# PJLab-ADG/OpenPCSeg

Hardware: AMD Instinct MI355X
Metric: LiDAR frames/sec training MinkUNet-34 SemanticKITTI (higher is better)
Workload: dtype f32; 1 GPU; MinkUNet-34 cr1.0 train step, 12 x 120k-pt synthetic SemanticKITTI scans/GPU, fp32; global_batch=12, voxels_per_gpu_batch=1158864, parallelism=dp1, wgrad=fp32

## Files before the change

include/pcseg_hip.h:

```cpp
#ifndef PCSEG_HIP_H_
#define PCSEG_HIP_H_

#include <stddef.h>
#include <stdint.h>

#ifdef __cplusplus
extern "C" {
#endif

#define PCS_OK 0
#define PCS_EINVAL (-1)
#define PCS_EWORKSPACE (-2)
#define PCS_ELAUNCH (-3)
#define PCS_EUNSUPPORTED (-4)

#define PCS_ABI_VERSION 12

int pcs_abi_version(void);
const char *pcs_last_error(void);

int pcs_hash(const int32_t *coords, int64_t n, int64_t *out, void *stream);

int pcs_kernel_hash(const int32_t *coords, int64_t n, const int32_t *offsets, int32_t K,
                    int64_t *out, void *stream);

int64_t pcs_hashtable_capacity(int64_t n);
size_t pcs_hashtable_bytes(int64_t capacity);
int pcs_hashtable_build(const int64_t *keys, int64_t n, void *table, int64_t capacity,
                        void *stream);
int pcs_hashtable_query(const void *table, int64_t capacity, const int64_t *queries,
                        int64_t n1, int64_t *out, void *stream);

int pcs_count(const int32_t *idx, int64_t n, int32_t *out, int64_t s, void *stream);

int pcs_voxelize_fwd_f32(const float *feats, const int32_t *idx, const int32_t *counts,
                         int64_t n, int64_t m, int32_t c, float *out, void *stream);
size_t pcs_index_csr_ws_bytes(int64_t n, int64_t m);
int pcs_index_csr_i32(const int32_t *index, int64_t n, int64_t m, int64_t *order, int64_t *rowptr, void *ws,
                      size_t ws_bytes, void *stream);
int pcs_voxelize_fwd_csr_f32(const float *feats, const int64_t *order, const int64_t *rowptr,
                             const int32_t *counts, int64_t m, int32_t c, float *out, void *stream);
int pcs_voxelize_bwd_f32(const float *gout, const int32_t *idx, const int32_t *counts,
                         int64_t n, int32_t c, float *gin, void *stream);
int pcs_voxelize_fwd_csr_h(const void *feats, const int64_t *order, const int64_t *rowptr, const int32_t *counts,
                           int64_t m, int32_t c, int32_t dtype, void *out, void *stream);
int pcs_voxelize_bwd_h(const void *gout, const int32_t *idx, const int32_t *counts, int64_t n, int32_t c,
                       int32_t dtype, void *gin, void *stream);

int pcs_devoxelize_fwd_f32(const float *feat, const int32_t *idx8, const float *w8, int64_t n,
                           int32_t c, float *out, void *stream);
int pcs_devoxelize_bwd_f32(const float *gout, const int32_t *idx8, const float *w8, int64_t n,
                           int64_t m, int32_t c, float *gfeat, void *stream);
int pcs_devoxelize_fwd_h(const void *feat, const int32_t *idx8, const float *w8, int64_t n, int32_t c,
                         int32_t dtype, void *out, void *stream);
int pcs_point_merge_f32(const float *vox, const int32_t *idx8, const float *w8, const float *lin, const double *stat,
                        const float *gamma, const float *beta, int64_t n, int32_t c, float *out, uint32_t *mask,
                        void *stream);
int pcs_point_merge_h(const void *vox, const int32_t *idx8, const float *w8, const void *lin, const double *stat,
                      const float *gamma, const float *beta, int64_t n, int32_t c, int32_t dtype, void *out,
                      uint32_t *mask, void *stream);
int pcs_range_point_merge_f32(const float *vox, const int32_t *idx8, const float *w8, const float *img, const float *pxpy,
                              int32_t B, int32_t H, int32_t W, const float *lin, const double *stat, const float *gamma,
                              const float *beta, int64_t n, int32_t c, float *out, uint32_t *mask, void *stream);
int pcs_range_point_merge_h(const void *vox, const int32_t *idx8, const float *w8, const float *img, const float *pxpy,
                            int32_t B, int32_t H, int32_t W, const void *lin, const double *stat, const float *gamma,
                            const float *beta, int64_t n, int32_t c, int32_t dtype, void *out, uint32_t *mask, void *stream);

int pcs_corner_map_f32(const float *coords, int32_t coord_ld, int64_t n, int32_t stride, const void *table,
                       int64_t capacity, int32_t *idx8, float *w8, void *stream);

int pcs_devoxelize_bwd_csr_f32(const float *gout, const int64_t *order, const int64_t *rowptr,
                               const float *w8, int64_t m, int32_t c, float *gfeat, void *stream);
int pcs_devoxelize_bwd_csr_h(const void *gout, const int64_t *order, const int64_t *rowptr, const float *w8,
                             int64_t m, int32_t c, int32_t dtype, void *gfeat, void *stream);
void pcs_debug_pointvoxel_h_inflight(int32_t loads);

int pcs_ti_weights_f32(const float *coords, int32_t coord_ld, const int64_t *idx_query,
                       int64_t n, float scale, float *w, void *stream);

int pcs_downsample_pack(const int32_t *coords, int64_t n, const int32_t *sample_stride3,
                        int32_t mode, const int32_t *offsets, int32_t K,
                        const int32_t *coords_min3, int64_t *keys, int32_t *err, void *stream);
int pcs_downsample_unpack(const int64_t *keys, int64_t m, int32_t *coords, void *stream);
size_t pcs_sort_unique_ws_bytes(int64_t n);
int pcs_sort_unique_i64(const int64_t *keys, int64_t n, int64_t *out, int64_t *info, const int32_t *err_flag, void *ws,
                        size_t ws_bytes, void *stream);

size_t pcs_rulebook_ws_bytes(int64_t nq, int32_t K);
int pcs_rulebook_probe(const int32_t *qcoords, int64_t nq, const int32_t *offsets, int32_t K,
                       const void *table, int64_t capacity, int32_t *results,
                       int64_t *nbsizes, void *ws, size_t ws_bytes, int32_t symmetric, void *stream);
int pcs_rulebook_fill(const int32_t *results, int64_t nq, int32_t K, const void *ws,
                      int32_t *pairs, int32_t *koff, void *stream);
int pcs_rulebook_tile_segments(const int32_t *pairs, const int32_t *koff, int32_t K,
                               int64_t n_dst, int32_t tile_rows, int32_t dst_col,
                               int32_t *seg, void *stream);
int pcs_rulebook_tile_order(const int32_t *seg, int32_t K, int64_t ntiles, int32_t *order, void *stream);

const char *pcs_conv_kernel_revision(void);
int32_t pcs_conv_tile_rows(int32_t cin, int32_t cout);
int32_t pcs_conv_pick_tile_rows(int64_t n_dst, int64_t n_pairs, int32_t K, int32_t cin, int32_t cout);
int32_t pcs_conv_pick_tile_rows_dt(int64_t n_dst, int64_t n_pairs, int32_t K, int32_t cin, int32_t cout,
                                   int32_t dtype);
int32_t pcs_conv_emits_bn_partials(int32_t cin, int32_t cout, int32_t K, int32_t tile_rows, int32_t dtype);
int32_t pcs_conv_uses_tile_order(int32_t cin, int32_t cout, int32_t K, int32_t dtype);
int pcs_conv_gather_gemm_f32(const float *src, int64_t n_src, int32_t cin, const float *W,
                             int32_t K, int32_t cout, const int32_t *pairs, int32_t src_col,
                             const int32_t *seg, int32_t tile_rows, int64_t n_dst,
                             const float *bias, float *dst, double *bn_partial, const int32_t *tile_order,
                             void *stream);
#define PCS_EP_RELU 1
#define PCS_EP_POST_AFFINE 16
typedef struct pcs_conv_epilogue {
  const void *addend;
  float act_slope;
  int32_t flags;
  const float *post_scale;
  const float *post_shift;
} pcs_conv_epilogue;
int pcs_conv_gather_gemm_f32_ex(const float *src, int64_t n_src, int32_t cin, const float *W,
                                int32_t K, int32_t cout, const int32_t *pairs, int32_t src_col,
                                const int32_t *seg, int32_t tile_rows, int64_t n_dst,
                                const float *bias, const pcs_conv_epilogue *ep, float *dst, double *bn_partial,
                                const int32_t *tile_order, void *stream);
int32_t pcs_conv_supports_epilogue(int32_t cin, int32_t cout, int32_t K, int32_t dtype);

int pcs_transpose_kab_f32(const float *src, int32_t K, int32_t A, int32_t B, float *dst, void *stream);

size_t pcs_conv_wgrad_ws_bytes(const int32_t *koff_host, int32_t K, int32_t ca, int32_t cb);
int pcs_conv_wgrad_f32(const float *fa, int32_t ca, const float *fb, int32_t cb,
                       const int32_t *pairs, int32_t a_col, const int32_t *koff_dev,
                       const int32_t *koff_host, int32_t K, float *gW, void *ws,
                       size_t ws_bytes, void *stream);

int pcs_scatter_max_fwd_f32(const float *src, const int64_t *order, const int64_t *rowptr, int64_t m,
                            int32_t c, float *out, int32_t *arg, void *stream);
int pcs_scatter_max_bwd_f32(const float *gout, const int32_t *arg, int64_t m, int64_t n, int32_t c,
                            float *gsrc, void *stream);

int pcs_map_count(const int32_t *pxpy, int64_t n, int32_t B, int32_t H, int32_t W, int32_t *out,
                  void *stream);
int pcs_denselize_fwd_f32(const float *feat, const int32_t *count_map, const int32_t *pxpy, int64_t n,
                          int32_t B, int32_t C, int32_t H, int32_t W, float *out, void *stream);
int pcs_denselize_fwd_csr_f32(const float *feat, const int64_t *order, const int64_t *rowptr,
                              const int32_t *count_map, int32_t B, int32_t C, int32_t H, int32_t W,
                              float *out, void *stream);
int pcs_denselize_bwd_csr_f32(const float *gout, const int64_t *order, const int64_t *rowptr,
                              const int32_t *count_map, int64_t n, int32_t B, int32_t C, int32_t H, int32_t W,
                              float *gfeat, void *stream);
int pcs_denselize_bwd_f32(const float *gout, const int32_t *count_map, const int32_t *pxpy, int64_t n,
                          int32_t B, int32_t C, int32_t H, int32_t W, float *gfeat, void *stream);

int pcs_range_sample_fwd_f32(const float *img, const float *pxpy, int64_t n, int32_t B, int32_t C, int32_t H, int32_t W,
                             float *out, void *stream);
int pcs_range_sample_corners(const float *pxpy, int64_t n, int32_t B, int32_t H, int32_t W, int64_t *keys, float *wts,
                             void *stream);
int pcs_range_sample_bwd_csr_f32(const float *gout, const int64_t *order, const int64_t *rowptr, const float *wts,
                                 int32_t B, int32_t C, int32_t H, int32_t W, float *gimg, void *stream);

int32_t pcs_bn_num_partials(void);
int pcs_bn_stats_f32(const float *x, int64_t n, int32_t c, float *partial_ws, double *sums, void *stream);
int pcs_bn_reduce_partials(const double *partial, int64_t nrows, int32_t c, int64_t n, double *sums, void *stream);
int pcs_bn_reduce_partials_finalize(const double *partial, int64_t nrows, int32_t c, int64_t n, double eps, double momentum,
                                    float *running_mean, float *running_var, double *sums, double *stat, void *stream);
int pcs_bn_finalize_f32(const double *sums, double count, const double *count_dev, int32_t c, double eps,
                        double momentum, float *running_mean, float *running_var, double *stat, void *stream);
int pcs_bn_apply_f32(const float *x, const float *res, const double *stat, const float *w, const float *b,
                     int64_t n, int32_t c, int32_t relu, float *y, uint32_t *mask, int64_t ldy, const float *tail,
                     int32_t ctail, void *stream);
int pcs_bn_bwd_stats_f32(const float *dy, const float *x, const float *y, const uint32_t *mask, const double *stat,
                         int64_t n, int32_t c, int32_t relu, float *partial_ws, double *sums2, int64_t sums2_doubles,
                         int64_t lddy, void *stream);
int pcs_bn_bwd_apply_f32(const float *dy, const float *x, const float *y, const uint32_t *mask, const double *stat,
                         const double *sums2, double count, const double *count_dev, const float *w, int64_t n,
                         int32_t c, int32_t relu, float *dx, float *dres, int64_t lddy, void *stream);
int pcs_bn_stats_h(const void *x, int64_t n, int32_t c, int32_t dtype, float *partial_ws, double *sums, void *stream);
int pcs_bn_apply_h(const void *x, const void *res, const double *stat, const float *w, const float *b, int64_t n,
                   int32_t c, int32_t relu, int32_t dtype, void *y, uint32_t *mask, int64_t ldy, const void *tail,
                   int32_t ctail, void *stream);
int pcs_bn_bwd_stats_h(const void *dy, const void *x, const void *y, const uint32_t *mask, const double *stat, int64_t n,
                       int32_t c, int32_t relu, int32_t dtype, float *partial_ws, double *sums2, int64_t sums2_doubles,
                       int64_t lddy, void *stream);
int pcs_bn_bwd_apply_h(const void *dy, const void *x, const void *y, const uint32_t *mask, const double *stat,
                       const double *sums2, double count, const double *count_dev, const float *w, int64_t n,
                       int32_t c, int32_t relu, int32_t dtype, void *dx, void *dres, int64_t lddy, void *stream);
int pcs_bn_bwd_apply_act(const void *dy, const void *x, const void *y, const uint32_t *mask, const double *stat,
                         const double *sums2, double count, const double *count_dev, const float *w, int64_t n, int32_t c,
                         int32_t relu, int32_t dtype, float in_slope, void *dx, void *dres, int64_t lddy, void *stream);

int pcs_recon_gate_f32(const float *a0, const float *a1, const float *a2, const float *x, const double *stat3,
                       const float *gamma3, const float *beta3, int64_t n, int32_t c, float *out, void *stream);
int pcs_recon_gate_h(const void *a0, const void *a1, const void *a2, const void *x, const double *stat3, const float *gamma3,
                     const float *beta3, int64_t n, int32_t c, int32_t dtype, void *out, void *stream);
int pcs_recon_gate_bwd_stats_f32(const float *dy, const float *x, const float *a0, const float *a1, const float *a2,
                                 const double *stat3, const float *gamma3, const float *beta3, int64_t n, int32_t c,
                                 float *partial_ws, double *sums2, int64_t sums2_doubles, void *stream);
int pcs_recon_gate_bwd_stats_h(const void *dy, const void *x, const void *a0, const void *a1, const void *a2,
                               const double *stat3, const float *gamma3, const float *beta3, int64_t n, int32_t c,
                               int32_t dtype, float *partial_ws, double *sums2, int64_t sums2_doubles, void *stream);
int pcs_recon_gate_bwd_apply_f32(const float *dy, const float *x, const float *a0, const float *a1, const float *a2,
                                 const double *stat3, const float *gamma3, const float *beta3, const double *sums2,
                                 double count, const double *count_dev, int64_t n, int32_t c, float *dx_gate, float *da0,
                                 float *da1, float *da2, void *stream);
int pcs_recon_gate_bwd_apply_h(const void *dy, const void *x, const void *a0, const void *a1, const void *a2,
                               const double *stat3, const float *gamma3, const float *beta3, const double *sums2, double count,
                               const double *count_dev, int64_t n, int32_t c, int32_t dtype, void *dx_gate, void *da0,
                               void *da1, void *da2, void *stream);

int pcs_quantize_floor(const void *points, int32_t is_float, int64_t n, int32_t row_stride,
                       const double *voxel_size3, int32_t *coords, int32_t *bbox, void *stream);
int pcs_quantize_keys(const int32_t *coords, int64_t n, const int32_t *bbox, int64_t *keys, void *stream);
int pcs_quantize_frame_keys(const int32_t *coords, const int64_t *frames, int64_t n, const int32_t *bbox, int64_t *keys, void *stream);
int pcs_quantize_flags(const int64_t *sorted_keys, int64_t n, int32_t *flags, void *stream);
int pcs_quantize_emit(const int32_t *flags, const int64_t *rank, const int64_t *perm, const int32_t *coords,
                      int64_t n, int32_t *vox, int64_t *index, int64_t *inverse, void *stream);

#define PCS_SCAN_MAX_VOTES 16
#define PCS_SCAN_MAX_COLUMNS 8
int64_t pcs_scan_transform_ws_bytes(int64_t n, int32_t num_frames, int32_t num_votes);
int pcs_scan_transform(const float *points, int64_t n, int32_t c, const int64_t *frame_offsets, int32_t num_frames,
                       const double *params, int32_t num_votes, float voxel_size, float *feats, int32_t *coords,
                       int32_t *mins, void *ws, int64_t ws_bytes, void *stream);
int pcs_scan_shift(int32_t *coords, int64_t n, const int64_t *frame_offsets, int32_t num_frames, const int32_t *mins,
                   int32_t num_votes, int64_t *frames, void *stream);

int pcs_unique_emit(const int32_t *flags, const int64_t *rank, const int64_t *perm, const int64_t *sorted_keys,
                    int64_t n, int64_t *uniq, int64_t *inverse, int64_t *rowptr, void *stream);

int pcs_conv_x3_applies(int32_t cin, int32_t cout, int32_t K);
int32_t pcs_conv_x3_column_tiles(int32_t cout);
int32_t pcs_conv_x3_emits_bn_partials(int32_t cin, int32_t cout, int32_t K, int32_t tile_rows);
size_t pcs_conv_prepared_weights_x3_bytes(int32_t K, int32_t ccon, int32_t ccols);
int pcs_conv_prepare_weights_x3(const float *W, int32_t K, int32_t A, int32_t B, int32_t transpose, void *Wp, void *stream);
int pcs_conv_gather_gemm_f32_bf16x3(const float *src, int64_t n_src, int32_t cin, const void *Wp, int32_t K, int32_t cout,
                                    const int32_t *pairs, int32_t src_col, const int32_t *seg, int32_t tile_rows,
                                    int64_t n_dst, const float *bias, float *dst, double *bn_partial,
                                    const int32_t *tile_order, void *stream);

int pcs_conv_h_applies(int32_t cin, int32_t cout, int32_t K);
size_t pcs_conv_prepared_weights_bytes(int32_t K, int32_t contraction, int32_t columns);
int pcs_conv_prepare_weights_h(const float *W, int32_t K, int32_t A, int32_t B, int32_t transpose, int32_t dtype,
                               void *Wp, void *stream);
int pcs_conv_gather_gemm_h(const void *src, int64_t n_src, int32_t cin, const void *Wp, int32_t K, int32_t cout,
                           const int32_t *pairs, int32_t src_col, const int32_t *seg, int32_t tile_rows,
                           int64_t n_dst, const float *bias, void *dst, int32_t dtype, double *bn_partial,
                           const int32_t *tile_order, void *stream);
int pcs_conv_gather_gemm_h_ex(const void *src, int64_t n_src, int32_t cin, const void *Wp, int32_t K, int32_t cout,
                              const int32_t *pairs, int32_t src_col, const int32_t *seg, int32_t tile_rows,
                              int64_t n_dst, const float *bias, const pcs_conv_epilogue *ep, void *dst, int32_t dtype,
                              double *bn_partial, const int32_t *tile_order, void *stream);
int pcs_conv_wgrad_f32_bf16x3(const float *fa, int32_t ca, const float *fb, int32_t cb, const int32_t *pairs,
                              int32_t a_col, const int32_t *koff_dev, const int32_t *koff_host, int32_t K, float *gW,
                              void *ws, size_t ws_bytes, void *stream);
int pcs_conv_wgrad_h(const void *fa, int32_t ca, const void *fb, int32_t cb, const int32_t *pairs, int32_t a_col,
                     const int32_t *koff_dev, const int32_t *koff_host, int32_t K, float *gW, void *ws,
                     size_t ws_bytes, int32_t dtype, void *stream);

int pcs_cylinder_partition_f32(const float *points, int64_t n, int32_t row_stride, const double *space_min3,
                               const double *space_max3, const int32_t *grid3, float *polar, int32_t *coord,
                               float *feat, void *stream);
int pcs_voxel_label_vote(const int64_t *inverse, const int64_t *labels, int64_t n, int64_t m, int32_t num_classes,
                         int64_t ignore_label, int32_t *counter_ws, int32_t *bad_flag, int64_t *voxel_labels,
                         void *stream);
int pcs_rows_argmax_gather_f32(const float *logits, int64_t m, int32_t c, const int64_t *inverse, int64_t n,
                               int64_t *out, void *stream);

int pcs_cylinder_scan_batch_f32(const float *points, int64_t n, int32_t c, const int64_t *frame_offsets, int32_t num_frames,
                                const double *params, int32_t num_votes, const double *space_min3, const double *space_max3,
                                const int32_t *grid3, float *feat, int32_t *coord, int64_t *scenes, void *stream);

int64_t pcs_range_project_ws_bytes(int32_t num_scenes, int32_t H, int32_t W);
int pcs_range_project_f32(const float *feats, int64_t n, int32_t c, const int32_t *scenes, const float *cuts32, int32_t num_scenes,
                          int32_t H, int32_t W, int32_t *winner, float *pxpy, int32_t *bad, void *stream);
int pcs_range_image_fill_f32(const int32_t *winner, const float *feats, int64_t n, int32_t c, int32_t num_scenes, int32_t H,
                             int32_t W, float *image, void *stream);

int64_t pcs_range_scan_ws_bytes(int32_t num_frames, int32_t H, int32_t W);
int pcs_range_scan_f32(const float *points, int64_t n, int32_t c, const int64_t *frame_offsets, int32_t num_frames,
                       const int64_t *labels, const int64_t *lut, int32_t lut_size, int32_t H, int32_t W, float fov_down_abs,
                       float fov_total, int32_t mask_hit, void *winner, float *scan, int64_t *label_rv, float *mask_rv,
                       int32_t *proj_idx, int32_t *proj_x, int32_t *proj_y, float *unproj_range, int32_t *bad, void *stream);
int pcs_range_knn_vote(const float *proj_range, const int64_t *proj_argmax, int32_t num_scenes, int32_t H, int32_t W,
                       const float *unproj_range, const int32_t *proj_x, const int32_t *proj_y, int64_t n,
                       const int64_t *point_offset, int32_t search, int32_t knn, float cutoff, const float *weights_host,
                       int32_t num_class, const int64_t *labels, int64_t *hist, int64_t *pred, void *stream);

#define PCS_MIX_BUCKETS 10
#define PCS_MIX_MAX_CLASSES 8
#define PCS_MIX_PLAN_STRIDE 16
int64_t pcs_scan_mix_ws_bytes(int64_t n1, int64_t n2, int32_t num_frames);
int pcs_scan_mix_count(const float *points1, int64_t n1, const int64_t *frame_offsets1, const float *points2,
                       const int64_t *labels2, int64_t n2, const int64_t *frame_offsets2, int32_t num_frames, const double *plan,
                       const int64_t *classes, int32_t num_classes, void *ws, int64_t ws_bytes, int32_t *totals,
                       int64_t *frame_base, void *stream);
int pcs_scan_mix_place(const float *points1, const int64_t *labels1, int64_t n1, const int64_t *frame_offsets1,
                       const float *points2, const int64_t *labels2, int64_t n2, const int64_t *frame_offsets2,
                       int32_t num_frames, const double *plan, const int64_t *classes, int32_t num_classes, const double *omega,
                       const void *ws, int64_t ws_bytes, const int32_t *totals, const int64_t *frame_base, int64_t m, int32_t c_out,
                       float *out_points, int64_t *out_labels, void *stream);
int64_t pcs_scan_ring_ws_bytes(int64_t m);
int pcs_scan_ring_f32(float *points, int64_t m, int32_t c, const int64_t *frame_base, int32_t num_frames, void *ws,
                      int64_t ws_bytes, void *stream);

int pcs_predict_points_f32(const float *logits, int64_t m, int32_t c, const int64_t *inverse, int64_t n,
                           const int64_t *point_offset, const int64_t *row_offset, int32_t n_scenes,
                           const int64_t *labels, float *votes, int64_t *pred, int64_t *hist, int32_t *bad_flag,
                           void *stream);

typedef struct {
  const float *src;
  void *dst;
  int32_t K, A, B;
  int32_t kind;
  int32_t transpose;
  int32_t nctt, nt16, ns;
  int64_t first_block;
} pcs_weight_job;
int64_t pcs_weights_multi_plan(pcs_weight_job *jobs_host, int32_t n_jobs);
int pcs_weights_multi(const pcs_weight_job *jobs_dev, int32_t n_jobs, int64_t total_blocks, void *stream);

#define PCS_STEP_BLOCK_ELEMS 4096
#define PCS_STEP_MAX_GROUPS 8
#define PCS_STEP_WS_BYTES(total_blocks) (16 + 12 * (int64_t)(total_blocks))
typedef struct {
  float *p;
  const float *g;
  float *buf;
  int64_t numel;
  int32_t group;
  int32_t reserved;
  int64_t first_block;
} pcs_step_job;
typedef struct {
  float lr[PCS_STEP_MAX_GROUPS], wd[PCS_STEP_MAX_GROUPS], mu[PCS_STEP_MAX_GROUPS];
  int32_t nesterov[PCS_STEP_MAX_GROUPS];
  int32_t n_groups;
} pcs_step_hyper;
int64_t pcs_step_plan(pcs_step_job *jobs_host, int32_t n_jobs, const pcs_step_hyper *hyper);
int pcs_step_norm(const pcs_step_job *jobs_dev, int32_t n_jobs, int64_t total_blocks, float max_norm, float *scale,
                  int32_t *growth_tracker, double growth_factor, double backoff_factor, int32_t growth_interval, void *ws,
                  int64_t ws_bytes, float *record, void *stream);
int pcs_step_apply(const pcs_step_job *jobs_dev, int32_t n_jobs, int64_t total_blocks, const pcs_step_hyper *hyper,
                   const float *record, int32_t skip_on_inf, void *stream);

int64_t pcs_lovasz_workspace_bytes(int64_t n, int32_t num_class, int32_t has_ignore, int64_t ignore);
int pcs_lovasz_softmax_f32(const float *probas, const int64_t *labels, int64_t n, int32_t num_class, int32_t has_ignore,
                           int64_t ignore, float *loss, float *grad, void *ws, int64_t ws_bytes, void *stream);

void pcs_debug_convh_ws(int32_t mode, int32_t ru, int32_t rs);
void pcs_debug_conv_plan(int32_t kind, int32_t dtype, int32_t cin, int32_t cout, int32_t K, int32_t tile_rows, int32_t flags,
                         int32_t out[12]);
void pcs_debug_wgrad_interleave(int32_t mode);
void pcs_debug_cylscan_store(int32_t form);

#ifdef __cplusplus
}
#endif
#endif
```

openpcseg_amd/csrc/conv_wgrad.hip:

```cpp
#include "conv_common.h"

using namespace pcs;

namespace {

constexpr int WG_PB = 32;
constexpr int WG_TS = 128 + 16;

struct WgradArgs {
  const float *fa;
  const float *fb;
  const int32_t *pairs;
  const int32_t *koff;
  float *partial;
  int ca, cb, K, a_col, pch;
};

__device__ __forceinline__ void find_split(const int32_t *koff, int K, int pch, int split, int *k_out,
                                           int *beg, int *end) {
  int acc = 0;
  for (int k = 0; k < K; ++k) {
    const int nk = koff[k + 1] - koff[k];
    const int ns = (nk + pch - 1) / pch;
    if (split < acc + ns) {
      const int s = split - acc;
      *k_out = k;
      *beg = koff[k] + s * pch;
      const int e = *beg + pch;
      *end = e < koff[k + 1] ? e : koff[k + 1];
      return;
    }
    acc += ns;
  }
  *k_out = -1; *beg = 0; *end = 0;
}

__device__ __forceinline__ void find_split_wave(const int32_t *koff, int K, int pch, int split, int lane, int *beg,
                                                int *end, int *gsid, int interleave) {
  if (K > 64) {
    int k;
    find_split(koff, K, pch, split, &k, beg, end);
    *gsid = split;
    return;
  }
  const int lo = lane < K ? koff[lane] : 0, hi = lane < K ? koff[lane + 1] : 0;
  const int ns = (hi - lo + pch - 1) / pch;
  int incl = ns;
  for (int o = 1; o < 64; o <<= 1) {
    const int t = __shfl_up(incl, o, 64);
    if (lane >= o) incl += t;
  }
  int src, sidx;
  if (!interleave) {
    const unsigned long long hit = __ballot(split >= incl - ns && split < incl);
    if (!hit) { *beg = 0; *end = 0; *gsid = split; return; }
    src = __ffsll((long long)hit) - 1;
    sidx = split - __shfl(incl - ns, src, 64);
  } else {
    const int total = __shfl(incl, 63, 64);
    if (interleave == 2) {
      const int chunk = (total + 7) >> 3;
      split = (split & 7) * chunk + (split >> 3);
    }
    if (split >= total) { *beg = 0; *end = 0; *gsid = 0; return; }
    int rmax = ns;
    for (int o = 32; o > 0; o >>= 1) { const int t = __shfl_xor(rmax, o, 64); rmax = t > rmax ? t : rmax; }
    auto upto = [&](int r) {
      int c = ns > 0 ? (int)(((long long)r * ns) / rmax) + 1 : 0;
      for (int o = 32; o > 0; o >>= 1) c += __shfl_xor(c, o, 64);
      return c;
    };
    int a = 0, b = rmax - 1;
    while (a < b) {
      const int m = (a + b) >> 1;
      if (upto(m) > split) b = m; else a = m + 1;
    }
    const int r = a;
    const int before = r > 0 ? upto(r - 1) : 0;
    const int s_r = ns > 0 ? (int)(((long long)r * ns) / rmax) : -1;
    const int s_p = (ns > 0 && r > 0) ? (int)(((long long)(r - 1) * ns) / rmax) : -1;
    unsigned long long fresh = __ballot(ns > 0 && s_r != s_p);
    int want = split - before;
    while (want > 0) { fresh &= fresh - 1; --want; }
    src = __ffsll((long long)fresh) - 1;
    sidx = __shfl(s_r, src, 64);
  }
  const int b0 = lo + sidx * pch;
  const int e0 = b0 + pch < hi ? b0 + pch : hi;
  *beg = __shfl(b0, src, 64);
  *end = __shfl(e0, src, 64);
  *gsid = __shfl(incl - ns, src, 64) + sidx;
}

__global__ void __launch_bounds__(256) wgrad_kernel(WgradArgs w) {
  __shared__ __attribute__((aligned(16))) float abuf[WG_PB * WG_TS];
  __shared__ __attribute__((aligned(16))) float bbuf[WG_PB * WG_TS];
  __shared__ int ia[WG_PB], ib[WG_PB];
  __shared__ int sh[3];
  const int tid = threadIdx.x, lane = tid & 63, wid = tid >> 6;
  const int a0 = blockIdx.y * 128, b0 = blockIdx.z * 128;
  const int cat = (w.ca - a0) < 128 ? (w.ca - a0) : 128;
  const int cbt = (w.cb - b0) < 128 ? (w.cb - b0) : 128;
  const int ta_n = (cat + 15) / 16, tb_n = (cbt + 15) / 16;
  if (tid == 0) find_split(w.koff, w.K, w.pch, blockIdx.x, &sh[0], &sh[1], &sh[2]);
  __syncthreads();
  const int beg = sh[1], end = sh[2];
  const int wa = wid >> 1, wb = wid & 1;
  f32x4 acc[4][4];
#pragma unroll
  for (int i = 0; i < 4; ++i)
#pragma unroll
    for (int j = 0; j < 4; ++j) acc[i][j] = (f32x4){0, 0, 0, 0};

  const int capad = ta_n * 16, cbpad = tb_n * 16;
  for (int p0 = beg; p0 < end; p0 += WG_PB) {
    const int np = (end - p0) < WG_PB ? (end - p0) : WG_PB;
    __syncthreads();
    if (tid < WG_PB) {
      int2 p = make_int2(-1, -1);
      if (tid < np) p = reinterpret_cast<const int2 *>(w.pairs)[p0 + tid];
      ia[tid] = w.a_col ? p.y : p.x;
      ib[tid] = w.a_col ? p.x : p.y;
    }
    __syncthreads();
    for (int e = tid; e < WG_PB * capad; e += 256) {
      const int r = e / capad, c = e % capad;
      abuf[r * WG_TS + c] = (r < np && c < cat) ? w.fa[(int64_t)ia[r] * w.ca + a0 + c] : 0.f;
    }
    for (int e = tid; e < WG_PB * cbpad; e += 256) {
      const int r = e / cbpad, c = e % cbpad;
      bbuf[r * WG_TS + c] = (r < np && c < cbt) ? w.fb[(int64_t)ib[r] * w.cb + b0 + c] : 0.f;
    }
    __syncthreads();
    const int g = lane >> 4, l15 = lane & 15;
#pragma unroll
    for (int kk = 0; kk < WG_PB / 4; ++kk) {
      float av[4], bv[4];
#pragma unroll
      for (int i = 0; i < 4; ++i) {
        const int ta = wa + 2 * i;
        av[i] = (ta < ta_n) ? abuf[(kk * 4 + g) * WG_TS + ta * 16 + l15] : 0.f;
      }
#pragma unroll
      for (int j = 0; j < 4; ++j) {
        const int tb = wb + 2 * j;
        bv[j] = (tb < tb_n) ? bbuf[(kk * 4 + g) * WG_TS + tb * 16 + l15] : 0.f;
      }
#pragma unroll
      for (int i = 0; i < 4; ++i) {
        if (wa + 2 * i < ta_n) {
#pragma unroll
          for (int j = 0; j < 4; ++j) {
            if (wb + 2 * j < tb_n)
// ... 97 lines not shown
  __syncthreads();
  if (ql == 0 && ok) {
    float4 t = red[0][et];
#pragma unroll
    for (int j = 1; j < 16; ++j) {
      const float4 v = red[j][et];
      t.x += v.x; t.y += v.y; t.z += v.z; t.w += v.w;
    }
    *reinterpret_cast<float4 *>(gW + (int64_t)k * cc + e) = t;
  }
}

struct Wgrad2Args {
  const void *fa;
  const void *fb;
  const int32_t *pairs;
  const int32_t *koff;
  float *partial;
  int ca, cb, K, a_col, pch, nbg;
  int interleave;
};

__host__ __device__ inline int wg_ngroups(int c) { return (c + 63) / 64; }
__host__ __device__ inline int wg_gwidth(int c) {
  const int per = (c + wg_ngroups(c) - 1) / wg_ngroups(c);
  return (per + 15) / 16 * 16;
}

template <int W> struct WVec;
template <> struct WVec<64> { using T = float4; static constexpr int N = 4; };
template <> struct WVec<48> { using T = float3; static constexpr int N = 3; };
template <> struct WVec<32> { using T = float2; static constexpr int N = 2; };
template <> struct WVec<16> { using T = float;  static constexpr int N = 1; };
__device__ __forceinline__ float wcomp(const float4 &v, int i) { return i == 0 ? v.x : (i == 1 ? v.y : (i == 2 ? v.z : v.w)); }
__device__ __forceinline__ float wcomp(const float3 &v, int i) { return i == 0 ? v.x : (i == 1 ? v.y : v.z); }
__device__ __forceinline__ float wcomp(const float2 &v, int i) { return i == 0 ? v.x : v.y; }
__device__ __forceinline__ float wcomp(const float &v, int) { return v; }

template <typename V, int N> __device__ __forceinline__ V wload(Fp32, const void *base, int64_t elem) {
  return *reinterpret_cast<const V *>(reinterpret_cast<const float *>(base) + elem);
}
template <typename V, int N, typename HT> __device__ __forceinline__ V wload(HT, const void *base, int64_t elem) {
  const uint16_t *p = reinterpret_cast<const uint16_t *>(base) + elem;
  V v;
  if constexpr (N == 4) {
    const uint2 r = *reinterpret_cast<const uint2 *>(p);
    v.x = h2f(HT{}, (uint16_t)(r.x & 0xFFFFu)); v.y = h2f(HT{}, (uint16_t)(r.x >> 16));
    v.z = h2f(HT{}, (uint16_t)(r.y & 0xFFFFu)); v.w = h2f(HT{}, (uint16_t)(r.y >> 16));
  } else if constexpr (N == 3) {
    v.x = h2f(HT{}, p[0]); v.y = h2f(HT{}, p[1]); v.z = h2f(HT{}, p[2]);
  } else if constexpr (N == 2) {
    const uint32_t r = *reinterpret_cast<const uint32_t *>(p);
    v.x = h2f(HT{}, (uint16_t)(r & 0xFFFFu)); v.y = h2f(HT{}, (uint16_t)(r >> 16));
  } else {
    v = h2f(HT{}, p[0]);
  }
  return v;
}

template <int AW, int BW, typename ET>
__device__ __forceinline__ void wgrad_block(const Wgrad2Args &w, int a0, int b0, int beg, int end,
                                            float *out, int lane) {
  using AV = typename WVec<AW>::T;
  using BV = typename WVec<BW>::T;
  constexpr int NA = WVec<AW>::N, NB = WVec<BW>::N;
  const int g = lane >> 4, l15 = lane & 15;
  const int ac = a0 + NA * l15, bc = b0 + NB * l15;
  const bool aok = ac + NA <= w.ca, bok = bc + NB <= w.cb;
  const int acl = aok ? ac : 0, bcl = bok ? bc : 0;
  f32x4 acc[NA][NB];
#pragma unroll
  for (int f = 0; f < NA; ++f)
#pragma unroll
    for (int h = 0; h < NB; ++h) acc[f][h] = (f32x4){0, 0, 0, 0};

  struct Batch { AV a[4]; BV b[4]; };
  auto load_pairs = [&](int p0) {
    int pi = p0 + l15;
    pi = pi < end ? pi : end - 1;
    return reinterpret_cast<const int2 *>(w.pairs)[pi];
  };
  auto load_rows = [&](Batch &bt, const int2 pr) {
    const int ia = w.a_col ? pr.y : pr.x, ib = w.a_col ? pr.x : pr.y;
#pragma unroll
    for (int j = 0; j < 4; ++j) {
      const int ra = __shfl(ia, 4 * j + g, 64), rb = __shfl(ib, 4 * j + g, 64);
      bt.a[j] = wload<AV, NA>(ET{}, w.fa, (int64_t)ra * w.ca + acl);
      bt.b[j] = wload<BV, NB>(ET{}, w.fb, (int64_t)rb * w.cb + bcl);
    }
  };
  auto mfma_batch = [&](const Batch &bt, int p0) {
#pragma unroll
    for (int j = 0; j < 4; ++j) {
      const bool pv = aok && (p0 + 4 * j + g) < end;
#pragma unroll
      for (int f = 0; f < NA; ++f) {
        const float av = pv ? wcomp(bt.a[j], f) : 0.f;
#pragma unroll
        for (int h = 0; h < NB; ++h)
          acc[f][h] = __builtin_amdgcn_mfma_f32_16x16x4f32(av, wcomp(bt.b[j], h), acc[f][h], 0, 0, 0);
      }
    }
  };
  Batch b0s, b1s;
  load_rows(b0s, load_pairs(beg));
  int2 prn = load_pairs(beg + 16 < end ? beg + 16 : beg);
#ifndef PCS_ABLATEW
#define PCS_ABLATEW 0
#endif
#if PCS_ABLATEW == 1
  load_rows(b1s, prn);
#endif
  for (int p0 = beg; p0 < end; p0 += 32) {
    const int p2 = p0 + 32 < end ? p0 + 32 : p0;
    const int p3 = p0 + 48 < end ? p0 + 48 : p0;
#if PCS_ABLATEW != 1
    load_rows(b1s, prn);
#endif
    prn = load_pairs(p2);
    __builtin_amdgcn_sched_barrier(0);
#if PCS_ABLATEW != 2
    mfma_batch(b0s, p0);
#else
    acc[0][0][0] += wcomp(b0s.a[0], 0) + wcomp(b0s.a[1], 0) + wcomp(b0s.a[2], 0) + wcomp(b0s.a[3], 0) + wcomp(b0s.b[0], 0) + wcomp(b0s.b[1], 0) + wcomp(b0s.b[2], 0) + wcomp(b0s.b[3], 0);
#endif
    __builtin_amdgcn_sched_barrier(0);
#if PCS_ABLATEW != 1
    load_rows(b0s, prn);
#endif
    prn = load_pairs(p3);
    __builtin_amdgcn_sched_barrier(0);
#if PCS_ABLATEW != 2
    if (p0 + 16 < end) mfma_batch(b1s, p0 + 16);
#else
    acc[0][0][1] += wcomp(b1s.a[0], 0) + wcomp(b1s.a[1], 0) + wcomp(b1s.a[2], 0) + wcomp(b1s.a[3], 0) + wcomp(b1s.b[0], 0) + wcomp(b1s.b[1], 0) + wcomp(b1s.b[2], 0) + wcomp(b1s.b[3], 0);
#endif
    __builtin_amdgcn_sched_barrier(0);
  }
#pragma unroll
  for (int f = 0; f < NA; ++f) {
#pragma unroll
    for (int r = 0; r < 4; ++r) {
      const int row = a0 + NA * (4 * g + r) + f;
      if (row < w.ca && bok) {
        float *d = out + (int64_t)row * w.cb + bc;
#pragma unroll
        for (int h = 0; h < NB; ++h) d[h] = acc[f][h][r];
      }
    }
  }
}

template <typename ET>
__global__ void __launch_bounds__(256, 3) wgrad2_kernel(Wgrad2Args w) {
  const int tid = threadIdx.x, lane = tid & 63, wid = tid >> 6;
  int beg, end, gsid;
  find_split_wave(w.koff, w.K, w.pch, blockIdx.x, lane, &beg, &end, &gsid, w.interleave);
  const int nag = wg_ngroups(w.ca);
  const int nsb = (w.nbg + 1) >> 1;
  const int sa = blockIdx.y / nsb, sb = blockIdx.y - sa * nsb;
  const int ag = 2 * sa + (wid >> 1), bg = 2 * sb + (wid & 1);
  if (beg >= end || ag >= nag || bg >= w.nbg) return;
  const int aw = wg_gwidth(w.ca), bw = wg_gwidth(w.cb);
  float *out = w.partial + (int64_t)gsid * w.ca * w.cb;
  const int a0 = aw * ag, b0 = bw * bg;
#define PCS_WG_CASE(A, B) if (aw == A && bw == B) { wgrad_block<A, B, ET>(w, a0, b0, beg, end, out, lane); return; }
  PCS_WG_CASE(64, 64) PCS_WG_CASE(64, 48) PCS_WG_CASE(64, 32) PCS_WG_CASE(64, 16)
  PCS_WG_CASE(48, 64) PCS_WG_CASE(48, 48) PCS_WG_CASE(48, 32) PCS_WG_CASE(48, 16)
  PCS_WG_CASE(32, 64) PCS_WG_CASE(32, 48) PCS_WG_CASE(32, 32) PCS_WG_CASE(32, 16)
  PCS_WG_CASE(16, 64) PCS_WG_CASE(16, 48) PCS_WG_CASE(16, 32) PCS_WG_CASE(16, 16)
#undef PCS_WG_CASE
}

constexpr int W3_PB = 32;
constexpr int W3_ROW = 128;

typedef __bf16 w3_bf16x2 __attribute__((ext_vector_type(2)));
typedef float w3_f32x2 __attribute__((ext_vector_type(2)));
typedef __bf16 w3_bf16x8 __attribute__((ext_vector_type(8)));
typedef _Float16 w3_f16x8 __attribute__((ext_vector_type(8)));

struct Wgrad3Args {
  const void *fa;
  const void *fb;
  const int32_t *pairs;
  const int32_t *koff;
  float *partial;
  int ca, cb, K, a_col, pch;
  int aw, bw, nag, nbg, nsb;
  int interleave;
  int nsy = 1;
};

template <typename ET> struct W3Mode;
template <> struct W3Mode<Fp32> { static constexpr int PLANES = 3; using MT = Bf16; };
template <> struct W3Mode<Bf16> { static constexpr int PLANES = 1; using MT = Bf16; };
template <> struct W3Mode<Fp16> { static constexpr int PLANES = 1; using MT = Fp16; };

__device__ __forceinline__ f32x4 w3_mfma(Bf16, const uint4 &a, const uint4 &b, f32x4 c) {
  return __builtin_amdgcn_mfma_f32_16x16x32_bf16(__builtin_bit_cast(w3_bf16x8, a), __builtin_bit_cast(w3_bf16x8, b), c, 0, 0, 0);
}
__device__ __forceinline__ f32x4 w3_mfma(Fp16, const uint4 &a, const uint4 &b, f32x4 c) {
  return __builtin_amdgcn_mfma_f32_16x16x32_f16(__builtin_bit_cast(w3_f16x8, a), __builtin_bit_cast(w3_f16x8, b), c, 0, 0, 0);
}

__device__ __forceinline__ void w3_split(float x, float y, uint32_t &hi, uint32_t &mid, uint32_t &lo) {
  const w3_f32x2 v = {x, y};
  const w3_bf16x2 h = __builtin_convertvector(v, w3_bf16x2);
  const w3_f32x2 r1 = v - __builtin_convertvector(h, w3_f32x2);
  const w3_bf16x2 m = __builtin_convertvector(r1, w3_bf16x2);
  const w3_f32x2 r2 = r1 - __builtin_convertvector(m, w3_f32x2);
  const w3_bf16x2 l = __builtin_convertvector(r2, w3_bf16x2);
  hi = __builtin_bit_cast(uint32_t, h); mid = __builtin_bit_cast(uint32_t, m); lo = __builtin_bit_cast(uint32_t, l);
}

template <typename ET, int NA, int NB, int NT = 256, int ROW = W3_ROW>
__global__ void __launch_bounds__(NT, NT == 256 ? (W3Mode<ET>::PLANES == 1 ? 3 : 2) : 4) wgrad3_kernel(Wgrad3Args w) {
  constexpr int PL = W3Mode<ET>::PLANES;
  using MT = typename W3Mode<ET>::MT;
  constexpr bool F32IN = std::is_same<ET, Fp32>::value;
  constexpr int NBUF = PL == 1 ? 2 : 1;
  constexpr int IMG = PL * 2 * W3_PB * ROW;
  __shared__ __attribute__((aligned(16))) uint16_t lds[NBUF * IMG];
  const int tid = threadIdx.x, lane = tid & 63, wid = tid >> 6;
  const int g = lane >> 4, l15 = lane & 15;
  int beg, end, gsid;
  int bx = blockIdx.x, by = blockIdx.y;
  if (w.interleave == 2 && w.nsy > 1) {
    const int slot = bx >> 3;
    by = slot % w.nsy;
    bx = ((slot / w.nsy) << 3) | (bx & 7);
  }
  find_split_wave(w.koff, w.K, w.pch, bx, lane, &beg, &end, &gsid, w.interleave);
  if (beg >= end) return;
  const int sa = by / w.nsb, sb = by - sa * w.nsb;
  const int a_base = 2 * sa * w.aw, b_base = 2 * sb * w.bw;
  const int a_stage = (w.ca - a_base) < 2 * w.aw ? (w.ca - a_base) : 2 * w.aw;
  const int b_stage = (w.cb - b_base) < 2 * w.bw ? (w.cb - b_base) : 2 * w.bw;
  const int ag = 2 * sa + (wid >> 1), bg = 2 * sb + (wid & 1);
  const bool active = ag < w.nag && bg < w.nbg;
  const int aoff = (wid >> 1) * w.aw, boff = (wid & 1) * w.bw;

  f32x4 acc[NA][NB];
#pragma unroll
  for (int i = 0; i < NA; ++i)
#pragma unroll
    for (int j = 0; j < NB; ++j) acc[i][j] = (f32x4){0, 0, 0, 0};

  constexpr int CPP = F32IN ? 4 : 8;
  constexpr int PPR = ROW / CPP;
  constexpr int PIECES = (W3_PB / 2) * PPR / NT;
  static_assert(PIECES >= 1 && (W3_PB / 2) * PPR % NT == 0, "staging items must divide over the threads");
  uint32_t *ldw = reinterpret_cast<uint32_t *>(lds);
  constexpr int IMGW = IMG / 2;
  constexpr int OPW = (W3_PB / 2) * ROW;
  auto wpos = [](int q, int ch) { return q * ROW + ((((ch >> 4) ^ (q >> 2)) & (ROW / 16 - 1)) << 4) + (ch & 15); };
  int2 prs[PIECES][2];
  uint4 ra[PIECES][2], rb[PIECES][2];
  auto fetch_pairs = [&](int p0) {
#pragma unroll
    for (int i = 0; i < PIECES; ++i) {
      const int q = (tid + NT * i) / PPR;
#pragma unroll
      for (int h = 0; h < 2; ++h) {
        prs[i][h] = make_int2(-1, -1);
        if (p0 + 2 * q + h < end) prs[i][h] = reinterpret_cast<const int2 *>(w.pairs)[p0 + 2 * q + h];
      }
    }
  };
  auto fetch_rows = [&]() {
#pragma unroll
    for (int i = 0; i < PIECES; ++i) {
      const int c = ((tid + NT * i) % PPR) * CPP;
#pragma unroll
      for (int h = 0; h < 2; ++h) {
        const bool pv = prs[i][h].x >= 0;
        const int ia = w.a_col ? prs[i][h].y : prs[i][h].x, ib = w.a_col ? prs[i][h].x : prs[i][h].y;
        ra[i][h] = make_uint4(0u, 0u, 0u, 0u);
        rb[i][h] = make_uint4(0u, 0u, 0u, 0u);
        if (pv && c < a_stage) {
          if (F32IN) ra[i][h] = *reinterpret_cast<const uint4 *>(reinterpret_cast<const float *>(w.fa) + (int64_t)ia * w.ca + a_base + c);
          else ra[i][h] = *reinterpret_cast<const uint4 *>(reinterpret_cast<const uint16_t *>(w.fa) + (int64_t)ia * w.ca + a_base + c);
        }
        if (pv && c < b_stage) {
          if (F32IN) rb[i][h] = *reinterpret_cast<const uint4 *>(reinterpret_cast<const float *>(w.fb) + (int64_t)ib * w.cb + b_base + c);
          else rb[i][h] = *reinterpret_cast<const uint4 *>(reinterpret_cast<const uint16_t *>(w.fb) + (int64_t)ib * w.cb + b_base + c);
        }
      }
    }
  };
  auto stage = [&](int buf) {
#pragma unroll
    for (int i = 0; i < PIECES; ++i) {
      const int e = tid + NT * i, q = e / PPR, c = (e % PPR) * CPP;
      const int pos = wpos(q, c);
#pragma unroll
      for (int op = 0; op < 2; ++op) {
        const uint4 v0 = op ? rb[i][0] : ra[i][0], v1 = op ? rb[i][1] : ra[i][1];
        uint32_t *base = ldw + buf * IMGW + op * OPW + pos;
        if (F32IN) {
          uint4 hi, mid, lo;
          w3_split(__uint_as_float(v0.x), __uint_as_float(v1.x), hi.x, mid.x, lo.x);
          w3_split(__uint_as_float(v0.y), __uint_as_float(v1.y), hi.y, mid.y, lo.y);
          w3_split(__uint_as_float(v0.z), __uint_as_float(v1.z), hi.z, mid.z, lo.z);
          w3_split(__uint_as_float(v0.w), __uint_as_float(v1.w), hi.w, mid.w, lo.w);
          *reinterpret_cast<uint4 *>(base) = hi;
          *reinterpret_cast<uint4 *>(base + 2 * OPW) = mid;
          *reinterpret_cast<uint4 *>(base + 4 * OPW) = lo;
        } else {
          uint4 w0, w1;
          w0.x = __builtin_amdgcn_perm(v1.x, v0.x, 0x05040100u); w0.y = __builtin_amdgcn_perm(v1.x, v0.x, 0x07060302u);
          w0.z = __builtin_amdgcn_perm(v1.y, v0.y, 0x05040100u); w0.w = __builtin_amdgcn_perm(v1.y, v0.y, 0x07060302u);
          w1.x = __builtin_amdgcn_perm(v1.z, v0.z, 0x05040100u); w1.y = __builtin_amdgcn_perm(v1.z, v0.z, 0x07060302u);
          w1.z = __builtin_amdgcn_perm(v1.w, v0.w, 0x05040100u); w1.w = __builtin_amdgcn_perm(v1.w, v0.w, 0x07060302u);
          *reinterpret_cast<uint4 *>(base) = w0;
          *reinterpret_cast<uint4 *>(base + 4) = w1;
        }
      }
    }
  };
  auto frag = [&](int buf, int plane, int op, int ch) {
    const uint32_t *q = ldw + buf * IMGW + (plane * 2 + op) * OPW + wpos(4 * g, ch);
    uint4 f;
    f.x = q[0 * ROW]; f.y = q[1 * ROW]; f.z = q[2 * ROW]; f.w = q[3 * ROW];
    return f;
  };
  auto compute = [&](int buf) {
    uint4 bf[NB][PL];
#pragma unroll
    for (int j = 0; j < NB; ++j)
#pragma unroll
      for (int pl = 0; pl < PL; ++pl) bf[j][pl] = frag(buf, pl, 1, boff + 16 * j + l15);
#pragma unroll
    for (int i = 0; i < NA; ++i) {
      uint4 af[PL];
#pragma unroll
      for (int pl = 0; pl < PL; ++pl) af[pl] = frag(buf, pl, 0, aoff + 16 * i + l15);
      if (PL == 3) {
#pragma unroll
        for (int j = 0; j < NB; ++j) acc[i][j] = w3_mfma(MT{}, af[PL - 1], bf[j][0], acc[i][j]);
#pragma unroll
        for (int j = 0; j < NB; ++j) acc[i][j] = w3_mfma(MT{}, af[0], bf[j][PL - 1], acc[i][j]);
#pragma unroll
        for (int j = 0; j < NB; ++j) acc[i][j] = w3_mfma(MT{}, af[PL / 2], bf[j][PL / 2], acc[i][j]);
#pragma unroll
        for (int j = 0; j < NB; ++j) acc[i][j] = w3_mfma(MT{}, af[PL / 2], bf[j][0], acc[i][j]);
#pragma unroll
        for (int j = 0; j < NB; ++j) acc[i][j] = w3_mfma(MT{}, af[0], bf[j][PL / 2], acc[i][j]);
      }
#pragma unroll
      for (int j = 0; j < NB; ++j) acc[i][j] = w3_mfma(MT{}, af[0], bf[j][0], acc[i][j]);
    }
  };

  fetch_pairs(beg);
  fetch_rows();
  fetch_pairs(beg + W3_PB);
  stage(0);
  __syncthreads();
  int cur = 0;
  for (int p0 = beg; p0 < end; p0 += W3_PB) {
    const bool more = p0 + W3_PB < end;
    if (more) {
      fetch_rows();
      fetch_pairs(p0 + 2 * W3_PB);
    }
    if (active) compute(cur);
    if (NBUF == 2) {
      if (more) stage(cur ^ 1);
      __syncthreads();
      cur ^= 1;
    } else {
      __syncthreads();
      if (more) stage(0);
      __syncthreads();
    }
  }
  if (!active) return;
  const int a0 = a_base + aoff, b0 = b_base + boff;
  float *out = w.partial + (int64_t)gsid * w.ca * w.cb;
#pragma unroll
  for (int i = 0; i < NA; ++i)
#pragma unroll
    for (int r = 0; r < 4; ++r) {
      const int row = a0 + 16 * i + 4 * g + r;
      if (row < w.ca) {
#pragma unroll
        for (int j = 0; j < NB; ++j) {
          const int col = b0 + 16 * j + l15;
          if (col < w.cb) out[(int64_t)row * w.cb + col] = acc[i][j][r];
        }
      }
    }
}

struct WgradEnv { int wgrad3, thin, target, interleave; };
const WgradEnv &wgrad_env() {
  auto num = [](const char *v, int dflt) { return v ? atoi(v) : dflt; };
  static const WgradEnv env = {num(getenv("PCS_WGRAD3"), 1),
                               num(getenv("PCS_WGRAD3_THIN"), 1),
                               num(getenv("PCS_WGRAD_TARGET"), 0),
                               num(getenv("PCS_WGRAD_INTERLEAVE"), -1)};
  return env;
}

int g_wgrad_interleave = -1;
enum class WgradFamily { generic, wgrad2, wgrad3, wgrad3_thin };
struct WgradPlan { WgradFamily family; int pch, ns, interleave; dim3 grid; };

int wgrad_splits(const int32_t *koff_host, int K, int pch) {
  int64_t ns = 0;
  for (int k = 0; k < K; ++k) ns += ceil_div((int64_t)koff_host[k + 1] - koff_host[k], pch);
  return (int)ns;
}

WgradPlan wgrad_route(const int32_t *koff_host, int K, int ca, int cb, int dtype, bool force_split, bool operands_aligned,
                      int use3 = wgrad_env().wgrad3, bool count = true) {
  const WgradEnv &env = wgrad_env();
  const bool half = dtype != 0;
  const int nag = wg_ngroups(ca), nbg = wg_ngroups(cb);
  WgradPlan p;
  const bool thin = use3 >= 1 && env.thin && half && ca % 16 == 0 && cb % 16 == 0 && ca <= 64 && cb <= 64 && ca >= 32 && cb >= 32 &&
                    operands_aligned;
  const bool vec = (ca % 4 == 0) && (cb % 4 == 0) && operands_aligned;
  const int cgran = half ? 8 : 4;
  const bool want3 = !half ? (use3 == 2 || force_split) : (use3 >= 1 && (use3 == 2 || nag * nbg >= 4));
  p.family = thin ? WgradFamily::wgrad3_thin
                  : (vec && want3 && ca % cgran == 0 && cb % cgran == 0) ? WgradFamily::wgrad3
                                                                         : (vec ? WgradFamily::wgrad2 : WgradFamily::generic);
  const int nbq = (nag * nbg + 3) / 4;
  const int64_t P = koff_host[K] - koff_host[0];
  int64_t target = (env.target > 0 ? env.target : (nbq >= 4 ? (half ? 2048 : 3072) : 1536)) / nbq;
  if (thin) target *= 4;
  if (target < K) target = K;
  p.pch = (int)ceil_div(P > 0 ? P : 1, target);
  p.pch = (int)(ceil_div(p.pch, 32) * 32);
  if (p.pch < 64) p.pch = 64;
  p.ns = count ? wgrad_splits(koff_host, K, p.pch) : 0;
  p.interleave = g_wgrad_interleave >= 0 ? g_wgrad_interleave : (env.interleave >= 0 ? env.interleave : (half ? 2 : 0));
  const unsigned nx = (unsigned)(p.interleave == 2 ? 8 * ((p.ns + 7) / 8) : p.ns), nsy = (unsigned)(((nag + 1) / 2) * ((nbg + 1) / 2));
  if (p.family == WgradFamily::generic) p.grid = dim3((unsigned)p.ns, (unsigned)ceil_div(ca, 128), (unsigned)ceil_div(cb, 128));
  else if (p.family == WgradFamily::wgrad2) p.grid = dim3(nx, nsy);
  else p.grid = p.interleave == 2 ? dim3(nx * nsy, 1u) : dim3((unsigned)p.ns, nsy);
  return p;
}

template <typename Args>
Args wgrad_args(const void *fa, const void *fb, const int32_t *pairs, const int32_t *koff_dev, void *ws, int ca, int cb, int K,
                int a_col, int pch) {
  Args w;
  w.fa = static_cast<decltype(w.fa)>(fa); w.fb = static_cast<decltype(w.fb)>(fb); w.pairs = pairs; w.koff = koff_dev;
  w.partial = reinterpret_cast<float *>(ws);
  w.ca = ca; w.cb = cb; w.K = K; w.a_col = a_col; w.pch = pch;
  return w;
}

template <typename ET, int NT, int ROW>
int launch_wgrad3(const Wgrad3Args &w, dim3 grid, hipStream_t st, const char *what) {
  const int na = w.aw / 16, nb = w.bw / 16;
#define PCS_W3_CASE(A, B) if constexpr (NT == 256 || (A >= 2 && B >= 2)) if (na == A && nb == B) { hipLaunchKernelGGL((wgrad3_kernel<ET, A, B, NT, ROW>), grid, dim3(NT), 0, st, w); return check_launch(what); }
  PCS_W3_CASE(4, 4) PCS_W3_CASE(4, 3) PCS_W3_CASE(4, 2) PCS_W3_CASE(4, 1)
  PCS_W3_CASE(3, 4) PCS_W3_CASE(3, 3) PCS_W3_CASE(3, 2) PCS_W3_CASE(3, 1)
  PCS_W3_CASE(2, 4) PCS_W3_CASE(2, 3) PCS_W3_CASE(2, 2) PCS_W3_CASE(2, 1)
  PCS_W3_CASE(1, 4) PCS_W3_CASE(1, 3) PCS_W3_CASE(1, 2) PCS_W3_CASE(1, 1)
#undef PCS_W3_CASE
  set_error("%s: unreachable", what);
  return PCS_EINVAL;
}

}

extern "C" size_t pcs_conv_wgrad_ws_bytes(const int32_t *koff_host, int32_t K, int32_t ca, int32_t cb) {
  if (!koff_host || K <= 0 || ca <= 0 || cb <= 0) return 0;
  int pch = INT_MAX;
  for (int dtype = 0; dtype <= 2; ++dtype)
    for (int in = 0; in < 4; ++in)
      for (int use3 = 0; use3 <= 2; ++use3) pch = std::min(pch, wgrad_route(koff_host, K, ca, cb, dtype, in & 1, in & 2, use3, false).pch);
  return (size_t)std::max(wgrad_splits(koff_host, K, pch), 1) * ca * cb * sizeof(float);
}

extern "C" void pcs_debug_wgrad_interleave(int32_t mode) { g_wgrad_interleave = mode; }

static int conv_wgrad_any(const void *fa, int32_t ca, const void *fb, int32_t cb, const int32_t *pairs, int32_t a_col,
                          const int32_t *koff_dev, const int32_t *koff_host, int32_t K, float *gW, void *ws, size_t ws_bytes,
                          int dtype, void *stream, bool force_split = false) {
  if (ca <= 0 || cb <= 0 || K <= 0 || !koff_dev || !koff_host || !gW || (a_col != 0 && a_col != 1) || dtype < 0 || dtype > 2) {
    set_error("pcs_conv_wgrad_f32: bad args");
    return PCS_EINVAL;
  }
  hipStream_t st = as_stream(stream);
  const WgradPlan p = wgrad_route(koff_host, K, ca, cb, dtype, force_split, (((uintptr_t)fa | (uintptr_t)fb) & 15) == 0);
  const int64_t cc = (int64_t)ca * cb;
  if (p.ns == 0) {
    if (hipMemsetAsync(gW, 0, (size_t)K * cc * 4, st) != hipSuccess) { set_error("pcs_conv_wgrad_f32: memset failed"); return PCS_ELAUNCH; }
    return PCS_OK;
  }
  if (!fa || !fb || !pairs || !ws) { set_error("pcs_conv_wgrad_f32: null pointer"); return PCS_EINVAL; }
  if (ws_bytes < (size_t)p.ns * cc * 4) { set_error("pcs_conv_wgrad_f32: workspace too small"); return PCS_EWORKSPACE; }
  const bool vec = p.family != WgradFamily::generic;
  if (dtype != 0 && !vec) { set_error("pcs_conv_wgrad_h: half operands need channel counts that are multiples of 4 and 16-byte aligned tensors"); return PCS_EUNSUPPORTED; }
  switch (p.family) {
    case WgradFamily::generic:
      hipLaunchKernelGGL(wgrad_kernel, p.grid, dim3(256), 0, st, wgrad_args<WgradArgs>(fa, fb, pairs, koff_dev, ws, ca, cb, K, a_col, p.pch));
      break;
    case WgradFamily::wgrad2: {
      Wgrad2Args w = wgrad_args<Wgrad2Args>(fa, fb, pairs, koff_dev, ws, ca, cb, K, a_col, p.pch);
      w.nbg = wg_ngroups(cb); w.interleave = p.interleave;
      if (dtype == 0) hipLaunchKernelGGL(wgrad2_kernel<Fp32>, p.grid, dim3(256), 0, st, w);
      else if (dtype == 1) hipLaunchKernelGGL(wgrad2_kernel<Bf16>, p.grid, dim3(256), 0, st, w);
      else hipLaunchKernelGGL(wgrad2_kernel<Fp16>, p.grid, dim3(256), 0, st, w);
      break;
    }
    default: {
      Wgrad3Args w = wgrad_args<Wgrad3Args>(fa, fb, pairs, koff_dev, ws, ca, cb, K, a_col, p.pch);
      w.aw = wg_gwidth(ca); w.bw = wg_gwidth(cb); w.nag = wg_ngroups(ca); w.nbg = wg_ngroups(cb); w.nsb = (w.nbg + 1) / 2;
      w.interleave = p.interleave;
      w.nsy = ((w.nag + 1) / 2) * w.nsb;
      const bool thin = p.family == WgradFamily::wgrad3_thin;
      const char *what = thin ? "pcs_conv_wgrad(wgrad3 thin)" : "pcs_conv_wgrad(wgrad3)";
      const int rc3 = thin ? (dtype == 1 ? launch_wgrad3<Bf16, 64, 64>(w, p.grid, st, what) : launch_wgrad3<Fp16, 64, 64>(w, p.grid, st, what))
                      : dtype == 0 ? launch_wgrad3<Fp32, 256, W3_ROW>(w, p.grid, st, what)
                      : dtype == 1 ? launch_wgrad3<Bf16, 256, W3_ROW>(w, p.grid, st, what) : launch_wgrad3<Fp16, 256, W3_ROW>(w, p.grid, st, what);
      if (rc3) return rc3;
    }
  }
  int rc = check_launch("pcs_conv_wgrad_f32");
  if (rc) return rc;
  if (vec && (((uintptr_t)ws | (uintptr_t)gW) & 15) == 0) {
    hipLaunchKernelGGL(wgrad_reduce4_kernel, dim3((unsigned)ceil_div(cc, 64), K), dim3(256), 0, st,
                       reinterpret_cast<const float *>(ws), koff_dev, (int)K, p.pch, cc, gW);
  } else {
    int gx = (int)ceil_div(cc, 256);
    if (gx > 64) gx = 64;
    hipLaunchKernelGGL(wgrad_reduce_kernel, dim3(gx, K), dim3(256), 0, st,
                       reinterpret_cast<const float *>(ws), koff_dev, (int)K, p.pch, cc, gW);
  }
  return check_launch("pcs_conv_wgrad_f32(reduce)");
}

extern "C" int pcs_conv_wgrad_f32(const float *fa, int32_t ca, const float *fb, int32_t cb,
                                  const int32_t *pairs, int32_t a_col, const int32_t *koff_dev,
                                  const int32_t *koff_host, int32_t K, float *gW, void *ws,
                                  size_t ws_bytes, void *stream) {
  return conv_wgrad_any(fa, ca, fb, cb, pairs, a_col, koff_dev, koff_host, K, gW, ws, ws_bytes, 0, stream);
}

extern "C" int pcs_conv_wgrad_h(const void *fa, int32_t ca, const void *fb, int32_t cb,
                                const int32_t *pairs, int32_t a_col, const int32_t *koff_dev,
                                const int32_t *koff_host, int32_t K, float *gW, void *ws,
                                size_t ws_bytes, int32_t dtype, void *stream) {
  if (dtype != 1 && dtype != 2) { set_error("pcs_conv_wgrad_h: dtype must be 1 (bf16) or 2 (fp16)"); return PCS_EINVAL; }
  return conv_wgrad_any(fa, ca, fb, cb, pairs, a_col, koff_dev, koff_host, K, gW, ws, ws_bytes, dtype, stream);
}

extern "C" int pcs_conv_wgrad_f32_bf16x3(const float *fa, int32_t ca, const float *fb, int32_t cb,
                                         const int32_t *pairs, int32_t a_col, const int32_t *koff_dev,
                                         const int32_t *koff_host, int32_t K, float *gW, void *ws,
                                         size_t ws_bytes, void *stream) {
  if ((ca % 4) || (cb % 4) || (((uintptr_t)fa | (uintptr_t)fb) & 15)) { set_error("pcs_conv_wgrad_f32_bf16x3: needs 16-byte granular rows"); return PCS_EUNSUPPORTED; }
  return conv_wgrad_any(fa, ca, fb, cb, pairs, a_col, koff_dev, koff_host, K, gW, ws, ws_bytes, 0, stream, true);
}
```

openpcseg_amd/csrc/norm.hip:

```cpp
#include "row_storage.h"

using namespace pcs;

namespace {

template <int V> struct NV;
template <> struct NV<4> { using T = float4; };
template <> struct NV<1> { using T = float; };
template <int V, typename ET> __device__ __forceinline__ typename NV<V>::T ldv(ET, const void *p, int64_t e) {
  const Acc<V> a = widen(ET{}, *reinterpret_cast<const typename Raw<ET, V>::T *>(reinterpret_cast<const typename Elem<ET>::T *>(p) + e));
  if constexpr (V == 4) return make_float4(a.f[0], a.f[1], a.f[2], a.f[3]);
  else return a.f[0];
}
template <typename ET> __device__ __forceinline__ void stv(ET, void *p, int64_t e, const float4 &v) {
  *reinterpret_cast<typename Raw<ET, 4>::T *>(reinterpret_cast<typename Elem<ET>::T *>(p) + e) = narrow(ET{}, Acc<4>{{v.x, v.y, v.z, v.w}});
}
template <typename ET> __device__ __forceinline__ void stv(ET, void *p, int64_t e, const float &v) {
  reinterpret_cast<typename Elem<ET>::T *>(p)[e] = narrow(ET{}, Acc<1>{{v}});
}

__device__ __forceinline__ float comp(const float4 &v, int i) { return i == 0 ? v.x : (i == 1 ? v.y : (i == 2 ? v.z : v.w)); }
__device__ __forceinline__ float comp(const float &v, int) { return v; }
__device__ __forceinline__ void setc(float4 &v, int i, float s) { if (i == 0) v.x = s; else if (i == 1) v.y = s; else if (i == 2) v.z = s; else v.w = s; }
__device__ __forceinline__ void setc(float &v, int, float s) { v = s; }


template <bool BWD, int V, typename ET>
__global__ void __launch_bounds__(256) bn_partial_kernel(const void *__restrict__ x, const void *__restrict__ dy,
                                                         const void *__restrict__ y, const uint32_t *__restrict__ mask,
                                                         const double *__restrict__ stat,
                                                         int64_t n, int c, int cv, int relu, float *__restrict__ partial,
                                                         int64_t lddy) {
  using VT = typename NV<V>::T;
  extern __shared__ float red[];
  const int tx = threadIdx.x, ty = threadIdx.y, TX = blockDim.x, TY = blockDim.y;
  const int W = TX * V;
  for (int j0 = 0; j0 < cv; j0 += TX) {
    const int j = j0 + tx;
    float s0[V], s1[V];
#pragma unroll
    for (int q = 0; q < V; ++q) { s0[q] = 0.f; s1[q] = 0.f; }
    if (j < cv) {
      float mean[V], invstd[V];
#pragma unroll
      for (int q = 0; q < V; ++q) {
        mean[q] = BWD ? (float)stat[j * V + q] : (n > 0 ? ldv<1>(ET{}, x, j * V + q) : 0.f);
        invstd[q] = BWD ? (float)stat[c + j * V + q] : 0.f;
        if (!BWD && blockIdx.x == 0 && ty == 0) partial[(int64_t)gridDim.x * 2 * c + j * V + q] = mean[q];
      }
#pragma unroll 4
      for (int64_t i = (int64_t)blockIdx.x * TY + ty; i < n; i += (int64_t)gridDim.x * TY) {
        const VT xv = ldv<V>(ET{}, x, i * c + (int64_t)j * V);
        if (BWD) {
          const VT gv = ldv<V>(ET{}, dy, i * lddy + (int64_t)j * V);
          VT yv; unsigned bits = 0xFu;
          if (relu) {
            if (V == 4 && mask) bits = (mask[i * (c >> 5) + (j >> 3)] >> (4 * (j & 7))) & 0xFu;
            else yv = ldv<V>(ET{}, y, i * c + (int64_t)j * V);
          }
#pragma unroll
          for (int q = 0; q < V; ++q) {
            float g = comp(gv, q);
            if (relu && ((V == 4 && mask) ? !((bits >> q) & 1u) : comp(yv, q) <= 0.f)) g = 0.f;
            s0[q] += g;
            s1[q] += g * ((comp(xv, q) - mean[q]) * invstd[q]);
          }
        } else {
#pragma unroll
          for (int q = 0; q < V; ++q) { const float t = comp(xv, q) - mean[q]; s0[q] += t; s1[q] += t * t; }
        }
      }
    }
#pragma unroll
    for (int q = 0; q < V; ++q) {
      red[(ty * 2 + 0) * W + tx * V + q] = s0[q];
      red[(ty * 2 + 1) * W + tx * V + q] = s1[q];
    }
    __syncthreads();
    if (ty == 0 && j < cv) {
#pragma unroll
      for (int q = 0; q < V; ++q) {
        float a = 0.f, b = 0.f;
        for (int r = 0; r < TY; ++r) { a += red[(r * 2 + 0) * W + tx * V + q]; b += red[(r * 2 + 1) * W + tx * V + q]; }
        partial[((int64_t)blockIdx.x * 2 + 0) * c + j * V + q] = a;
        partial[((int64_t)blockIdx.x * 2 + 1) * c + j * V + q] = b;
      }
    }
    __syncthreads();
  }
}

template <typename PT>
__global__ void __launch_bounds__(1024) bn_reduce_kernel(const PT *__restrict__ partial, int nblk, int c,
                                                         const float *__restrict__ pivot, int64_t n,
                                                         double *__restrict__ sums, int write_count,
                                                         float *__restrict__ f32copy = nullptr, double *__restrict__ stat = nullptr,
                                                         double eps = 0.0, double momentum = 0.0, float *running_mean = nullptr,
                                                         float *running_var = nullptr) {
  __shared__ double red[2][kRedLanes][kRedCh + 1];
  __shared__ double red2[2][16][kRedCh + 1];
  const int ch = blockIdx.x * kRedCh + threadIdx.x;
  double s0 = 0.0, s1 = 0.0;
  if (ch < c) {
    PT v0[8], v1[8];
    for (int b0 = threadIdx.y; b0 < nblk; b0 += kRedLanes * 8) {
#pragma unroll
      for (int u = 0; u < 8; ++u) {
        const int b = b0 + kRedLanes * u;
        v0[u] = b < nblk ? partial[(int64_t)b * 2 * c + ch] : (PT)0;
        v1[u] = b < nblk ? partial[(int64_t)b * 2 * c + c + ch] : (PT)0;
      }
#pragma unroll
      for (int u = 0; u < 8; ++u) { s0 += (double)v0[u]; s1 += (double)v1[u]; }
    }
  }
  red[0][threadIdx.y][threadIdx.x] = s0;
  red[1][threadIdx.y][threadIdx.x] = s1;
  __syncthreads();
  if (threadIdx.y < 16) {
    double a = 0.0, b = 0.0;
    for (int r = 0; r < 16; ++r) { a += red[0][threadIdx.y * 16 + r][threadIdx.x]; b += red[1][threadIdx.y * 16 + r][threadIdx.x]; }
    red2[0][threadIdx.y][threadIdx.x] = a;
    red2[1][threadIdx.y][threadIdx.x] = b;
  }
  __syncthreads();
  if (threadIdx.y == 0 && ch < c) {
    double t0 = 0.0, t1 = 0.0;
    for (int r = 0; r < 16; ++r) { t0 += red2[0][r][threadIdx.x]; t1 += red2[1][r][threadIdx.x]; }
    if (pivot) {
      const double p = n > 0 ? (double)pivot[ch] : 0.0, dn = (double)n;
      t1 = t1 + 2.0 * p * t0 + dn * p * p;
      t0 = t0 + dn * p;
    }
    if (sums) {
      sums[ch] = t0;
      sums[c + ch] = t1;
    }
    if (f32copy) {
      f32copy[ch] = (float)t0;
      f32copy[c + ch] = (float)t1;
    }
    if (stat) {
      const double count = n > 0 ? (double)n : 1.0;
      const double mean = t0 / count;
      double var = t1 / count - mean * mean;
      if (var < 0.0) var = 0.0;
      stat[ch] = mean;
      stat[c + ch] = 1.0 / sqrt(var + eps);
      if (running_mean) {
        const double unb = count > 1.0 ? var * count / (count - 1.0) : var;
        running_mean[ch] = (float)((1.0 - momentum) * running_mean[ch] + momentum * mean);
        running_var[ch] = (float)((1.0 - momentum) * running_var[ch] + momentum * unb);
      }
    }
  }
  if (sums && write_count && blockIdx.x == 0 && threadIdx.x == 0 && threadIdx.y == 0) sums[2 * c] = (double)n;
}

__global__ void __launch_bounds__(256) bn_finalize_kernel(const double *__restrict__ sums, double count,
                                                          const double *__restrict__ count_dev, int c,
                                                          double eps, double momentum, float *running_mean,
                                                          float *running_var, double *__restrict__ stat) {
  const int ch = blockIdx.x * blockDim.x + threadIdx.x;
  if (ch >= c) return;
  if (count_dev) count = *count_dev;
  if (!(count > 0.0)) count = 1.0;
  const double mean = sums[ch] / count;
  double var = sums[c + ch] / count - mean * mean;
  if (var < 0.0) var = 0.0;
  stat[ch] = mean;
  stat[c + ch] = 1.0 / sqrt(var + eps);
  if (running_mean) {
    const double unb = count > 1.0 ? var * count / (count - 1.0) : var;
    running_mean[ch] = (float)((1.0 - momentum) * running_mean[ch] + momentum * mean);
    running_var[ch] = (float)((1.0 - momentum) * running_var[ch] + momentum * unb);
  }
}

template <int V, typename ET>
__global__ void __launch_bounds__(256) bn_apply_kernel(const void *__restrict__ x, const void *__restrict__ res,
                                                       const double *__restrict__ stat, const float *__restrict__ w,
                                                       const float *__restrict__ b, int64_t n, int c, int cv, int relu,
                                                       void *__restrict__ y, uint32_t *__restrict__ mask, int64_t ldy,
                                                       const void *__restrict__ tail, int ctail) {
  using VT = typename NV<V>::T;
  for (int j = threadIdx.x; j < ctail / V; j += blockDim.x) {
#pragma unroll 4
    for (int64_t i = (int64_t)blockIdx.x * blockDim.y + threadIdx.y; i < n; i += (int64_t)gridDim.x * blockDim.y)
      stv(ET{}, y, i * ldy + c + (int64_t)j * V, ldv<V>(ET{}, tail, i * ctail + (int64_t)j * V));
  }
  for (int j = threadIdx.x; j < cv; j += blockDim.x) {
    float sc[V], sh[V];
#pragma unroll
    for (int q = 0; q < V; ++q) {
      const int ch = j * V + q;
      const float invstd = (float)stat[c + ch], mean = (float)stat[ch];
      sc[q] = invstd * (w ? w[ch] : 1.f);
      sh[q] = (b ? b[ch] : 0.f) - mean * sc[q];
    }
#pragma unroll 4
    for (int64_t i = (int64_t)blockIdx.x * blockDim.y + threadIdx.y; i < n; i += (int64_t)gridDim.x * blockDim.y) {
      const VT xv = ldv<V>(ET{}, x, i * c + (int64_t)j * V);
      VT rv; if (res) rv = ldv<V>(ET{}, res, i * c + (int64_t)j * V);
      VT o;
#pragma unroll
      for (int q = 0; q < V; ++q) {
        float t = fmaf(comp(xv, q), sc[q], sh[q]);
        if (res) t += comp(rv, q);
        if (relu && t < 0.f) t = 0.f;
        setc(o, q, t);
      }
      stv(ET{}, y, i * ldy + (int64_t)j * V, o);
      if (V == 4 && mask) {
        unsigned bits = 0;
#pragma unroll
        for (int q = 0; q < V; ++q) bits |= (stored(ET{}, comp(o, q)) > 0.f ? 1u : 0u) << q;
        unsigned m = bits << (4 * (j & 7));
        m |= __shfl_xor(m, 1, 64); m |= __shfl_xor(m, 2, 64); m |= __shfl_xor(m, 4, 64);
        if ((j & 7) == 0) mask[i * (c >> 5) + (j >> 3)] = m;
      }
    }
  }
}

template <int V, typename ET>
__global__ void __launch_bounds__(256) bn_bwd_apply_kernel(const void *__restrict__ dy, const void *__restrict__ x,
                                                           const void *__restrict__ y, const uint32_t *__restrict__ mask,
                                                           const double *__restrict__ stat,
                                                           const double *__restrict__ sums2, double count,
                                                           const double *__restrict__ count_dev,
                                                           const float *__restrict__ w, int64_t n, int c, int cv,
                                                           int relu, void *__restrict__ dx, void *__restrict__ dres,
                                                           int64_t lddy, float in_slope) {
  using VT = typename NV<V>::T;
  if (count_dev) count = *count_dev;
  if (!(count > 0.0)) count = 1.0;
  for (int j = threadIdx.x; j < cv; j += blockDim.x) {
    float mean[V], invstd[V], k1[V], k2[V], ws[V];
#pragma unroll
    for (int q = 0; q < V; ++q) {
      const int ch = j * V + q;
      mean[q] = (float)stat[ch]; invstd[q] = (float)stat[c + ch];
      k1[q] = (float)(sums2[ch] / count);
      k2[q] = (float)(sums2[c + ch] / count);
      ws[q] = invstd[q] * (w ? w[ch] : 1.f);
    }
#pragma unroll 4
    for (int64_t i = (int64_t)blockIdx.x * blockDim.y + threadIdx.y; i < n; i += (int64_t)gridDim.x * blockDim.y) {
      const VT gv = ldv<V>(ET{}, dy, i * lddy + (int64_t)j * V);
      const VT xv = ldv<V>(ET{}, x, i * c + (int64_t)j * V);
      VT yv; unsigned bits = 0xFu;
      if (relu) {
        if (V == 4 && mask) bits = (mask[i * (c >> 5) + (j >> 3)] >> (4 * (j & 7))) & 0xFu;
        else yv = ldv<V>(ET{}, y, i * c + (int64_t)j * V);
      }
      VT o, r;
#pragma unroll
      for (int q = 0; q < V; ++q) {
        float g = comp(gv, q);
        if (relu && ((V == 4 && mask) ? !((bits >> q) & 1u) : comp(yv, q) <= 0.f)) g = 0.f;
        const float xh = (comp(xv, q) - mean[q]) * invstd[q];
        float d = (g - k1[q] - xh * k2[q]) * ws[q];
        if (in_slope != 1.f && !(comp(xv, q) > 0.f)) d *= in_slope;
        setc(o, q, d);
        setc(r, q, g);
      }
      stv(ET{}, dx, i * c + (int64_t)j * V, o);
      if (dres) stv(ET{}, dres, i * c + (int64_t)j * V, r);
    }
  }
}

template <int V> RowLaunch geo(int64_t n, int c) { return row_launch(n, c / V, kRowsExact4); }

}

extern "C" int32_t pcs_bn_num_partials(void) { return kStatBlocks + 1; }

static bool al_v4(int dtype, const void *p) { return aligned(p, dtype == 0 ? 16 : 8); }

static int bn_partial(bool bwd, int dtype, const void *x, const void *dy, const void *y, const uint32_t *mask, const double *stat,
                      int64_t n, int c, int relu, float *partial, double *sums, hipStream_t st, int64_t lddy = 0) {
  if (lddy == 0) lddy = c;
  if (lddy < c) { set_error("pcs_bn: row stride of dy smaller than c"); return PCS_EINVAL; }
  const bool vec = (c & 3) == 0 && (lddy & 3) == 0 && al_v4(dtype, x) && al_v4(dtype, dy) && al_v4(dtype, y);
  if (mask && (!vec || (c & 31))) { set_error("pcs_bn: the ReLU bit mask needs c % 32 == 0 and aligned rows"); return PCS_EUNSUPPORTED; }
  const int V = vec ? 4 : 1, cv = c / V;
  const dim3 block = row_launch(n, cv, kRowsExact4).block;
  const size_t lds = (size_t)block.y * 2 * block.x * V * sizeof(float);
  if (vec) {
    if (bwd) PCS_DTYPE(dtype, hipLaunchKernelGGL((bn_partial_kernel<true, 4, ET>), dim3(kStatBlocks), block, lds, st, x, dy, y, mask, stat, n, c, cv, relu, partial, lddy));
    else PCS_DTYPE(dtype, hipLaunchKernelGGL((bn_partial_kernel<false, 4, ET>), dim3(kStatBlocks), block, lds, st, x, dy, y, mask, stat, n, c, cv, relu, partial, lddy));
  } else {
    if (bwd) PCS_DTYPE(dtype, hipLaunchKernelGGL((bn_partial_kernel<true, 1, ET>), dim3(kStatBlocks), block, lds, st, x, dy, y, mask, stat, n, c, cv, relu, partial, lddy));
    else PCS_DTYPE(dtype, hipLaunchKernelGGL((bn_partial_kernel<false, 1, ET>), dim3(kStatBlocks), block, lds, st, x, dy, y, mask, stat, n, c, cv, relu, partial, lddy));
  }
  const float *pivot = bwd ? nullptr : partial + (size_t)kStatBlocks * 2 * c;
  hipLaunchKernelGGL(bn_reduce_kernel<float>, dim3((unsigned)ceil_div(c, kRedCh)), dim3(kRedCh, kRedLanes), 0, st, partial, kStatBlocks, c,
                     pivot, n, sums, bwd ? 0 : 1, bwd ? reinterpret_cast<float *>(sums + 2 * (size_t)c) : (float *)nullptr,
                     (double *)nullptr, 0.0, 0.0, (float *)nullptr, (float *)nullptr);
  return check_launch("pcs_bn_partial");
}

static int bn_apply_any(int dtype, const void *x, const void *res, const double *stat, const float *w, const float *b,
                        int64_t n, int32_t c, int32_t relu, void *y, uint32_t *mask, int64_t ldy, const void *tail,
                        int32_t ctail, void *stream) {
  if (n < 0 || c <= 0 || ctail < 0) { set_error("pcs_bn_apply: bad sizes"); return PCS_EINVAL; }
  if (n == 0) return PCS_OK;
  if (!x || !stat || !y || (ctail > 0 && !tail)) { set_error("pcs_bn_apply: null pointer"); return PCS_EINVAL; }
  if (ldy == 0) ldy = c;
  if (ldy < (int64_t)c + ctail) { set_error("pcs_bn_apply: row stride of y smaller than c + ctail"); return PCS_EINVAL; }
  hipStream_t st = as_stream(stream);
  const bool vec = (c & 3) == 0 && (ldy & 3) == 0 && (ctail & 3) == 0 && al_v4(dtype, x) && al_v4(dtype, y) && al_v4(dtype, res) &&
                   al_v4(dtype, tail);
  if (mask && (!vec || (c & 31))) { set_error("pcs_bn_apply: the ReLU bit mask needs c % 32 == 0 and aligned rows"); return PCS_EUNSUPPORTED; }
  if (vec) {
    const RowLaunch g = geo<4>(n, c);
    PCS_DTYPE(dtype, hipLaunchKernelGGL((bn_apply_kernel<4, ET>), g.grid, g.block, 0, st, x, res, stat, w, b, n, c, g.cv, relu, y, mask, ldy, tail, ctail));
  } else {
    const RowLaunch g = geo<1>(n, c);
    PCS_DTYPE(dtype, hipLaunchKernelGGL((bn_apply_kernel<1, ET>), g.grid, g.block, 0, st, x, res, stat, w, b, n, c, g.cv, relu, y, mask, ldy, tail, ctail));
  }
  return check_launch("pcs_bn_apply");
}

static int bn_bwd_apply_any(int dtype, const void *dy, const void *x, const void *y, const uint32_t *mask,
                            const double *stat, const double *sums2, double count, const double *count_dev,
                            const float *w, int64_t n, int32_t c, int32_t relu, void *dx, void *dres, int64_t lddy,
                            void *stream, float in_slope = 1.f) {
  if (n < 0 || c <= 0) { set_error("pcs_bn_bwd_apply: bad sizes"); return PCS_EINVAL; }
  if (n == 0) return PCS_OK;
  if (!count_dev && !(count > 0)) { set_error("pcs_bn_bwd_apply: count must be positive"); return PCS_EINVAL; }
  if (lddy == 0) lddy = c;
  if (lddy < c) { set_error("pcs_bn_bwd_apply: row stride of dy smaller than c"); return PCS_EINVAL; }
  if (!dy || !x || !stat || !sums2 || !dx || (relu && !y && !mask)) { set_error("pcs_bn_bwd_apply: null pointer"); return PCS_EINVAL; }
  hipStream_t st = as_stream(stream);
  const bool vec = (c & 3) == 0 && (lddy & 3) == 0 && al_v4(dtype, dy) && al_v4(dtype, x) && al_v4(dtype, y) && al_v4(dtype, dx) && al_v4(dtype, dres);
  if (mask && (!vec || (c & 31))) { set_error("pcs_bn_bwd_apply: the ReLU bit mask needs c % 32 == 0 and aligned rows"); return PCS_EUNSUPPORTED; }
  if (vec) {
    const RowLaunch g = geo<4>(n, c);
    PCS_DTYPE(dtype, hipLaunchKernelGGL((bn_bwd_apply_kernel<4, ET>), g.grid, g.block, 0, st, dy, x, y, mask, stat, sums2, count, count_dev, w, n, c, g.cv, relu, dx, dres, lddy, in_slope));
  } else {
    const RowLaunch g = geo<1>(n, c);
    PCS_DTYPE(dtype, hipLaunchKernelGGL((bn_bwd_apply_kernel<1, ET>), g.grid, g.block, 0, st, dy, x, y, mask, stat, sums2, count, count_dev, w, n, c, g.cv, relu, dx, dres, lddy, in_slope));
  }
  return check_launch("pcs_bn_bwd_apply");
}

extern "C" int pcs_bn_stats_f32(const float *x, int64_t n, int32_t c, float *partial_ws, double *sums, void *stream) {
  if (n < 0 || c <= 0 || (n > 0 && !x) || !partial_ws || !sums) { set_error("pcs_bn_stats: bad args"); return PCS_EINVAL; }
  return bn_partial(false, 0, x, nullptr, nullptr, nullptr, nullptr, n, c, 0, partial_ws, sums, as_stream(stream));
}
extern "C" int pcs_bn_stats_h(const void *x, int64_t n, int32_t c, int32_t dtype, float *partial_ws, double *sums, void *stream) {
  if (n < 0 || c <= 0 || (n > 0 && !x) || !partial_ws || !sums || !is_half(dtype)) { set_error("pcs_bn_stats_h: bad args"); return PCS_EINVAL; }
  return bn_partial(false, dtype, x, nullptr, nullptr, nullptr, nullptr, n, c, 0, partial_ws, sums, as_stream(stream));
}

extern "C" int pcs_bn_reduce_partials(const double *partial, int64_t nrows, int32_t c, int64_t n, double *sums, void *stream) {
  if (nrows < 0 || nrows > 0x7FFFFFFF || c <= 0 || n < 0 || (nrows > 0 && !partial) || !sums) { set_error("pcs_bn_reduce_partials: bad args"); return PCS_EINVAL; }
  hipLaunchKernelGGL(bn_reduce_kernel<double>, dim3((unsigned)ceil_div(c, kRedCh)), dim3(kRedCh, kRedLanes), 0, as_stream(stream), partial,
                     (int)nrows, c, (const float *)nullptr, n, sums, 1, (float *)nullptr, (double *)nullptr, 0.0, 0.0,
                     (float *)nullptr, (float *)nullptr);
  return check_launch("pcs_bn_reduce_partials");
}

extern "C" int pcs_bn_reduce_partials_finalize(const double *partial, int64_t nrows, int32_t c, int64_t n, double eps,
                                               double momentum, float *running_mean, float *running_var, double *sums,
                                               double *stat, void *stream) {
  if (nrows < 0 || nrows > 0x7FFFFFFF || c <= 0 || n < 0 || (nrows > 0 && !partial) || !stat || (!running_mean) != (!running_var)) {
    set_error("pcs_bn_reduce_partials_finalize: bad args");
    return PCS_EINVAL;
  }
  hipLaunchKernelGGL(bn_reduce_kernel<double>, dim3((unsigned)ceil_div(c, kRedCh)), dim3(kRedCh, kRedLanes), 0, as_stream(stream), partial,
                     (int)nrows, c, (const float *)nullptr, n, sums, 1, (float *)nullptr, stat, eps, momentum, running_mean,
                     running_var);
  return check_launch("pcs_bn_reduce_partials_finalize");
}

extern "C" int pcs_bn_finalize_f32(const double *sums, double count, const double *count_dev, int32_t c, double eps,
                                   double momentum, float *running_mean, float *running_var, double *stat, void *stream) {
  if (c <= 0 || (!count_dev && !(count > 0)) || !sums || !stat) { set_error("pcs_bn_finalize: bad args"); return PCS_EINVAL; }
  hipLaunchKernelGGL(bn_finalize_kernel, dim3((unsigned)ceil_div(c, 256)), dim3(256), 0, as_stream(stream), sums, count,
                     count_dev, c, eps, momentum, running_mean, running_var, stat);
  return check_launch("pcs_bn_finalize");
}

extern "C" int pcs_bn_apply_f32(const float *x, const float *res, const double *stat, const float *w, const float *b,
                                int64_t n, int32_t c, int32_t relu, float *y, uint32_t *mask, int64_t ldy, const float *tail,
                                int32_t ctail, void *stream) {
  return bn_apply_any(0, x, res, stat, w, b, n, c, relu, y, mask, ldy, tail, ctail, stream);
}
extern "C" int pcs_bn_apply_h(const void *x, const void *res, const double *stat, const float *w, const float *b,
                              int64_t n, int32_t c, int32_t relu, int32_t dtype, void *y, uint32_t *mask, int64_t ldy,
                              const void *tail, int32_t ctail, void *stream) {
  if (bad_half("pcs_bn_apply_h", dtype, false)) return PCS_EINVAL;
  return bn_apply_any(dtype, x, res, stat, w, b, n, c, relu, y, mask, ldy, tail, ctail, stream);
}

extern "C" int pcs_bn_bwd_stats_f32(const float *dy, const float *x, const float *y, const uint32_t *mask,
                                    const double *stat, int64_t n, int32_t c, int32_t relu, float *partial_ws,
                                    double *sums2, int64_t sums2_doubles, int64_t lddy, void *stream) {
  if (n < 0 || c <= 0 || (n > 0 && (!dy || !x || (relu && !y && !mask))) || !stat || !partial_ws || !sums2) { set_error("pcs_bn_bwd_stats: bad args"); return PCS_EINVAL; }
  if (sums2_doubles < 3 * (int64_t)c) { set_error("pcs_bn_bwd_stats: sums2 must hold 3c doubles (2c sums + the same 2c values as floats)"); return PCS_EWORKSPACE; }
  return bn_partial(true, 0, x, dy, y, mask, stat, n, c, relu, partial_ws, sums2, as_stream(stream), lddy);
}
extern "C" int pcs_bn_bwd_stats_h(const void *dy, const void *x, const void *y, const uint32_t *mask,
                                  const double *stat, int64_t n, int32_t c, int32_t relu, int32_t dtype, float *partial_ws,
                                  double *sums2, int64_t sums2_doubles, int64_t lddy, void *stream) {
  if (n < 0 || c <= 0 || (n > 0 && (!dy || !x || (relu && !y && !mask))) || !stat || !partial_ws || !sums2 || !is_half(dtype)) { set_error("pcs_bn_bwd_stats_h: bad args"); return PCS_EINVAL; }
  if (sums2_doubles < 3 * (int64_t)c) { set_error("pcs_bn_bwd_stats_h: sums2 must hold 3c doubles (2c sums + the same 2c values as floats)"); return PCS_EWORKSPACE; }
  return bn_partial(true, dtype, x, dy, y, mask, stat, n, c, relu, partial_ws, sums2, as_stream(stream), lddy);
}

extern "C" int pcs_bn_bwd_apply_f32(const float *dy, const float *x, const float *y, const uint32_t *mask,
                                    const double *stat, const double *sums2, double count, const double *count_dev,
                                    const float *w, int64_t n, int32_t c, int32_t relu, float *dx, float *dres,
                                    int64_t lddy, void *stream) {
  return bn_bwd_apply_any(0, dy, x, y, mask, stat, sums2, count, count_dev, w, n, c, relu, dx, dres, lddy, stream);
}
extern "C" int pcs_bn_bwd_apply_act(const void *dy, const void *x, const void *y, const uint32_t *mask,
                                    const double *stat, const double *sums2, double count, const double *count_dev,
                                    const float *w, int64_t n, int32_t c, int32_t relu, int32_t dtype, float in_slope, void *dx,
                                    void *dres, int64_t lddy, void *stream) {
  if (dtype < 0 || dtype > 2 || !(in_slope > 0.f)) { set_error("pcs_bn_bwd_apply_act: dtype must be 0 / 1 / 2 and in_slope > 0"); return PCS_EINVAL; }
  return bn_bwd_apply_any(dtype, dy, x, y, mask, stat, sums2, count, count_dev, w, n, c, relu, dx, dres, lddy, stream, in_slope);
}
extern "C" int pcs_bn_bwd_apply_h(const void *dy, const void *x, const void *y, const uint32_t *mask,
                                  const double *stat, const double *sums2, double count, const double *count_dev,
                                  const float *w, int64_t n, int32_t c, int32_t relu, int32_t dtype, void *dx, void *dres,
                                  int64_t lddy, void *stream) {
  if (bad_half("pcs_bn_bwd_apply_h", dtype, false)) return PCS_EINVAL;
  return bn_bwd_apply_any(dtype, dy, x, y, mask, stat, sums2, count, count_dev, w, n, c, relu, dx, dres, lddy, stream);
}
```

openpcseg_amd/functional.py:

```python
import os

import torch
from torch.autograd import Function
from torch.amp import custom_bwd, custom_fwd

from . import native
from .sparse import SparseTensor, get_kernel_offsets, make_ntuple

__all__ = ["sphash", "sphashquery", "spcount", "spvoxelize", "spdevoxelize", "calc_ti_weights",
           "spdownsample", "prebuild_coords", "conv3d", "conv3d_inference", "relu", "leaky_relu"]


def _be():
    return native.backend()


def sphash(coords, offsets=None):
    assert coords.dtype == torch.int, coords.dtype
    assert coords.ndim == 2 and coords.shape[1] == 4, coords.shape
    coords = coords.contiguous()
    if offsets is None:
        return _be().hash(coords)
    assert offsets.dtype == torch.int, offsets.dtype
    assert offsets.ndim == 2 and offsets.shape[1] == 3, offsets.shape
# ... 25 lines not shown


def _voxelize_forward(ctx, feats, coords, counts):
    feats = feats.contiguous()
    holder = coords
    coords = coords.contiguous().int()
    out = _be().voxelize_fwd(feats, coords, counts, cache_on=holder)
    ctx.for_backwards = (coords, counts, feats.shape[0])
    return out


def _devoxelize_forward(ctx, feats, coords, weights):
    feats = feats.contiguous()
    coords = coords.contiguous().int()
    weights = weights.contiguous().float()
    out = _be().devoxelize_fwd(feats, coords, weights)
    ctx.for_backwards = (coords, weights, feats.shape[0])
    return out


class _Voxelize(Function):
    @staticmethod
    @custom_fwd(device_type="cuda", cast_inputs=torch.float32)
    def forward(ctx, feats, coords, counts):
        return _voxelize_forward(ctx, feats, coords, counts)

    @staticmethod
    @custom_bwd(device_type="cuda")
    def backward(ctx, grad_output):
        coords, counts, n = ctx.for_backwards
        return _be().voxelize_bwd(grad_output.contiguous(), coords, counts, n), None, None


class _VoxelizeKeep(_Voxelize):

    @staticmethod
    @custom_fwd(device_type="cuda")
    def forward(ctx, feats, coords, counts):
        return _voxelize_forward(ctx, feats, coords, counts)


def spvoxelize(feats, coords, counts):
    fn = _VoxelizeKeep if _POINTVOXEL_POLICY["mode"] == "keep" else _Voxelize
    return fn.apply(feats, coords, counts)


class _Devoxelize(Function):
    @staticmethod
    @custom_fwd(device_type="cuda", cast_inputs=torch.float32)
    def forward(ctx, feats, coords, weights):
        return _devoxelize_forward(ctx, feats, coords, weights)

    @staticmethod
    @custom_bwd(device_type="cuda")
    def backward(ctx, grad_output):
        coords, weights, m = ctx.for_backwards
        return _be().devoxelize_bwd(grad_output.contiguous(), coords, weights, m), None, None


class _DevoxelizeKeep(_Devoxelize):
    @staticmethod
    @custom_fwd(device_type="cuda")
    def forward(ctx, feats, coords, weights):
        return _devoxelize_forward(ctx, feats, coords, weights)


def spdevoxelize(feats, coords, weights):
    fn = _DevoxelizeKeep if _POINTVOXEL_POLICY["mode"] == "keep" else _Devoxelize
    return fn.apply(feats, coords, weights)


def calc_ti_weights(coords, idx_query, scale=1):
    with torch.no_grad():
        return _be().ti_weights(coords.float(), idx_query.long(), scale)


def spdownsample(coords, stride=2, kernel_size=2, tensor_stride=1):
    stride = make_ntuple(stride, ndim=3)
    kernel_size = make_ntuple(kernel_size, ndim=3)
    tensor_stride = make_ntuple(tensor_stride, ndim=3)
    sample_stride = [stride[k] * tensor_stride[k] for k in range(3)]
    if all(stride[k] in [1, kernel_size[k]] for k in range(3)):
        return _be().downsample(coords, sample_stride)
    offsets = get_kernel_offsets(kernel_size, tensor_stride, device=coords.device)
    coords_min = torch.min(coords[:, :3], dim=0).values.int()
    return _be().downsample(coords, sample_stride, offsets, coords_min)


class KmapEntry(list):

    def __init__(self, fwd, in_coords, out_coords, offsets, symmetric=False, hint_key=None):
        super().__init__([None, fwd.nbsizes, (in_coords.shape[0], out_coords.shape[0])])
        self.fwd = fwd
        self._rev = None
        self._ctx = (in_coords, out_coords, offsets)
        self._hint_key = hint_key
        self._mirror = symmetric and in_coords is out_coords

    def __getitem__(self, i):
        if isinstance(i, int) and i in (0, -3):
            return self.fwd.pairs
        return super().__getitem__(i)

    def __iter__(self):
        return iter([self[0], super().__getitem__(1), super().__getitem__(2)])

    @property
    def rev(self):
        if self._rev is None:
            in_coords, out_coords, offsets = self._ctx
            if self._mirror:
                self._rev = self.fwd.mirror()
            else:
                key = None if self._hint_key is None else self._hint_key + ("rev",)
                self._rev = _be().build_kmap(out_coords, in_coords, -offsets, hint_key=key)
        return self._rev


def build_kernel_map(in_coords, out_coords, kernel_size, in_stride, dilation):
    offsets = get_kernel_offsets(kernel_size, stride=in_stride, dilation=dilation, device="cpu")
    symmetric = bool(torch.equal(offsets.flip(0), -offsets))
    offsets = (offsets.pin_memory() if in_coords.is_cuda else offsets).to(in_coords.device, non_blocking=True)
    hint_key = (tuple(kernel_size), tuple(in_stride), tuple(dilation), in_coords is out_coords)
    fwd = _be().build_kmap(in_coords, out_coords, offsets, hint_key=hint_key, symmetric=symmetric and in_coords is out_coords)
    return KmapEntry(fwd, in_coords, out_coords, offsets, symmetric, hint_key)


_HALF = (torch.bfloat16, torch.float16)

_WGRAD_POLICY = {"mode": "fp32"}


def set_wgrad_policy(mode):
    if mode not in ("fp32", "bf16x3"):
        raise ValueError("wgrad policy must be 'fp32' or 'bf16x3'")
    _WGRAD_POLICY["mode"] = mode


def get_wgrad_policy():
    return _WGRAD_POLICY["mode"]


_CONV_POLICY = {"mode": "fp32"}


def set_conv_policy(mode):
    if mode not in ("fp32", "bf16x3"):
        raise ValueError("conv policy must be 'fp32' or 'bf16x3'")
    _CONV_POLICY["mode"] = mode


def get_conv_policy():
    return _CONV_POLICY["mode"]


def _wgrad_split(cin, cout):
    return _WGRAD_POLICY["mode"] == "bf16x3" and cin >= 96 and cout >= 96 and cin % 4 == 0 and cout % 4 == 0


def _amp_dtype(t):
    if t.dtype in _HALF:
        return t.dtype
    if t.is_cuda and torch.is_autocast_enabled("cuda"):
        d = torch.get_autocast_dtype("cuda")
        return d if d in _HALF else None
    return None


class _WeightPrep:

    def __init__(self):
        self.entries = {}
        self.pass_id = 0

    @staticmethod
    def usable(be, weight):
        return (hasattr(be, "weights_multi") and isinstance(weight, torch.nn.Parameter) and weight.is_cuda and weight.dim() == 3 and
                weight.dtype == torch.float32 and weight.is_contiguous() and os.environ.get("PCS_WEIGHT_PREP", "1") != "0")

    def invalidate(self):
        self.pass_id += 1

    def _stamp(self, w):
        return (self.pass_id, w._version, w.data_ptr())

    def get(self, be, weight, key):
        import weakref
        e = self.entries.get(id(weight))
        if e is None or e[0]() is not weight:
            self.entries = {i: v for i, v in self.entries.items() if v[0]() is not None}
            e = [weakref.ref(weight), None, {}, set()]
            self.entries[id(weight)] = e
        if e[1] is not None and e[1][0] == self.pass_id and key in e[3]:
            self.pass_id += 1
        if e[1] == self._stamp(weight) and key in e[2]:
            e[3].add(key)
            return e[2][key]
        if key not in e[2]:
            e[2][key] = be.prepared_weights_buffer(weight, *((("t", False)) if key == ("t",) else key))
        jobs, marks = [], []
        for v in self.entries.values():
            w = v[0]()
            if w is None or w.device != weight.device:
                continue
            stamp = self._stamp(w)
            if v[1] != stamp or (v is e):
                for k_, dst in v[2].items():
                    if v[1] != stamp or k_ == key:
                        jobs.append((w.detach(), dst, "t" if k_ == ("t",) else k_[0], False if k_ == ("t",) else k_[1]))
                marks.append((v, stamp))
        be.weights_multi(jobs)
        for v, stamp in marks:
            if v[1] != stamp:
                v[3] = set()
            v[1] = stamp
        e[3].add(key)
        return e[2][key]


_WEIGHT_PREP = _WeightPrep()


def invalidate_prepared_weights():
    _WEIGHT_PREP.invalidate()


try:
    from torch.optim.optimizer import register_optimizer_step_post_hook as _reg_post_step
    _reg_post_step(lambda opt, args, kwargs: _WEIGHT_PREP.invalidate())
except ImportError:
    pass


def _conv_family(be, hd, on_device, cin, cout, k, x3=True):
    if not on_device:
        return "fp32"
    if hd is not None:
        return "half" if be.conv_h_applies(cin, cout, k) else "fp32"
    if x3 and _CONV_POLICY["mode"] == "bf16x3" and be.conv_x3_applies(cin, cout, k):
        return "x3"
    return "fp32"


def _memo(cache, key, make):
    if cache is None:
        return make()
    if key not in cache:
        cache[key] = make()
    return cache[key]


def _per_call(key, make):
    return make()


def _kept_in_pass(be, weight):
    return lambda key, make: (_WEIGHT_PREP.get(be, weight, key) if (key == ("t",) or key[0] in _HALF) and _WeightPrep.usable(be, weight)
                              else make())


def _kept_in(memo, prefix=()):
    return lambda key, make: _memo(memo, prefix + key, make)


def _weight_copy(be, w3, key, kept):
    def make():
        w = w3.detach().float().contiguous()
        if key == ("t",):
            return be.transpose_weights(w)
        return be.prepare_weights_x3(w, transpose=key[1]) if key[0] == "x3" else be.prepare_weights_h(w, key[0], transpose=key[1])
    return kept(key, make)


def _run_conv(be, fam, x, w3, kmap, hd, kept, transpose=False, bias=None, stats=None, addend=None, cast_addend=False,
              act_slope=None, relu=False, rounded=True, post_scale=None, post_shift=None, act_optional=False):
    k, a, b = w3.shape
    cin, cout = (b, a) if transpose else (a, b)
    kdt = hd if fam == "half" else torch.float32
    x = x.contiguous().to(hd) if fam == "half" else x.contiguous().float()
    if fam != "fp32":
        wp = _weight_copy(be, w3, (hd if fam == "half" else "x3", transpose), kept)
    else:
        wp = _weight_copy(be, w3, ("t",), kept) if transpose else w3.float().contiguous()
    kw = {}
    if bias is not None:
        kw["bias"] = bias
    if stats is not None:
        kw["bn_sums"] = stats
        if getattr(be, "supports_bn_raw", False):
            kw["bn_raw"] = True
    post = post_scale is not None
    if act_slope is not None and not act_optional:
        assert fam != "x3", "act_slope: the bf16x3 entry has no write-back extras (conv_act_fusable)"
        kw["act_slope"] = float(act_slope)
    took = False
    if (addend is not None or relu or post or (act_optional and act_slope is not None)) and fam != "x3" and \
            hasattr(be, "conv_supports_addend") and (not relu or getattr(be, "conv_epilogue_relu", False)) and \
            (not post or getattr(be, "conv_epilogue_post_affine", False)) and \
            (addend is None or cast_addend or (addend.is_cuda and addend.dtype == kdt == (hd or torch.float32))):
        code = native.HipBackend._HALF[hd] if fam == "half" else 0
        took = kept(("epilogue?", code, transpose), lambda: be.conv_supports_addend(cin, cout, k, code))
    if took and addend is not None:
        kw["addend"] = addend.to(hd) if fam == "half" else addend.float()
    if took and relu:
        kw["relu"] = True
    if took and act_optional and act_slope is not None:
        kw["act_slope"] = float(act_slope)
    if took and post:
        kw["post_scale"], kw["post_shift"] = post_scale, post_shift
    if fam == "fp32":
        out = be.conv_gather_gemm(x, wp, kmap, **kw)
    else:
        out = getattr(be, "conv_gather_gemm_h" if fam == "half" else "conv_gather_gemm_x3")(x, wp, k, cout, kmap, **kw)
    if rounded and hd is not None and out.dtype != hd:
        out = out.to(hd)
        if stats is not None:
            del stats[:]
    return out, x, took


class _SparseConv(Function):

    @staticmethod
    def forward(ctx, input, weight, entry, transposed, want_stats=False, with_skip=False, act_slope=None):
        be = _be()
        hd = _amp_dtype(input)
        w3 = weight if weight.dim() == 3 else weight.unsqueeze(0)
        k, cin, cout = w3.shape
        kmap = entry.rev if transposed else entry.fwd
        got = [] if want_stats else None
        fam = _conv_family(be, hd, input.is_cuda, cin, cout, k)
        out, x, _ = _run_conv(be, fam, input, w3, kmap, hd, _kept_in_pass(be, weight), stats=got, act_slope=act_slope)
        ctx.for_backwards = (x, weight, entry, transposed, hd)
        ctx.with_skip = with_skip
        ctx.in_dtype = input.dtype
        ctx.set_materialize_grads(False)
        outs = [out]
        if want_stats:
            sums = got[0] if got else torch.empty(0, dtype=torch.float64, device=out.device)
            ctx.mark_non_differentiable(sums)
            outs.append(sums)
        if with_skip:
            outs.append(input.view_as(input))
        return outs[0] if len(outs) == 1 else tuple(outs)

    @staticmethod
    def backward(ctx, grad_output, *rest):
        grad_skip = rest[-1] if ctx.with_skip and rest else None
        if grad_output is None:
            return grad_skip, None, None, None, None, None, None
        be = _be()
        x, weight, entry, transposed, hd = ctx.for_backwards
        w3 = weight if weight.dim() == 3 else weight.unsqueeze(0)
        k, cin, cout = w3.shape
        grad_input = grad_weight = None
        need_dx, need_dw = ctx.needs_input_grad[0], ctx.needs_input_grad[1]
        if need_dx:
            dmap = entry.fwd if transposed else entry.rev
            fam = _conv_family(be, hd, grad_output.is_cuda, cout, cin, k)
            grad_input, _, took = _run_conv(be, fam, grad_output, w3, dmap, hd, _kept_in_pass(be, weight), transpose=True,
                                            addend=grad_skip)
            if grad_skip is not None and not took:
                grad_input = grad_input + grad_skip.to(grad_input.dtype)
        elif grad_skip is not None:
            grad_input = grad_skip
        if need_dw:
            a_col = 1 if transposed else 0
            grad_weight = _weight_grad(be, x, grad_output.contiguous(), entry.fwd, a_col, x.dtype, split=_wgrad_split(cin, cout))
            grad_weight = grad_weight.view_as(weight).to(weight.dtype)
        return grad_input, grad_weight, None, None, None, None, None


def _weight_grad(be, fa, fb, kmap, a_col, hd, *, split=False, pad_a=False, pad_b=False):
    ca, cb = fa.shape[1], fb.shape[1]
    fa = torch.nn.functional.pad(fa, (0, (-ca) % 4)) if pad_a and ca % 4 else fa
    fb = torch.nn.functional.pad(fb, (0, (-cb) % 4)) if pad_b and cb % 4 else fb
    if hd in _HALF and hasattr(be, "conv_wgrad_h") and fa.shape[1] % 4 == 0 and fb.shape[1] % 4 == 0:
        gw = be.conv_wgrad_h(fa.to(hd), fb.to(hd), kmap, a_col)
    else:
        gw = be.conv_wgrad(fa.float(), fb.float(), kmap, a_col, split=split)
    return gw if gw.shape[1:] == (ca, cb) else gw[:, :ca, :cb]


def conv_act_fusable(feats, weight):
    be = _be()
    if not (feats.is_cuda and hasattr(be, "conv_supports_addend") and weight.dim() == 3) or _channel_padding(feats, weight) != (0, 0):
        return False
    k, cin, cout = weight.shape
    fam = _conv_family(be, _amp_dtype(feats), True, cin, cout, k)
    return fam == "half" or (fam == "fp32" and be.conv_supports_addend(cin, cout, k, 0))


def _identity_map(n, device, cache, limit=None):
    if limit is not None and len(cache) > limit:
        cache.clear()
    key = ("_pcs_identity", n, str(device))
    km = cache.get(key)
    if km is None:
        idx = torch.arange(n, dtype=torch.int32, device=device)
        km = native.KernelMap(torch.stack([idx, idx], dim=1).contiguous(),
                              native._h2d([0, n], torch.int32, device), [0, n],
                              native._h2d([n], torch.int64, device), n, n)
        cache[key] = km
    return km


def _rows_weight_grad(x, dy, hd, cache, limit=None, pad_in=False, pad_out=False):
    km = _identity_map(x.shape[0], x.device, cache, limit)
    return _weight_grad(_be(), x.contiguous(), dy, km, 0, hd, pad_a=pad_in, pad_b=pad_out)[0]


class _PointwiseConv(Function):

    @staticmethod
    def forward(ctx, feats, weight, cache):
        hd = _amp_dtype(feats)
        ctx.save_for_backward(feats, weight)
        ctx.cache, ctx.hd = cache, hd
        if hd is None:
            return feats.float().matmul(weight.float())
        return feats.to(hd).matmul(weight.to(hd))

    @staticmethod
    def backward(ctx, grad_output):
        feats, weight = ctx.saved_tensors
        grad_output = grad_output.contiguous()
        hd = ctx.hd
        gin = gw = None
        if ctx.needs_input_grad[0]:
            if hd is None:
                gin = grad_output.float().matmul(weight.float().t())
            else:
                gin = grad_output.to(hd).matmul(weight.to(hd).t())
        if ctx.needs_input_grad[1]:
            pad = feats.is_cuda and feats.shape[1] + (-feats.shape[1]) % 4 >= 32
            gw = _rows_weight_grad(feats, grad_output, hd, ctx.cache, pad_in=pad, pad_out=pad).to(weight.dtype)
        return gin, gw, None


def _channel_padding(feats, weight):
    if not feats.is_cuda or weight.dim() != 3 or weight.shape[0] > 32:
        return 0, 0
    k, cin, cout = weight.shape
    q = 8 if _amp_dtype(feats) is not None else 4
    pin, pout = (-cin) % q, (-cout) % q
    if (pin == 0 and pout == 0) or cin + pin < 32:
        return 0, 0
    return pin, pout


def _sparse_conv(feats, weight, entry, transposed, bn_stats, with_skip=False, act_slope=None):
    pin, pout = _channel_padding(feats, weight)
    assert act_slope is None or not (pin or pout), "act_slope: the caller checks conv_act_fusable()"
    x, cout, node_skip = feats, weight.shape[-1], bool(with_skip)
    if pin or pout:
        x = torch.nn.functional.pad(feats, (0, pin)) if pin else feats
        weight = torch.nn.functional.pad(weight, (0, pout, 0, pin))
        bn_stats = node_skip = False
    outs = _SparseConv.apply(x, weight, entry, transposed, bool(bn_stats), node_skip, act_slope)
    outs = outs if isinstance(outs, tuple) else (outs,)
    out = outs[0][:, :cout].contiguous() if pout else outs[0]
    sums = outs[1] if bn_stats and outs[1].numel() else None
    return (out, sums, outs[-1] if node_skip else feats) if with_skip else (out, sums)


def prebuild_coords(x, steps):
    coords, ts = x.coords, make_ntuple(x.stride, ndim=3)
    for stride, kernel_size in steps:
        stride, kernel_size = make_ntuple(stride, ndim=3), make_ntuple(kernel_size, ndim=3)
        out_stride = tuple(ts[k] * stride[k] for k in range(3))
        if out_stride in x.cmaps:
            coords = x.cmaps[out_stride]
        elif all(s == 1 for s in stride):
            pass
        else:
            coords = spdownsample(coords, stride, kernel_size, ts)
            x.cmaps[out_stride] = coords
        ts = out_stride
    return x


def _conv_geometry(input, kernel_size, stride, dilation, transposed):
    kernel_size = make_ntuple(kernel_size, ndim=3)
    stride = make_ntuple(stride, ndim=3)
    dilation = make_ntuple(dilation, ndim=3)
    ones = (1, 1, 1)
    if kernel_size == ones and stride == ones and dilation == ones:
        return input.stride, input.coords, None
    if not transposed:
        output_stride = tuple(input.stride[k] * stride[k] for k in range(3))
        if output_stride in input.cmaps:
            output_coords = input.cmaps[output_stride]
        elif all(stride[k] == 1 for k in range(3)):
            output_coords = input.coords
        else:
            output_coords = spdownsample(input.coords, stride, kernel_size, input.stride)
        key = (input.stride, kernel_size, stride, dilation)
        if key not in input.kmaps:
            input.kmaps[key] = build_kernel_map(input.coords, output_coords, kernel_size,
                                                input.stride, dilation)
        return output_stride, output_coords, input.kmaps[key]
    output_stride = tuple(input.stride[k] // stride[k] for k in range(3))
    output_coords = input.cmaps[output_stride]
    key = (output_stride, kernel_size, stride, dilation)
    return output_stride, output_coords, input.kmaps[key]


def conv3d(input, weight, kernel_size, bias=None, stride=1, dilation=1, transposed=False, bn_stats=False, with_skip=False,
           act_slope=None):
    skip_feats = None
    bn_sums = None
    output_stride, output_coords, entry = _conv_geometry(input, kernel_size, stride, dilation, transposed)

    if entry is None:
        if input.feats.is_cuda and weight.dim() == 2:
            output_feats = _PointwiseConv.apply(input.feats, weight, input.kmaps)
        else:
            output_feats = input.feats.matmul(weight)
    elif with_skip:
        output_feats, bn_sums, skip_feats = _sparse_conv(input.feats, weight, entry, bool(transposed), bn_stats and bias is None, True, act_slope)
    else:
        output_feats, bn_sums = _sparse_conv(input.feats, weight, entry, bool(transposed), bn_stats and bias is None, False, act_slope)

    if bias is not None:
        output_feats += bias

    output = SparseTensor(coords=output_coords, feats=output_feats, stride=output_stride)
    output.cmaps = input.cmaps
    output.cmaps.setdefault(output_stride, output_coords)
    output.kmaps = input.kmaps
    if bn_sums is not None:
# ... 70 lines not shown
```

openpcseg_amd/native.py:

```python
import ctypes
import os
from ctypes import c_char_p, c_double, c_float, c_int32, c_int64, c_size_t, c_void_p

import torch

_LIB_PATH = os.environ.get("PCS_LIB_PATH") or os.path.join(os.path.dirname(os.path.abspath(__file__)), "lib",
                                                          "libpcseg_hip.so")

_P = c_void_p
SIGNATURES = {
    "pcs_abi_version": (c_int32, []),
    "pcs_last_error": (c_char_p, []),
    "pcs_hash": (c_int32, [_P, c_int64, _P, _P]),
    "pcs_kernel_hash": (c_int32, [_P, c_int64, _P, c_int32, _P, _P]),
    "pcs_hashtable_capacity": (c_int64, [c_int64]),
    "pcs_hashtable_bytes": (c_size_t, [c_int64]),
    "pcs_hashtable_build": (c_int32, [_P, c_int64, _P, c_int64, _P]),
    "pcs_hashtable_query": (c_int32, [_P, c_int64, _P, c_int64, _P, _P]),
    "pcs_count": (c_int32, [_P, c_int64, _P, c_int64, _P]),
    "pcs_voxelize_fwd_f32": (c_int32, [_P, _P, _P, c_int64, c_int64, c_int32, _P, _P]),
    "pcs_voxelize_fwd_csr_f32": (c_int32, [_P, _P, _P, _P, c_int64, c_int32, _P, _P]),
    "pcs_voxelize_bwd_f32": (c_int32, [_P, _P, _P, c_int64, c_int32, _P, _P]),
    "pcs_devoxelize_fwd_f32": (c_int32, [_P, _P, _P, c_int64, c_int32, _P, _P]),
    "pcs_devoxelize_bwd_f32": (c_int32, [_P, _P, _P, c_int64, c_int64, c_int32, _P, _P]),
    "pcs_devoxelize_bwd_csr_f32": (c_int32, [_P, _P, _P, _P, c_int64, c_int32, _P, _P]),
    "pcs_voxelize_fwd_csr_h": (c_int32, [_P, _P, _P, _P, c_int64, c_int32, c_int32, _P, _P]),
    "pcs_voxelize_bwd_h": (c_int32, [_P, _P, _P, c_int64, c_int32, c_int32, _P, _P]),
    "pcs_devoxelize_fwd_h": (c_int32, [_P, _P, _P, c_int64, c_int32, c_int32, _P, _P]),
    "pcs_devoxelize_bwd_csr_h": (c_int32, [_P, _P, _P, _P, c_int64, c_int32, c_int32, _P, _P]),
    "pcs_point_merge_f32": (c_int32, [_P, _P, _P, _P, _P, _P, _P, c_int64, c_int32, _P, _P, _P]),
    "pcs_point_merge_h": (c_int32, [_P, _P, _P, _P, _P, _P, _P, c_int64, c_int32, c_int32, _P, _P, _P]),
    "pcs_range_point_merge_f32": (c_int32, [_P, _P, _P, _P, _P, c_int32, c_int32, c_int32, _P, _P, _P, _P, c_int64, c_int32, _P, _P, _P]),
    "pcs_range_point_merge_h": (c_int32, [_P, _P, _P, _P, _P, c_int32, c_int32, c_int32, _P, _P, _P, _P, c_int64, c_int32, c_int32,
                                          _P, _P, _P]),
    "pcs_recon_gate_f32": (c_int32, [_P, _P, _P, _P, _P, _P, _P, c_int64, c_int32, _P, _P]),
    "pcs_recon_gate_h": (c_int32, [_P, _P, _P, _P, _P, _P, _P, c_int64, c_int32, c_int32, _P, _P]),
    "pcs_recon_gate_bwd_stats_f32": (c_int32, [_P, _P, _P, _P, _P, _P, _P, _P, c_int64, c_int32, _P, _P, c_int64, _P]),
    "pcs_recon_gate_bwd_stats_h": (c_int32, [_P, _P, _P, _P, _P, _P, _P, _P, c_int64, c_int32, c_int32, _P, _P, c_int64, _P]),
    "pcs_recon_gate_bwd_apply_f32": (c_int32, [_P, _P, _P, _P, _P, _P, _P, _P, _P, c_double, _P, c_int64, c_int32,
                                               _P, _P, _P, _P, _P]),
    "pcs_recon_gate_bwd_apply_h": (c_int32, [_P, _P, _P, _P, _P, _P, _P, _P, _P, c_double, _P, c_int64, c_int32, c_int32,
                                             _P, _P, _P, _P, _P]),
    "pcs_corner_map_f32": (c_int32, [_P, c_int32, c_int64, c_int32, _P, c_int64, _P, _P, _P]),
    "pcs_ti_weights_f32": (c_int32, [_P, c_int32, _P, c_int64, c_float, _P, _P]),
    "pcs_downsample_pack": (c_int32, [_P, c_int64, _P, c_int32, _P, c_int32, _P, _P, _P, _P]),
    "pcs_downsample_unpack": (c_int32, [_P, c_int64, _P, _P]),
    "pcs_index_csr_ws_bytes": (c_size_t, [c_int64, c_int64]),
    "pcs_index_csr_i32": (c_int32, [_P, c_int64, c_int64, _P, _P, _P, c_size_t, _P]),
    "pcs_sort_unique_ws_bytes": (c_size_t, [c_int64]),
    "pcs_sort_unique_i64": (c_int32, [_P, c_int64, _P, _P, _P, _P, c_size_t, _P]),
    "pcs_rulebook_ws_bytes": (c_size_t, [c_int64, c_int32]),
    "pcs_rulebook_probe": (c_int32, [_P, c_int64, _P, c_int32, _P, c_int64, _P, _P, _P, c_size_t, c_int32, _P]),
    "pcs_rulebook_fill": (c_int32, [_P, c_int64, c_int32, _P, _P, _P, _P]),
    "pcs_rulebook_tile_segments": (c_int32, [_P, _P, c_int32, c_int64, c_int32, c_int32, _P, _P]),
    "pcs_rulebook_tile_order": (c_int32, [_P, c_int32, c_int64, _P, _P]),
    "pcs_conv_kernel_revision": (c_char_p, []),
    "pcs_conv_tile_rows": (c_int32, [c_int32, c_int32]),
    "pcs_conv_pick_tile_rows": (c_int32, [c_int64, c_int64, c_int32, c_int32, c_int32]),
    "pcs_conv_pick_tile_rows_dt": (c_int32, [c_int64, c_int64, c_int32, c_int32, c_int32, c_int32]),
    "pcs_conv_emits_bn_partials": (c_int32, [c_int32, c_int32, c_int32, c_int32, c_int32]),
    "pcs_conv_uses_tile_order": (c_int32, [c_int32, c_int32, c_int32, c_int32]),
    "pcs_conv_gather_gemm_f32": (c_int32, [_P, c_int64, c_int32, _P, c_int32, c_int32, _P, c_int32,
                                           _P, c_int32, c_int64, _P, _P, _P, _P, _P]),
    "pcs_conv_gather_gemm_f32_ex": (c_int32, [_P, c_int64, c_int32, _P, c_int32, c_int32, _P, c_int32,
                                              _P, c_int32, c_int64, _P, _P, _P, _P, _P, _P]),
    "pcs_conv_supports_epilogue": (c_int32, [c_int32, c_int32, c_int32, c_int32]),
    "pcs_bn_bwd_apply_act": (c_int32, [_P, _P, _P, _P, _P, _P, c_double, _P, _P, c_int64, c_int32, c_int32, c_int32, c_float, _P, _P,
                                       c_int64, _P]),
    "pcs_bn_reduce_partials": (c_int32, [_P, c_int64, c_int32, c_int64, _P, _P]),
    "pcs_bn_reduce_partials_finalize": (c_int32, [_P, c_int64, c_int32, c_int64, c_double, c_double, _P, _P, _P, _P, _P]),
    "pcs_transpose_kab_f32": (c_int32, [_P, c_int32, c_int32, c_int32, _P, _P]),
    "pcs_conv_wgrad_ws_bytes": (c_size_t, [_P, c_int32, c_int32, c_int32]),
    "pcs_conv_wgrad_f32": (c_int32, [_P, c_int32, _P, c_int32, _P, c_int32, _P, _P, c_int32, _P,
                                     _P, c_size_t, _P]),
    "pcs_scatter_max_fwd_f32": (c_int32, [_P, _P, _P, c_int64, c_int32, _P, _P, _P]),
    "pcs_scatter_max_bwd_f32": (c_int32, [_P, _P, c_int64, c_int64, c_int32, _P, _P]),
    "pcs_map_count": (c_int32, [_P, c_int64, c_int32, c_int32, c_int32, _P, _P]),
    "pcs_denselize_fwd_f32": (c_int32, [_P, _P, _P, c_int64, c_int32, c_int32, c_int32, c_int32, _P, _P]),
    "pcs_denselize_fwd_csr_f32": (c_int32, [_P, _P, _P, _P, c_int32, c_int32, c_int32, c_int32, _P, _P]),
    "pcs_denselize_bwd_csr_f32": (c_int32, [_P, _P, _P, _P, c_int64, c_int32, c_int32, c_int32, c_int32, _P, _P]),
    "pcs_denselize_bwd_f32": (c_int32, [_P, _P, _P, c_int64, c_int32, c_int32, c_int32, c_int32, _P, _P]),
    "pcs_range_sample_fwd_f32": (c_int32, [_P, _P, c_int64, c_int32, c_int32, c_int32, c_int32, _P, _P]),
    "pcs_range_sample_corners": (c_int32, [_P, c_int64, c_int32, c_int32, c_int32, _P, _P, _P]),
    "pcs_range_sample_bwd_csr_f32": (c_int32, [_P, _P, _P, _P, c_int32, c_int32, c_int32, c_int32, _P, _P]),
    "pcs_bn_num_partials": (c_int32, []),
    "pcs_bn_stats_f32": (c_int32, [_P, c_int64, c_int32, _P, _P, _P]),
    "pcs_bn_finalize_f32": (c_int32, [_P, c_double, _P, c_int32, c_double, c_double, _P, _P, _P, _P]),
    "pcs_bn_apply_f32": (c_int32, [_P, _P, _P, _P, _P, c_int64, c_int32, c_int32, _P, _P, c_int64, _P, c_int32, _P]),
    "pcs_bn_bwd_stats_f32": (c_int32, [_P, _P, _P, _P, _P, c_int64, c_int32, c_int32, _P, _P, c_int64, c_int64, _P]),
    "pcs_bn_bwd_apply_f32": (c_int32, [_P, _P, _P, _P, _P, _P, c_double, _P, _P, c_int64, c_int32, c_int32, _P, _P,
                                       c_int64, _P]),
    "pcs_bn_stats_h": (c_int32, [_P, c_int64, c_int32, c_int32, _P, _P, _P]),
    "pcs_bn_apply_h": (c_int32, [_P, _P, _P, _P, _P, c_int64, c_int32, c_int32, c_int32, _P, _P, c_int64, _P, c_int32, _P]),
    "pcs_bn_bwd_stats_h": (c_int32, [_P, _P, _P, _P, _P, c_int64, c_int32, c_int32, c_int32, _P, _P, c_int64, c_int64, _P]),
    "pcs_bn_bwd_apply_h": (c_int32, [_P, _P, _P, _P, _P, _P, c_double, _P, _P, c_int64, c_int32, c_int32, c_int32, _P, _P,
                                     c_int64, _P]),
    "pcs_quantize_floor": (c_int32, [_P, c_int32, c_int64, c_int32, _P, _P, _P, _P]),
    "pcs_quantize_keys": (c_int32, [_P, c_int64, _P, _P, _P]),
    "pcs_quantize_frame_keys": (c_int32, [_P, _P, c_int64, _P, _P, _P]),
    "pcs_quantize_flags": (c_int32, [_P, c_int64, _P, _P]),
    "pcs_quantize_emit": (c_int32, [_P, _P, _P, _P, c_int64, _P, _P, _P, _P]),
    "pcs_scan_transform_ws_bytes": (c_int64, [c_int64, c_int32, c_int32]),
    "pcs_scan_transform": (c_int32, [_P, c_int64, c_int32, _P, c_int32, _P, c_int32, c_float, _P, _P, _P, _P, c_int64, _P]),
    "pcs_scan_shift": (c_int32, [_P, c_int64, _P, c_int32, _P, c_int32, _P, _P]),
    "pcs_conv_h_applies": (c_int32, [c_int32, c_int32, c_int32]),
    "pcs_conv_prepared_weights_bytes": (c_size_t, [c_int32, c_int32, c_int32]),
    "pcs_conv_prepare_weights_h": (c_int32, [_P, c_int32, c_int32, c_int32, c_int32, c_int32, _P, _P]),
    "pcs_conv_gather_gemm_h": (c_int32, [_P, c_int64, c_int32, _P, c_int32, c_int32, _P, c_int32, _P, c_int32, c_int64,
                                         _P, _P, c_int32, _P, _P, _P]),
    "pcs_conv_gather_gemm_h_ex": (c_int32, [_P, c_int64, c_int32, _P, c_int32, c_int32, _P, c_int32, _P, c_int32, c_int64,
                                            _P, _P, _P, c_int32, _P, _P, _P]),
    "pcs_conv_x3_applies": (c_int32, [c_int32, c_int32, c_int32]),
    "pcs_conv_x3_column_tiles": (c_int32, [c_int32]),
    "pcs_conv_x3_emits_bn_partials": (c_int32, [c_int32, c_int32, c_int32, c_int32]),
    "pcs_conv_prepared_weights_x3_bytes": (c_size_t, [c_int32, c_int32, c_int32]),
    "pcs_conv_prepare_weights_x3": (c_int32, [_P, c_int32, c_int32, c_int32, c_int32, _P, _P]),
    "pcs_conv_gather_gemm_f32_bf16x3": (c_int32, [_P, c_int64, c_int32, _P, c_int32, c_int32, _P, c_int32, _P, c_int32, c_int64,
                                                  _P, _P, _P, _P, _P]),
    "pcs_conv_wgrad_f32_bf16x3": (c_int32, [_P, c_int32, _P, c_int32, _P, c_int32, _P, _P, c_int32, _P,
                                            _P, c_size_t, _P]),
    "pcs_conv_wgrad_h": (c_int32, [_P, c_int32, _P, c_int32, _P, c_int32, _P, _P, c_int32, _P, _P, c_size_t, c_int32, _P]),
    "pcs_unique_emit": (c_int32, [_P, _P, _P, _P, c_int64, _P, _P, _P, _P]),
    "pcs_cylinder_partition_f32": (c_int32, [_P, c_int64, c_int32, _P, _P, _P, _P, _P, _P, _P]),
    "pcs_cylinder_scan_batch_f32": (c_int32, [_P, c_int64, c_int32, _P, c_int32, _P, c_int32, _P, _P, _P, _P, _P, _P, _P]),
    "pcs_range_project_ws_bytes": (c_int64, [c_int32, c_int32, c_int32]),
    "pcs_range_project_f32": (c_int32, [_P, c_int64, c_int32, _P, _P, c_int32, c_int32, c_int32, _P, _P, _P, _P]),
    "pcs_range_image_fill_f32": (c_int32, [_P, _P, c_int64, c_int32, c_int32, c_int32, c_int32, _P, _P]),
    "pcs_range_scan_ws_bytes": (c_int64, [c_int32, c_int32, c_int32]),
    "pcs_range_scan_f32": (c_int32, [_P, c_int64, c_int32, _P, c_int32, _P, _P, c_int32, c_int32, c_int32, c_float, c_float, c_int32,
                                     _P, _P, _P, _P, _P, _P, _P, _P, _P, _P]),
    "pcs_range_knn_vote": (c_int32, [_P, _P, c_int32, c_int32, c_int32, _P, _P, _P, c_int64, _P, c_int32, c_int32, c_float, _P, c_int32,
                                     _P, _P, _P, _P]),
    "pcs_scan_mix_ws_bytes": (c_int64, [c_int64, c_int64, c_int32]),
    "pcs_scan_mix_count": (c_int32, [_P, c_int64, _P, _P, _P, c_int64, _P, c_int32, _P, _P, c_int32, _P, c_int64, _P, _P, _P]),
    "pcs_scan_mix_place": (c_int32, [_P, _P, c_int64, _P, _P, _P, c_int64, _P, c_int32, _P, _P, c_int32, _P, _P, c_int64, _P, _P, c_int64,
                                     c_int32, _P, _P, _P]),
    "pcs_scan_ring_ws_bytes": (c_int64, [c_int64]),
    "pcs_scan_ring_f32": (c_int32, [_P, c_int64, c_int32, _P, c_int32, _P, c_int64, _P]),
    "pcs_voxel_label_vote": (c_int32, [_P, _P, c_int64, c_int64, c_int32, c_int64, _P, _P, _P, _P]),
    "pcs_rows_argmax_gather_f32": (c_int32, [_P, c_int64, c_int32, _P, c_int64, _P, _P]),
    "pcs_predict_points_f32": (c_int32, [_P, c_int64, c_int32, _P, c_int64, _P, _P, c_int32, _P, _P, _P, _P, _P, _P]),
    "pcs_weights_multi_plan": (c_int64, [_P, c_int32]),
    "pcs_weights_multi": (c_int32, [_P, c_int32, c_int64, _P]),
    "pcs_step_plan": (c_int64, [_P, c_int32, _P]),
    "pcs_step_norm": (c_int32, [_P, c_int32, c_int64, c_float, _P, _P, c_double, c_double, c_int32, _P, c_int64, _P, _P]),
    "pcs_step_apply": (c_int32, [_P, c_int32, c_int64, _P, _P, c_int32, _P]),
    "pcs_lovasz_workspace_bytes": (c_int64, [c_int64, c_int32, c_int32, c_int64]),
    "pcs_lovasz_softmax_f32": (c_int32, [_P, _P, c_int64, c_int32, c_int32, c_int64, _P, _P, _P, c_int64, _P]),
    "pcs_debug_convh_ws": (None, [c_int32, c_int32, c_int32]),
    "pcs_debug_wgrad_interleave": (None, [c_int32]),
    "pcs_debug_conv_plan": (None, [c_int32] * 7 + [_P]),
    "pcs_debug_pointvoxel_h_inflight": (None, [c_int32]),
    "pcs_debug_cylscan_store": (None, [c_int32]),
}

class _WeightJob(ctypes.Structure):
    _fields_ = [("src", c_void_p), ("dst", c_void_p), ("K", c_int32), ("A", c_int32), ("B", c_int32), ("kind", c_int32),
                ("transpose", c_int32), ("nctt", c_int32), ("nt16", c_int32), ("ns", c_int32), ("first_block", c_int64)]


STEP_BLOCK_ELEMS = 4096
STEP_MAX_GROUPS = 8


class _StepJob(ctypes.Structure):
    _fields_ = [("p", c_void_p), ("g", c_void_p), ("buf", c_void_p), ("numel", c_int64), ("group", c_int32), ("reserved", c_int32),
                ("first_block", c_int64)]


class _StepHyper(ctypes.Structure):
    _fields_ = [("lr", c_float * STEP_MAX_GROUPS), ("wd", c_float * STEP_MAX_GROUPS), ("mu", c_float * STEP_MAX_GROUPS),
                ("nesterov", c_int32 * STEP_MAX_GROUPS), ("n_groups", c_int32)]


ABI_VERSION = 12
_lib = None


def lib_path():
    return _LIB_PATH


def load_library():
    global _lib
    if _lib is not None:
        return _lib
    if not os.path.exists(_LIB_PATH):
        raise RuntimeError(
            "openpcseg_amd: %s is missing -- build it with `python -m openpcseg_amd.build` "
            "(hipcc, gfx950). There is no CPU fallback." % _LIB_PATH)
    lib = ctypes.CDLL(_LIB_PATH)
    for name, (res, args) in SIGNATURES.items():
        fn = getattr(lib, name)
        fn.restype = res
        fn.argtypes = args
    if lib.pcs_abi_version() != ABI_VERSION:
        raise RuntimeError("openpcseg_amd: ABI version mismatch")
    _lib = lib
    return lib


def _check(rc, what):
    if rc != 0:
        msg = load_library().pcs_last_error()
        raise RuntimeError("openpcseg_amd: %s failed (%d): %s" % (what, rc, msg.decode() if msg else ""))


def _dev(t, name, dtype=None):
    if not isinstance(t, torch.Tensor) or not t.is_cuda:
        raise RuntimeError("openpcseg_amd: `%s` must be a HIP device tensor (got %s); the MI355X "
                           "backend has no CPU path" % (name, getattr(t, "device", type(t))))
    if dtype is not None and t.dtype != dtype:
        raise TypeError("openpcseg_amd: `%s` must be %s, got %s" % (name, dtype, t.dtype))
    return t if t.is_contiguous() else t.contiguous()


def _h2d(values, dtype, device):
    return torch.tensor(values, dtype=dtype, pin_memory=True).to(device, non_blocking=True)


def _ptr(t):
    return c_void_p(t.data_ptr()) if t is not None and t.numel() > 0 else c_void_p(0)


_raw_stream = getattr(torch._C, "_cuda_getCurrentRawStream", None)
_cur_device = getattr(torch._C, "_cuda_getDevice", None)


def _stream():
    if _raw_stream is not None and _cur_device is not None:
        return c_void_p(_raw_stream(_cur_device()))
    return c_void_p(torch.cuda.current_stream().cuda_stream)


def _cache_key(t):
    try:
        version = t._version
    except RuntimeError:
        _cache_key.uncached += 1
        return ("uncached", _cache_key.uncached)
    return (t.data_ptr(), tuple(t.shape), version)


_cache_key.uncached = 0


CACHE_STATS = {"hit": 0, "miss": 0, "cross": 0, "epoch": 0}


def _cached(holder, slot, extra, make):
    hit = getattr(holder, slot, None)
    if hit is not None and hit[0] == _cache_key(holder) + extra:
        CACHE_STATS["hit"] += 1
        if hit[2] != CACHE_STATS["epoch"]:
            CACHE_STATS["cross"] += 1
        return hit[1]
    CACHE_STATS["miss"] += 1
    return _cache_seed(holder, slot, extra, make())


def _cache_seed(holder, slot, extra, value):
    try:
        setattr(holder, slot, (_cache_key(holder) + extra, value, CACHE_STATS["epoch"]))
    except AttributeError:
        pass
    return value


def _vox_csr_memo(holder, m, n):
    return holder, "_pcs_vox_csr", (m, n)


def _sorted_csr(flat, m):
    vals, order = torch.sort(flat, stable=True)
    rowptr = torch.searchsorted(vals, torch.arange(m + 1, device=flat.device, dtype=vals.dtype))
    return order.contiguous(), rowptr.contiguous()


class HashTable:

    __slots__ = ("storage", "capacity", "n")

    def __init__(self, storage, capacity, n):
        self.storage, self.capacity, self.n = storage, capacity, n


_PPR_HINT = {}


class KernelMap:

    def __init__(self, pairs, koff, koff_host, nbsizes, n_src, n_dst, pending=None, hint_key=None):
        self._pairs_raw, self.koff, self.nbsizes = pairs, koff, nbsizes
        self.n_src, self.n_dst = n_src, n_dst
        self._koff_host, self._pending, self.hint_key = koff_host, pending, hint_key
        self.K = int(nbsizes.shape[0]) if koff_host is None else len(koff_host) - 1
        self._seg = {}
        self._koff_c_cache = None

    def _resolve(self):
        if self._koff_host is None:
            sizes, event = self._pending
            event.synchronize()
            ko = [0]
            for v in sizes.tolist():
                ko.append(ko[-1] + int(v))
            self._koff_host, self._pending = ko, None
            self._pairs_raw = self._pairs_raw[:ko[-1]].clone()
            if self.hint_key is not None and self.n_dst > 0:
                _PPR_HINT[self.hint_key] = ko[-1] / float(self.n_dst)
        return self._koff_host

    @property
    def resolved(self):
        return self._koff_host is not None

    @property
    def koff_host(self):
        return self._resolve()

    @property
    def pairs(self):
        self._resolve()
        return self._pairs_raw

    @property
    def _koff_c(self):
        if self._koff_c_cache is None:
            self._koff_c_cache = (c_int32 * (self.K + 1))(*self._resolve())
        return self._koff_c_cache

    @property
    def num_pairs(self):
        return self._resolve()[-1]

    def num_pairs_estimate(self):
        if self._koff_host is not None:
            return self._koff_host[-1]
        return int(_PPR_HINT.get(self.hint_key, 0.22 * self.K) * self.n_dst)

    def mirror(self):
        k, ko = self.K, self.koff_host
        pairs = torch.cat([self._pairs_raw[ko[k - 1 - j]:ko[k - j]] for j in range(k)], dim=0)
        koff_host = [0]
        for j in range(k):
            koff_host.append(koff_host[-1] + ko[k - j] - ko[k - 1 - j])
        koff = _h2d(koff_host, torch.int32, self._pairs_raw.device)
        return KernelMap(pairs, koff, koff_host, self.nbsizes.flip(0), self.n_dst, self.n_src)


class HipBackend:

    name = "hip-gfx950"

    def __init__(self):
        self.lib = load_library()

    def hash(self, coords):
        coords = _dev(coords, "coords", torch.int32)
        out = torch.empty(coords.shape[0], dtype=torch.int64, device=coords.device)
        _check(self.lib.pcs_hash(_ptr(coords), coords.shape[0], _ptr(out), _stream()), "pcs_hash")
        return out

    def kernel_hash(self, coords, offsets):
        coords = _dev(coords, "coords", torch.int32)
        offsets = _dev(offsets, "offsets", torch.int32)
        n, k = coords.shape[0], offsets.shape[0]
        out = torch.empty((k, n), dtype=torch.int64, device=coords.device)
        _check(self.lib.pcs_kernel_hash(_ptr(coords), n, _ptr(offsets), k, _ptr(out), _stream()),
               "pcs_kernel_hash")
        return out

    def table_build(self, keys):
        keys = _dev(keys, "references", torch.int64)
        n = keys.numel()
        cap = self.lib.pcs_hashtable_capacity(n)
        storage = torch.empty(self.lib.pcs_hashtable_bytes(cap), dtype=torch.uint8, device=keys.device)
        _check(self.lib.pcs_hashtable_build(_ptr(keys), n, _ptr(storage), cap, _stream()),
               "pcs_hashtable_build")
        return HashTable(storage, cap, n)

    def table_query(self, table, queries):
        queries = _dev(queries, "queries", torch.int64)
        out = torch.empty(queries.numel(), dtype=torch.int64, device=queries.device)
        _check(self.lib.pcs_hashtable_query(_ptr(table.storage), table.capacity, _ptr(queries),
                                            queries.numel(), _ptr(out), _stream()), "pcs_hashtable_query")
        return out

    def hash_query(self, queries, references):
        table = self.table_build(references)
        return self.table_query(table, queries.reshape(-1)) - 1

    def count(self, idx, num):
        idx = _dev(idx, "coords", torch.int32)
        out = torch.empty(int(num), dtype=torch.int32, device=idx.device)
        _check(self.lib.pcs_count(_ptr(idx), idx.numel(), _ptr(out), int(num), _stream()), "pcs_count")
        return out

    _CODE = {torch.float32: 0, torch.bfloat16: 1, torch.float16: 2}

    def _twin(self, stem, code, head, tail):
        name = stem + ("_h" if code else "_f32")
        _check(getattr(self.lib, name)(*head, *((code,) if code else ()), *tail), name)

    def _pv_feats(self, t, name):
        t = _dev(t, name)
        if t.dtype not in self._CODE:
            raise TypeError("openpcseg_amd: `%s` must be float32, bfloat16 or float16, got %s" % (name, t.dtype))
        return t, self._CODE[t.dtype]

    def voxelize_fwd(self, feats, idx, counts, cache_on=None):
        feats, code = self._pv_feats(feats, "feats")
        idx = _dev(idx, "coords", torch.int32)
        counts = _dev(counts, "counts", torch.int32)
        c = feats.shape[1]
        m = counts.shape[0]
        holder = cache_on if cache_on is not None else idx
        csr = _cached(*_vox_csr_memo(holder, m, idx.shape[0]), lambda: self._csr(idx, m))
        out = torch.empty((m, c), dtype=feats.dtype, device=feats.device)
        self._twin("pcs_voxelize_fwd_csr", code, [_ptr(feats), _ptr(csr[0]), _ptr(csr[1]), _ptr(counts), m, c], [_ptr(out), _stream()])
        return out

    def voxelize_fwd_atomic(self, feats, idx, counts):
        if isinstance(feats, torch.Tensor) and feats.dtype in self._HALF:
            raise TypeError("openpcseg_amd: voxelize_fwd_atomic is fp32 only (got %s); 16-bit rows take voxelize_fwd" % feats.dtype)
        feats = _dev(feats, "feats", torch.float32)
        idx = _dev(idx, "coords", torch.int32)
        counts = _dev(counts, "counts", torch.int32)
        n, c = feats.shape
        m = counts.shape[0]
        out = torch.empty((m, c), dtype=torch.float32, device=feats.device)
        _check(self.lib.pcs_voxelize_fwd_f32(_ptr(feats), _ptr(idx), _ptr(counts), n, m, c, _ptr(out),
                                             _stream()), "pcs_voxelize_fwd_f32")
        return out

    def voxelize_bwd(self, gout, idx, counts, n):
        gout, code = self._pv_feats(gout, "grad_output")
        c = gout.shape[1]
        gin = torch.empty((n, c), dtype=gout.dtype, device=gout.device)
        self._twin("pcs_voxelize_bwd", code, [_ptr(gout), _ptr(idx), _ptr(counts), n, c], [_ptr(gin), _stream()])
        return gin

    def devoxelize_fwd(self, feats, idx8, w8):
        feats, code = self._pv_feats(feats, "feats")
        idx8 = _dev(idx8, "coords", torch.int32)
        w8 = _dev(w8, "weights", torch.float32)
        n, c = idx8.shape[0], feats.shape[1]
        out = torch.empty((n, c), dtype=feats.dtype, device=feats.device)
        self._twin("pcs_devoxelize_fwd", code, [_ptr(feats), _ptr(idx8), _ptr(w8), n, c], [_ptr(out), _stream()])
        return out

    def _merge_operands(self, what, vox, idx8, w8, lin, stat, img=None, pxpy=None):
        vox, vcode = self._pv_feats(vox, "feats")
        lin, lcode = self._pv_feats(lin, "input")
        if vcode != lcode:
            if img is not None:
                raise TypeError("openpcseg_amd: %s takes vox and lin in one dtype, got %s and %s" % (what, vox.dtype, lin.dtype))
            vox, lin, vcode = vox.float(), lin.float(), 0
        idx8 = _dev(idx8, "coords", torch.int32)
        w8 = _dev(w8, "weights", torch.float32)
        n, c = lin.shape
        takes, got = "vox (m, c), lin (n, c), idx8 / w8 (n, 8)", [vox, lin, idx8, w8]
        ok = vox.dim() == 2 and vox.shape[1] == c and idx8.shape == (n, 8) and w8.shape == (n, 8)
        if img is not None:
            img = _dev(img, "feature_map", torch.float32)
            pxpy = _dev(pxpy, "pxpy", torch.float32)
            takes, got = takes + ", img (B, c, H, W), pxpy (n, 3)", got + [img, pxpy]
            ok = ok and img.dim() == 4 and img.shape[1] == c and pxpy.shape == (n, 3)
        if not ok:
            raise ValueError("openpcseg_amd: %s takes %s; got %s" % (what, takes, " ".join(str(tuple(t.shape)) for t in got)))
        out = torch.empty((n, c), dtype=lin.dtype, device=lin.device)
        mask = torch.empty((n, c // 32), dtype=torch.int32, device=lin.device) if stat is not None else None
        return vcode, vox, idx8, w8, lin, img, pxpy, out, mask

    def point_merge(self, vox, idx8, w8, lin, stat, gamma, beta):
        code, vox, idx8, w8, lin, _, _, out, mask = self._merge_operands("point_merge", vox, idx8, w8, lin, stat)
        n, c = lin.shape
        self._twin("pcs_point_merge", code, [_ptr(vox), _ptr(idx8), _ptr(w8), _ptr(lin), _ptr(stat), _ptr(gamma), _ptr(beta), n, c],
                   [_ptr(out), _ptr(mask), _stream()])
        return out, mask

    def range_point_merge(self, vox, idx8, w8, img, pxpy, lin, stat, gamma, beta):
        code, vox, idx8, w8, lin, img, pxpy, out, mask = self._merge_operands("range_point_merge", vox, idx8, w8, lin, stat, img, pxpy)
        if stat is None and (gamma is not None or beta is not None):
            raise ValueError("openpcseg_amd: range_point_merge in add mode (stat None) takes no gamma / beta")
        (n, c), (b, _, h, w) = lin.shape, img.shape
        self._twin("pcs_range_point_merge", code, [_ptr(vox), _ptr(idx8), _ptr(w8), _ptr(img), _ptr(pxpy), b, h, w, _ptr(lin),
                                                   _ptr(stat), _ptr(gamma), _ptr(beta), n, c], [_ptr(out), _ptr(mask), _stream()])
        return out, mask

    def devoxelize_bwd(self, gout, idx8, w8, m):
        gout, code = self._pv_feats(gout, "grad_output")
        n, c = gout.shape
        csr = self._index_csr(idx8, m)
        gfeat = torch.empty((m, c), dtype=gout.dtype, device=gout.device)
        if code:
            w8 = _dev(w8, "weights", torch.float32)
        self._twin("pcs_devoxelize_bwd_csr", code, [_ptr(gout), _ptr(csr[0]), _ptr(csr[1]), _ptr(w8), m, c], [_ptr(gfeat), _stream()])
        return gfeat

    def devoxelize_bwd_atomic(self, gout, idx8, w8, m):
        if isinstance(gout, torch.Tensor) and gout.dtype in self._HALF:
            raise TypeError("openpcseg_amd: devoxelize_bwd_atomic is fp32 only (got %s); 16-bit rows take devoxelize_bwd" % gout.dtype)
        gout = _dev(gout, "grad_output", torch.float32)
        n, c = gout.shape
        gfeat = torch.empty((m, c), dtype=torch.float32, device=gout.device)
        _check(self.lib.pcs_devoxelize_bwd_f32(_ptr(gout), _ptr(idx8), _ptr(w8), n, m, c, _ptr(gfeat),
                                               _stream()), "pcs_devoxelize_bwd_f32")
        return gfeat
# ... 217 lines not shown
        if src.shape[1] != cin:
            raise ValueError("Input feature size and kernel size mismatch")
        return self._conv_launch(self.lib.pcs_conv_gather_gemm_f32_ex, src, weight, k, cin, cout, kmap, bias, tile_rows, bn_sums, ordered,
                                 bn_raw, addend, act_slope, relu, post_scale=post_scale, post_shift=post_shift)

    _HALF = {torch.bfloat16: 1, torch.float16: 2}

    def conv_h_applies(self, cin, cout, k):
        return bool(self.lib.pcs_conv_h_applies(int(cin), int(cout), int(k)))

    def prepare_weights_h(self, weight, dtype, transpose):
        weight = _dev(weight, "weight", torch.float32)
        k, a, b = weight.shape
        con, cols = (b, a) if transpose else (a, b)
        nbytes = self.lib.pcs_conv_prepared_weights_bytes(k, con, cols)
        if nbytes == 0:
            raise RuntimeError("openpcseg_amd: shape (%d, %d, %d) is not served by the half-precision kernels" % (k, a, b))
        wp = torch.empty(nbytes, dtype=torch.uint8, device=weight.device)
        _check(self.lib.pcs_conv_prepare_weights_h(_ptr(weight), k, a, b, int(bool(transpose)), self._HALF[dtype], _ptr(wp),
                                                   _stream()), "pcs_conv_prepare_weights_h")
        wp._pcs_prepared = ("half", dtype, k, con, cols)
        return wp

    def conv_gather_gemm_h(self, src, wp, k, cout, kmap, bias=None, tile_rows=None, bn_sums=None, ordered=True, bn_raw=False,
                           addend=None, act_slope=None, relu=False, post_scale=None, post_shift=None):
        if src.dtype not in self._HALF:
            raise TypeError("openpcseg_amd: conv_gather_gemm_h wants bfloat16 / float16 features, got %s" % src.dtype)
        src = _dev(src, "input")
        cin = src.shape[1]
        meta = getattr(wp, "_pcs_prepared", None)
        if meta is not None and meta != ("half", src.dtype, k, cin, cout):
            raise ValueError("openpcseg_amd: prepared weights %s do not match this call (%s)" % (meta, ("half", src.dtype, k, cin, cout)))
        return self._conv_launch(self.lib.pcs_conv_gather_gemm_h_ex, src, wp, k, cin, cout, kmap, bias, tile_rows, bn_sums, ordered, bn_raw,
                                 addend, act_slope, relu, code=self._HALF[src.dtype], post_scale=post_scale, post_shift=post_shift)

    def conv_x3_applies(self, cin, cout, k):
        return bool(self.lib.pcs_conv_x3_applies(int(cin), int(cout), int(k)))

    def prepare_weights_x3(self, weight, transpose):
        weight = _dev(weight, "weight", torch.float32)
        k, a, b = weight.shape
        con, cols = (b, a) if transpose else (a, b)
        nbytes = self.lib.pcs_conv_prepared_weights_x3_bytes(k, con, cols)
        if nbytes == 0 or not self.conv_x3_applies(con, cols, k):
            raise RuntimeError("openpcseg_amd: shape (%d, %d, %d) is not served by the bf16x3 kernel" % (k, a, b))
        wp = torch.empty(nbytes, dtype=torch.uint8, device=weight.device)
        _check(self.lib.pcs_conv_prepare_weights_x3(_ptr(weight), k, a, b, int(bool(transpose)), _ptr(wp), _stream()),
               "pcs_conv_prepare_weights_x3")
        wp._pcs_prepared = ("x3", k, con, cols)
        return wp

    def conv_gather_gemm_x3(self, src, wp, k, cout, kmap, bias=None, tile_rows=None, bn_sums=None, ordered=True, bn_raw=False):
        src = _dev(src, "input", torch.float32)
        cin = src.shape[1]
        meta = getattr(wp, "_pcs_prepared", None)
        if meta is not None and meta != ("x3", k, cin, cout):
            raise ValueError("openpcseg_amd: prepared weights %s do not match this call (%s)" % (meta, ("x3", k, cin, cout)))
        return self._conv_launch(self.lib.pcs_conv_gather_gemm_f32_bf16x3, src, wp, k, cin, cout, kmap, bias, tile_rows, bn_sums, ordered,
                                 bn_raw, x3=True)

    def conv_wgrad_h(self, fa, fb, kmap, a_col):
        if fa.dtype not in self._HALF or fb.dtype != fa.dtype:
            raise TypeError("openpcseg_amd: conv_wgrad_h wants two tensors of the same half dtype")
        return self._wgrad_launch(self.lib.pcs_conv_wgrad_h, _dev(fa, "input"), _dev(fb, "grad_output"), kmap, a_col,
                                  self._HALF[fa.dtype])

    def transpose_weights(self, w):
        w = _dev(w, "weight", torch.float32)
        k, a, b = w.shape
        out = torch.empty((k, b, a), dtype=torch.float32, device=w.device)
        _check(self.lib.pcs_transpose_kab_f32(_ptr(w), k, a, b, _ptr(out), _stream()), "pcs_transpose_kab_f32")
        return out

    def prepared_weights_buffer(self, weight, kind, transpose):
        k, a, b = weight.shape
        if kind == "t":
            return torch.empty((k, b, a), dtype=torch.float32, device=weight.device)
        con, cols = (b, a) if transpose else (a, b)
        nbytes = self.lib.pcs_conv_prepared_weights_bytes(k, con, cols)
        if nbytes == 0:
            raise RuntimeError("openpcseg_amd: shape (%d, %d, %d) is not served by the half-precision kernels" % (k, a, b))
        wp = torch.empty(nbytes, dtype=torch.uint8, device=weight.device)
        wp._pcs_prepared = ("half", kind, k, con, cols)
        return wp

    def weights_multi(self, jobs):
        if not jobs:
            return
        arr = (_WeightJob * len(jobs))()
        sig = []
        for j, (w, dst, kind, tr) in zip(arr, jobs):
            w = _dev(w, "weight", torch.float32)
            if not w.is_contiguous() or w.dim() != 3:
                raise ValueError("openpcseg_amd: weights_multi wants contiguous (K, A, B) weights")
            j.src, j.dst = w.data_ptr(), dst.data_ptr()
            j.K, j.A, j.B = w.shape
            j.kind = 0 if kind == "t" else self._HALF[kind]
            j.transpose = int(bool(tr))
            sig.append((j.src, j.dst, j.K, j.A, j.B, j.kind, j.transpose))
        sig = (tuple(sig), str(jobs[0][0].device))
        hit = getattr(self, "_wm_table", None)
        if hit is None or hit[0] != sig:
            blocks = self.lib.pcs_weights_multi_plan(ctypes.byref(arr), len(jobs))
            if blocks < 0:
                _check(-1, "pcs_weights_multi_plan")
            host = torch.frombuffer(bytearray(bytes(arr)), dtype=torch.uint8).pin_memory()
            hit = (sig, host.to(jobs[0][0].device, non_blocking=True), int(blocks), host)
            self._wm_table = hit
        _check(self.lib.pcs_weights_multi(_ptr(hit[1]), len(jobs), hit[2], _stream()), "pcs_weights_multi")

    def step_tail(self, cache, jobs, hyper, record=None, max_norm=None, scaler=None):
        if not jobs:
            return
        if not 1 <= len(hyper) <= STEP_MAX_GROUPS:
            raise ValueError("openpcseg_amd: step_tail takes 1 .. %d groups" % STEP_MAX_GROUPS)
        hy = _StepHyper()
        hy.n_groups = len(hyper)
        for i, (lr, wd, mu, nesterov) in enumerate(hyper):
            hy.lr[i], hy.wd[i], hy.mu[i], hy.nesterov[i] = lr, wd, mu, int(bool(nesterov))
        dev = jobs[0][0].device
        sig = (tuple((p.data_ptr(), g.data_ptr(), 0 if b is None else b.data_ptr(), p.numel(), grp) for p, g, b, grp in jobs),
               tuple(h[2] != 0 for h in hyper), str(dev))
        hit = cache.get("table")
        if hit is None or hit[0] != sig:
            arr = (_StepJob * len(jobs))()
            for j, (pp, gp, bp, n, grp) in zip(arr, sig[0]):
                j.p, j.g, j.buf, j.numel, j.group = pp or None, gp or None, bp or None, n, grp
            blocks = self.lib.pcs_step_plan(ctypes.byref(arr), len(jobs), ctypes.byref(hy))
            if blocks < 0:
                _check(-1, "pcs_step_plan")
            host = torch.frombuffer(bytearray(bytes(arr)), dtype=torch.uint8).pin_memory()
            ws = cache.get("ws")
            if ws is None or ws.numel() < 16 + 12 * blocks or ws.device != dev:
                ws = torch.zeros(16 + 12 * int(blocks), dtype=torch.uint8, device=dev)
                cache["ws"] = ws
            hit = (sig, host.to(dev, non_blocking=True), int(blocks), host)
            cache["table"] = hit
        table, blocks = hit[1], hit[2]
        if blocks == 0:
            return
        if record is not None:
            ws = cache["ws"]
            scale, tracker, growth, backoff, interval = scaler if scaler is not None else (None, None, 1.0, 1.0, 0)
            _check(self.lib.pcs_step_norm(_ptr(table), len(jobs), blocks, -1.0 if max_norm is None else float(max_norm), _ptr(scale),
                                          _ptr(tracker), float(growth), float(backoff), int(interval), _ptr(ws), ws.numel(),
                                          _ptr(record), _stream()), "pcs_step_norm")
        _check(self.lib.pcs_step_apply(_ptr(table), len(jobs), blocks, ctypes.byref(hy), _ptr(record),
                                       int(scaler is not None), _stream()), "pcs_step_apply")

    def conv_wgrad(self, fa, fb, kmap, a_col, split=False):
        fn = self.lib.pcs_conv_wgrad_f32_bf16x3 if split else self.lib.pcs_conv_wgrad_f32
        return self._wgrad_launch(fn, _dev(fa, "input", torch.float32), _dev(fb, "grad_output", torch.float32), kmap, a_col)

    def _wgrad_launch(self, fn, fa, fb, kmap, a_col, *tail):
        ca, cb = fa.shape[1], fb.shape[1]
        gw = torch.empty((kmap.K, ca, cb), dtype=torch.float32, device=fa.device)
        ws_bytes = self.lib.pcs_conv_wgrad_ws_bytes(kmap._koff_c, kmap.K, ca, cb)
        ws = torch.empty(max(ws_bytes, 4), dtype=torch.uint8, device=fa.device)
        _check(fn(_ptr(fa), ca, _ptr(fb), cb, _ptr(kmap.pairs), a_col, _ptr(kmap.koff), kmap._koff_c, kmap.K, _ptr(gw),
                  _ptr(ws), ws_bytes, *tail, _stream()), "pcs_conv_wgrad_h" if tail else "pcs_conv_wgrad_f32")
        return gw

    def _csr(self, index, m):
        flat = index.reshape(-1)
        if not (flat.is_cuda and flat.dtype == torch.int32 and os.environ.get("PCS_INDEX_CSR", "1") != "0"):
            return _sorted_csr(flat, m)
        flat = flat if flat.is_contiguous() else flat.contiguous()
        n = flat.numel()
        order = torch.empty(n, dtype=torch.int64, device=flat.device)
        rowptr = torch.empty(m + 1, dtype=torch.int64, device=flat.device)
        ws_bytes = self.lib.pcs_index_csr_ws_bytes(n, m)
        ws = torch.empty(max(ws_bytes, 1), dtype=torch.uint8, device=flat.device)
        _check(self.lib.pcs_index_csr_i32(_ptr(flat), n, m, _ptr(order), _ptr(rowptr), _ptr(ws), ws_bytes, _stream()),
               "pcs_index_csr_i32")
        return order, rowptr

    def _index_csr(self, index, m):
        return _cached(index, "_pcs_csr", (m,), lambda: self._csr(index, m))

    def scatter_max_fwd(self, src, index, m):
        src = _dev(src, "src", torch.float32)
        index = _dev(index, "index", torch.int64)
        c = src.shape[1]
        order, rowptr = self._index_csr(index, m)
        out = torch.empty((m, c), dtype=torch.float32, device=src.device)
        arg = torch.empty((m, c), dtype=torch.int32, device=src.device)
        _check(self.lib.pcs_scatter_max_fwd_f32(_ptr(src), _ptr(order), _ptr(rowptr), m, c, _ptr(out), _ptr(arg),
                                                _stream()), "pcs_scatter_max_fwd_f32")
        return out, arg

    def scatter_max_bwd(self, gout, arg, n):
        gout = _dev(gout, "grad_output", torch.float32)
        m, c = gout.shape
        gsrc = torch.empty((n, c), dtype=torch.float32, device=gout.device)
        _check(self.lib.pcs_scatter_max_bwd_f32(_ptr(gout), _ptr(arg), m, n, c, _ptr(gsrc), _stream()),
               "pcs_scatter_max_bwd_f32")
        return gsrc

    def map_count(self, pxpy, b, h, w):
        pxpy = _dev(pxpy, "pxpy", torch.int32)
        out = torch.empty((b, h, w), dtype=torch.int32, device=pxpy.device)
        _check(self.lib.pcs_map_count(_ptr(pxpy), pxpy.shape[0], b, h, w, _ptr(out), _stream()), "pcs_map_count")
        return out

    def _pixel_csr(self, pxpy, b, h, w):
        def make():
            pb, px, py = pxpy[:, 0].long(), pxpy[:, 1].long(), pxpy[:, 2].long()
            ok = (pb >= 0) & (pb < b) & (px >= 0) & (px < w) & (py >= 0) & (py < h)
            return self._csr(torch.where(ok, (pb * h + py) * w + px, torch.full_like(pb, -1)), b * h * w)
        return _cached(pxpy, "_pcs_px_csr", (b, h, w), make)

    def denselize_fwd(self, feat, count_map, pxpy):
        feat = _dev(feat, "feat", torch.float32)
        count_map = _dev(count_map, "count_map", torch.int32)
        pxpy = _dev(pxpy, "pxpy", torch.int32)
        (b, h, w), c = count_map.shape, feat.shape[1]
        if c % 4:
            return self.denselize_fwd_atomic(feat, count_map, pxpy)
        csr = self._pixel_csr(pxpy, b, h, w)
        out = torch.empty((b, c, h, w), dtype=torch.float32, device=feat.device)
        _check(self.lib.pcs_denselize_fwd_csr_f32(_ptr(feat), _ptr(csr[0]), _ptr(csr[1]), _ptr(count_map), b, c, h, w,
                                                  _ptr(out), _stream()), "pcs_denselize_fwd_csr_f32")
        return out

    def denselize_fwd_atomic(self, feat, count_map, pxpy):
        feat = _dev(feat, "feat", torch.float32)
        count_map = _dev(count_map, "count_map", torch.int32)
        pxpy = _dev(pxpy, "pxpy", torch.int32)
        (b, h, w), c = count_map.shape, feat.shape[1]
        out = torch.empty((b, c, h, w), dtype=torch.float32, device=feat.device)
        _check(self.lib.pcs_denselize_fwd_f32(_ptr(feat), _ptr(count_map), _ptr(pxpy), feat.shape[0], b, c, h, w,
                                              _ptr(out), _stream()), "pcs_denselize_fwd_f32")
        return out

    def denselize_bwd(self, gout, count_map, pxpy):
        gout = _dev(gout, "top_grad", torch.float32)
        b, c, h, w = gout.shape
        n = pxpy.shape[0]
        gfeat = torch.empty((n, c), dtype=torch.float32, device=gout.device)
        if c % 4:
            return self.denselize_bwd_gather(gout, count_map, pxpy)
        csr = self._pixel_csr(pxpy, b, h, w)
        _check(self.lib.pcs_denselize_bwd_csr_f32(_ptr(gout), _ptr(csr[0]), _ptr(csr[1]), _ptr(count_map), n, b, c, h, w,
                                                  _ptr(gfeat), _stream()), "pcs_denselize_bwd_csr_f32")
        return gfeat

    def denselize_bwd_gather(self, gout, count_map, pxpy):
        gout = _dev(gout, "top_grad", torch.float32)
        b, c, h, w = gout.shape
        n = pxpy.shape[0]
        gfeat = torch.empty((n, c), dtype=torch.float32, device=gout.device)
        _check(self.lib.pcs_denselize_bwd_f32(_ptr(gout), _ptr(count_map), _ptr(pxpy), n, b, c, h, w, _ptr(gfeat),
                                              _stream()), "pcs_denselize_bwd_f32")
        return gfeat

    def range_sample_fwd(self, img, pxpy):
        img = _dev(img, "feature_map", torch.float32)
        pxpy = _dev(pxpy, "pxpy", torch.float32)
        b, c, h, w = img.shape
        n = pxpy.shape[0]
        out = torch.empty((n, c), dtype=torch.float32, device=img.device)
        _check(self.lib.pcs_range_sample_fwd_f32(_ptr(img), _ptr(pxpy), n, b, c, h, w, _ptr(out), _stream()), "pcs_range_sample_fwd_f32")
        return out

    def _corner_csr(self, pxpy, b, h, w):
        def make():
            n = pxpy.shape[0]
            keys = torch.empty(4 * n, dtype=torch.int64, device=pxpy.device)
            wts = torch.empty(4 * n, dtype=torch.float32, device=pxpy.device)
            _check(self.lib.pcs_range_sample_corners(_ptr(pxpy), n, b, h, w, _ptr(keys), _ptr(wts), _stream()), "pcs_range_sample_corners")
            return self._csr(keys, b * h * w) + (wts,)
        return _cached(pxpy, "_pcs_corner_csr", (b, h, w), make)

    def range_sample_bwd(self, gout, pxpy, b, h, w):
        gout = _dev(gout, "grad_output", torch.float32)
        pxpy = _dev(pxpy, "pxpy", torch.float32)
        c = gout.shape[1]
        order, rowptr, wts = self._corner_csr(pxpy, b, h, w)
        gimg = torch.empty((b, c, h, w), dtype=torch.float32, device=gout.device)
        _check(self.lib.pcs_range_sample_bwd_csr_f32(_ptr(gout), _ptr(order), _ptr(rowptr), _ptr(wts), b, c, h, w, _ptr(gimg),
                                                     _stream()), "pcs_range_sample_bwd_csr_f32")
        return gimg

    @staticmethod
    def _feat(t, name, like=None):
        t = _dev(t, name)
        if t.dtype not in HipBackend._CODE:
            raise TypeError("openpcseg_amd: `%s` must be float32 / bfloat16 / float16, got %s" % (name, t.dtype))
        if like is not None and t.dtype != like.dtype:
            t = t.to(like.dtype)
        return t

    def bn_stats(self, x):
        x = self._feat(x, "input")
        n, c = x.shape
        ws = torch.empty(self.lib.pcs_bn_num_partials() * 2 * c, dtype=torch.float32, device=x.device)
        sums = torch.empty(2 * c + 1, dtype=torch.float64, device=x.device)
        self._twin("pcs_bn_stats", self._CODE[x.dtype], [_ptr(x), n, c], [_ptr(ws), _ptr(sums), _stream()])
        return sums

    def bn_finalize(self, sums, count, eps, momentum, running_mean, running_var, count_dev=None):
        c = sums.numel() // 2
        stat = torch.empty(2 * c, dtype=torch.float64, device=sums.device)
        _check(self.lib.pcs_bn_finalize_f32(_ptr(sums), float(count), _ptr(count_dev), c, float(eps), float(momentum),
                                            _ptr(running_mean), _ptr(running_var), _ptr(stat), _stream()), "pcs_bn_finalize_f32")
        return stat

    def bn_apply(self, x, res, stat, w, b, relu, want_mask=False, tail=None):
        x = self._feat(x, "input")
        res = self._feat(res, "residual", x) if res is not None else None
        tail = self._feat(tail, "tail", x) if tail is not None else None
        n, c = x.shape
        ct = tail.shape[1] if tail is not None else 0
        if want_mask and c % 32:
            raise RuntimeError("openpcseg_amd: the ReLU bit mask needs a channel count that is a multiple of 32")
        if tail is not None and (tail.shape[0] != n or c % 4 or ct % 4):
            raise RuntimeError("openpcseg_amd: concat fusion needs equal row counts and channel counts that are multiples of 4")
        y = torch.empty((n, c + ct), dtype=x.dtype, device=x.device)
        mask = torch.empty((n, c // 32), dtype=torch.int32, device=x.device) if want_mask else None
        self._twin("pcs_bn_apply", self._CODE[x.dtype], [_ptr(x), _ptr(res), _ptr(stat), _ptr(w), _ptr(b), n, c, int(relu)],
                   [_ptr(y), _ptr(mask), c + ct, _ptr(tail), ct, _stream()])
        return (y, mask) if want_mask else y

    @staticmethod
    def _gate(gate, relu):
        if not relu or gate is None:
            return None, None
        return (None, _ptr(gate)) if gate.dtype == torch.int32 else (_ptr(gate), None)

    @staticmethod
    def _rows(t, name, like, c):
        if not isinstance(t, torch.Tensor) or not t.is_cuda:
            raise RuntimeError("openpcseg_amd: `%s` must be a HIP device tensor" % name)
        if t.dtype != like.dtype:
            t = t.to(like.dtype)
        unit = 16 // t.element_size() if t.dtype == torch.float32 else 4
        ok = t.dim() == 2 and t.stride(1) == 1 and t.stride(0) >= c and t.stride(0) % 4 == 0 and \
            t.data_ptr() % (unit * t.element_size()) == 0
        if not ok:
            t = t.contiguous()
        return t, t.stride(0)

    def bn_bwd_stats(self, dy, x, gate, stat, relu):
        x = self._feat(x, "input")
        n, c = x.shape
        dy, lddy = self._rows(dy, "grad_output", x, c)
        ws = torch.empty(self.lib.pcs_bn_num_partials() * 2 * c, dtype=torch.float32, device=x.device)
        buf = torch.empty(3 * c, dtype=torch.float64, device=x.device)
        sums2 = buf[:2 * c]
        sums2._pcs_f32 = buf[2 * c:].view(torch.float32)
        yp, mp = self._gate(gate, relu)
        self._twin("pcs_bn_bwd_stats", self._CODE[x.dtype], [_ptr(dy), _ptr(x), yp, mp, _ptr(stat), n, c, int(relu)],
                   [_ptr(ws), _ptr(sums2), buf.numel(), lddy, _stream()])
        return sums2

    def bn_bwd_apply(self, dy, x, gate, stat, sums2, count, w, relu, want_res, count_dev=None, in_slope=None):
        x = self._feat(x, "input")
        n, c = x.shape
        dy, lddy = self._rows(dy, "grad_output", x, c)
        dx = torch.empty_like(x)
        dres = torch.empty_like(x) if want_res else None
        yp, mp = self._gate(gate, relu)
        if in_slope is not None and float(in_slope) != 1.0:
            _check(self.lib.pcs_bn_bwd_apply_act(_ptr(dy), _ptr(x), yp, mp, _ptr(stat), _ptr(sums2), float(count), _ptr(count_dev),
                                                 _ptr(w), n, c, int(relu), self._CODE[x.dtype], float(in_slope),
                                                 _ptr(dx), _ptr(dres), lddy, _stream()), "pcs_bn_bwd_apply_act")
            return dx, dres
        self._twin("pcs_bn_bwd_apply", self._CODE[x.dtype],
                   [_ptr(dy), _ptr(x), yp, mp, _ptr(stat), _ptr(sums2), float(count), _ptr(count_dev), _ptr(w), n, c, int(relu)],
                   [_ptr(dx), _ptr(dres), lddy, _stream()])
        return dx, dres

    def _recon_rows(self, tensors):
        ts = [self._feat(t, "input") for t in tensors]
        dt = ts[0].dtype if all(t.dtype == ts[0].dtype for t in ts) else torch.float32
        ts = [(t if t.dtype == dt else t.to(dt)).contiguous() for t in ts]
        if any(t.dim() != 2 or t.shape != ts[0].shape for t in ts):
            raise ValueError("openpcseg_amd: the recon gate takes (n, c) tensors of one shape, got %s" % [tuple(t.shape) for t in ts])
        return ts, self._CODE[dt]

    def recon_gate(self, a3, x, stat3, gamma3, beta3):
        (a0, a1, a2, x), code = self._recon_rows(list(a3) + [x])
        n, c = x.shape
        out = torch.empty_like(x)
        self._twin("pcs_recon_gate", code, [_ptr(a0), _ptr(a1), _ptr(a2), _ptr(x), _ptr(stat3), _ptr(gamma3), _ptr(beta3), n, c],
                   [_ptr(out), _stream()])
        return out

    def recon_gate_bwd_stats(self, dy, x, a3, stat3, gamma3, beta3):
        (dy, x, a0, a1, a2), code = self._recon_rows([dy, x] + list(a3))
        n, c = x.shape
        buf = torch.empty(9 * c, dtype=torch.float64, device=x.device) if n > 0 else \
            torch.zeros(9 * c, dtype=torch.float64, device=x.device)
        ws = torch.empty(self.lib.pcs_bn_num_partials() * 6 * c, dtype=torch.float32, device=x.device)
        sums2 = buf[:6 * c]
        sums2._pcs_f32 = buf[6 * c:].view(torch.float32)
        self._twin("pcs_recon_gate_bwd_stats", code,
                   [_ptr(dy), _ptr(x), _ptr(a0), _ptr(a1), _ptr(a2), _ptr(stat3), _ptr(gamma3), _ptr(beta3), n, c],
                   [_ptr(ws), _ptr(sums2), buf.numel(), _stream()])
        return sums2

    def recon_gate_bwd_apply(self, dy, x, a3, stat3, gamma3, beta3, sums2, count, count_dev=None):
        (dy, x, a0, a1, a2), code = self._recon_rows([dy, x] + list(a3))
        n, c = x.shape
        dx = torch.empty_like(x)
        da = [torch.empty_like(x) for _ in range(3)]
        self._twin("pcs_recon_gate_bwd_apply", code,
                   [_ptr(dy), _ptr(x), _ptr(a0), _ptr(a1), _ptr(a2), _ptr(stat3), _ptr(gamma3), _ptr(beta3), _ptr(sums2), float(count),
                    _ptr(count_dev), n, c], [_ptr(dx), _ptr(da[0]), _ptr(da[1]), _ptr(da[2]), _stream()])
        return dx, da

    def quantize(self, points, voxel_size3, want_index, want_inverse):
        points = _dev(points, "coords")
        if points.dim() != 2 or points.shape[1] != 3:
            raise ValueError("sparse_quantize: coords must be (n, 3), got %s" % (tuple(points.shape),))
        if points.dtype not in (torch.float32, torch.float64, torch.int32):
            points = points.float() if points.is_floating_point() else points.int()
        points = points.contiguous()
        kind = 2 if points.dtype == torch.float64 else int(points.is_floating_point())
        n, stride = points.shape
        dev = points.device
        vox_size = (c_double * 3)(*[float(v) for v in voxel_size3])
        coords = torch.empty((n, 3), dtype=torch.int32, device=dev)
        i32 = torch.iinfo(torch.int32)
        bbox = _h2d([i32.max] * 3 + [i32.min] * 3, torch.int32, dev)
        _check(self.lib.pcs_quantize_floor(_ptr(points), kind, n, stride, vox_size,
                                           _ptr(coords), _ptr(bbox), _stream()), "pcs_quantize_floor")
        keys = torch.empty(n, dtype=torch.int64, device=dev)
        _check(self.lib.pcs_quantize_keys(_ptr(coords), n, _ptr(bbox), _ptr(keys), _stream()), "pcs_quantize_keys")
        return self._voxel_emit(keys, coords, want_index, want_inverse)

    def _run_heads(self, skeys):
        flags = torch.empty(skeys.numel(), dtype=torch.int32, device=skeys.device)
        _check(self.lib.pcs_quantize_flags(_ptr(skeys), skeys.numel(), _ptr(flags), _stream()), "pcs_quantize_flags")
        return flags

    def _run_emit(self, entry, flags, rank, perm, src, *outs):
        _check(getattr(self.lib, entry)(_ptr(flags), _ptr(rank), _ptr(perm), _ptr(src), flags.numel(), *[_ptr(o) for o in outs],
                                        _stream()), entry)

    def _sorted_runs(self, keys):
        if keys.numel() == 0:
            e = torch.empty(0, dtype=torch.int64, device=keys.device)
            return e, e, torch.empty(0, dtype=torch.int32, device=keys.device), e, 0
        skeys, perm = torch.sort(keys, stable=True)
        flags = self._run_heads(skeys)
        rank = torch.cumsum(flags, dim=0, dtype=torch.int64)
        return skeys, perm, flags, rank, int(rank[-1].item())

    def _voxel_emit(self, keys, coords, want_index, want_inverse):
        _, perm, flags, rank, m = self._sorted_runs(keys)
        n, dev = keys.numel(), keys.device
        vox = torch.empty((m, 3), dtype=torch.int32, device=dev)
        index = torch.empty(m, dtype=torch.int64, device=dev) if want_index else None
        inverse = torch.empty(n, dtype=torch.int64, device=dev) if want_inverse else None
        self._run_emit("pcs_quantize_emit", flags, rank, perm, coords, vox, index, inverse)
        return vox, index, inverse

    def quantize_frame_keys(self, coords, frames):
        coords = _dev(coords, "coords", torch.int32)
        frames = _dev(frames, "frames", torch.int64)
        n = coords.shape[0]
        keys = torch.empty(n, dtype=torch.int64, device=coords.device)
        if n == 0:
            return keys
        bbox = torch.cat([coords.amin(0), coords.amax(0)]).contiguous()
        _check(self.lib.pcs_quantize_frame_keys(_ptr(coords), _ptr(frames), n, _ptr(bbox), _ptr(keys), _stream()), "pcs_quantize_frame_keys")
        return keys

    def quantize_sorted_keys(self, keys, coords, frames):
        keys = _dev(keys, "keys", torch.int64)
        coords = _dev(coords, "coords", torch.int32)
        vox, index, inverse = self._voxel_emit(keys, coords, True, True)
        return torch.cat([vox, frames[index].int()[:, None]], dim=1), index, inverse

    MAX_VOTES, MAX_COLUMNS = 16, 8

    def _scan_args(self, what, points, offsets, params, votes):
        import numpy as np
        points = _dev(points, "points", torch.float32)
        if points.dim() != 2:
            raise ValueError("openpcseg_amd: %s wants (n, C) points, got %s" % (what, tuple(points.shape)))
        n, c = points.shape
        nf, v = len(offsets) - 1, int(votes)
        params = np.ascontiguousarray(params, dtype=np.float64)
        if nf < 1 or params.shape != (v * nf, 8):
            raise ValueError("openpcseg_amd: %s wants (votes * num_frames, 8) parameters, got %s for %d votes of %d frames"
                             % (what, params.shape, v, nf))
        table = _h2d(params.reshape(-1).view(np.int64).tolist() + [int(o) for o in offsets], torch.int64, points.device)
        return points, n, c, nf, v, table[:v * nf * 8].view(torch.float64), table[v * nf * 8:]

    def scan_transform(self, points, offsets, params, votes, voxel_size):
        points, n, c, nf, v, par, off = self._scan_args("scan_transform", points, offsets, params, votes)
        dev = points.device
        feats = torch.empty((v * n, c), dtype=torch.float32, device=dev)
        coords = torch.empty((v * n, 3), dtype=torch.int32, device=dev)
        mins = torch.empty((v * nf, 3), dtype=torch.int32, device=dev)
        ws_bytes = self.lib.pcs_scan_transform_ws_bytes(n, nf, v)
        if ws_bytes < 0:
            _check(-1, "pcs_scan_transform_ws_bytes")
        ws = torch.empty(max(int(ws_bytes), 4), dtype=torch.uint8, device=dev)
        _check(self.lib.pcs_scan_transform(_ptr(points), n, c, _ptr(off), nf, _ptr(par), v, float(voxel_size), _ptr(feats), _ptr(coords),
                                           _ptr(mins), _ptr(ws), ws.numel(), _stream()), "pcs_scan_transform")
        return feats, coords, mins, off

    def scan_shift(self, coords, mins, frame_offsets, votes):
        coords = _dev(coords, "coords", torch.int32)
        mins = _dev(mins, "mins", torch.int32)
        frame_offsets = _dev(frame_offsets, "frame_offsets", torch.int64)
        v, nf = int(votes), frame_offsets.numel() - 1
        if v < 1 or coords.shape[0] % v or mins.numel() != v * nf * 3:
            raise ValueError("openpcseg_amd: scan_shift wants votes * n coordinate rows and votes * num_frames minima")
        n = coords.shape[0] // v
        frames = torch.empty(v * n, dtype=torch.int64, device=coords.device)
        _check(self.lib.pcs_scan_shift(_ptr(coords), n, _ptr(frame_offsets), nf, _ptr(mins), v, _ptr(frames), _stream()),
               "pcs_scan_shift")
        return frames

    def unique_inverse_csr(self, keys):
        keys = _dev(keys, "keys", torch.int64)
        skeys, perm, flags, rank, m = self._sorted_runs(keys)
        n, dev = keys.numel(), keys.device
        uniq = torch.empty(m, dtype=torch.int64, device=dev)
# ... 271 lines not shown
```

Measured before the change: 105.9 frames/s.

## Defer fp32 weight-grad launches and run BN backward blocks inside them

The fp32 wgrad2 launch is now deferred and recorded per stream instead of being issued right away. The next BN backward stats or apply pass on that stream is fused into the pending wgrad kernel as extra 'rider' blocks, together with a slice of the remaining wgrad tiles. The goal is to overlap the bandwidth-bound BN backward work with the compute-bound weight-gradient GEMM, instead of running them back to back. A cost model gates when the two are combined, and Python-side bookkeeping keeps tensors alive and flushes pending work at the end of backward. This adds global mutable state, lifetime hazards and more launch complexity, and the path only applies when the weight grad is unset and no hooks or distributed training are present.

```diff
diff --git a/include/pcseg_hip.h b/include/pcseg_hip.h
--- a/include/pcseg_hip.h
+++ b/include/pcseg_hip.h
@@ -132,6 +132,12 @@
                        const int32_t *pairs, int32_t a_col, const int32_t *koff_dev,
                        const int32_t *koff_host, int32_t K, float *gW, void *ws,
                        size_t ws_bytes, void *stream);
+
+int pcs_conv_wgrad_f32_defer(const float *fa, int32_t ca, const float *fb, int32_t cb, const int32_t *pairs, int32_t a_col,
+                             const int32_t *koff_dev, const int32_t *koff_host, int32_t K, float *gW, void *ws, size_t ws_bytes,
+                             void *stream);
+int pcs_conv_wgrad_flush(void *stream);
+int32_t pcs_conv_wgrad_pending(void *stream);
 
 int pcs_scatter_max_fwd_f32(const float *src, const int64_t *order, const int64_t *rowptr, int64_t m,
                             int32_t c, float *out, int32_t *arg, void *stream);
@@ -351,6 +357,7 @@
 void pcs_debug_conv_plan(int32_t kind, int32_t dtype, int32_t cin, int32_t cout, int32_t K, int32_t tile_rows, int32_t flags,
                          int32_t out[12]);
 void pcs_debug_wgrad_interleave(int32_t mode);
+void pcs_debug_wgrad_ride(int32_t mode, int32_t riders);
 void pcs_debug_cylscan_store(int32_t form);
 
 #ifdef __cplusplus
diff --git a/openpcseg_amd/csrc/bn_rows.h b/openpcseg_amd/csrc/bn_rows.h
--- /dev/null
+++ b/openpcseg_amd/csrc/bn_rows.h
@@ -0,0 +1,159 @@
+#pragma once
+#include "row_storage.h"
+
+namespace pcs {
+
+template <int V> struct NV;
+template <> struct NV<4> { using T = float4; };
+template <> struct NV<1> { using T = float; };
+template <int V, typename ET> __device__ __forceinline__ typename NV<V>::T ldv(ET, const void *p, int64_t e) {
+  const Acc<V> a = widen(ET{}, *reinterpret_cast<const typename Raw<ET, V>::T *>(reinterpret_cast<const typename Elem<ET>::T *>(p) + e));
+  if constexpr (V == 4) return make_float4(a.f[0], a.f[1], a.f[2], a.f[3]);
+  else return a.f[0];
+}
+template <typename ET> __device__ __forceinline__ void stv(ET, void *p, int64_t e, const float4 &v) {
+  *reinterpret_cast<typename Raw<ET, 4>::T *>(reinterpret_cast<typename Elem<ET>::T *>(p) + e) = narrow(ET{}, Acc<4>{{v.x, v.y, v.z, v.w}});
+}
+template <typename ET> __device__ __forceinline__ void stv(ET, void *p, int64_t e, const float &v) {
+  reinterpret_cast<typename Elem<ET>::T *>(p)[e] = narrow(ET{}, Acc<1>{{v}});
+}
+
+__device__ __forceinline__ float comp(const float4 &v, int i) { return i == 0 ? v.x : (i == 1 ? v.y : (i == 2 ? v.z : v.w)); }
+__device__ __forceinline__ float comp(const float &v, int) { return v; }
+__device__ __forceinline__ void setc(float4 &v, int i, float s) { if (i == 0) v.x = s; else if (i == 1) v.y = s; else if (i == 2) v.z = s; else v.w = s; }
+__device__ __forceinline__ void setc(float &v, int, float s) { v = s; }
+
+template <bool BWD, int V, typename ET, bool GUARD = false>
+__device__ __forceinline__ void bn_partial_rows(const void *__restrict__ x, const void *__restrict__ dy,
+                                                const void *__restrict__ y, const uint32_t *__restrict__ mask,
+                                                const double *__restrict__ stat, int64_t n, int c, int cv, int relu,
+                                                float *__restrict__ partial, int64_t lddy, unsigned vb, unsigned vgrid, unsigned utx, unsigned uty,
+                                                unsigned uTX, unsigned uTY) {
+  using VT = typename NV<V>::T;
+  extern __shared__ float red[];
+  const int tx = utx, ty = uty, TX = uTX, TY = uTY;
+  const int W = TX * V;
+  const bool live = !GUARD || ty < TY;
+  for (int j0 = 0; j0 < cv; j0 += TX) {
+    const int j = j0 + tx;
+    float s0[V], s1[V];
+#pragma unroll
+    for (int q = 0; q < V; ++q) { s0[q] = 0.f; s1[q] = 0.f; }
+    if (j < cv && live) {
+      float mean[V], invstd[V];
+#pragma unroll
+      for (int q = 0; q < V; ++q) {
+        mean[q] = BWD ? (float)stat[j * V + q] : (n > 0 ? ldv<1>(ET{}, x, j * V + q) : 0.f);
+        invstd[q] = BWD ? (float)stat[c + j * V + q] : 0.f;
+        if (!BWD && vb == 0 && ty == 0) partial[(int64_t)vgrid * 2 * c + j * V + q] = mean[q];
+      }
+#pragma unroll 4
+      for (int64_t i = (int64_t)vb * TY + ty; i < n; i += (int64_t)vgrid * TY) {
+        const VT xv = ldv<V>(ET{}, x, i * c + (int64_t)j * V);
+        if (BWD) {
+          const VT gv = ldv<V>(ET{}, dy, i * lddy + (int64_t)j * V);
+          VT yv; unsigned bits = 0xFu;
+          if (relu) {
+            if (V == 4 && mask) bits = (mask[i * (c >> 5) + (j >> 3)] >> (4 * (j & 7))) & 0xFu;
+            else yv = ldv<V>(ET{}, y, i * c + (int64_t)j * V);
+          }
+#pragma unroll
+          for (int q = 0; q < V; ++q) {
+            float g = comp(gv, q);
+            if (relu && ((V == 4 && mask) ? !((bits >> q) & 1u) : comp(yv, q) <= 0.f)) g = 0.f;
+            s0[q] += g;
+            s1[q] += g * ((comp(xv, q) - mean[q]) * invstd[q]);
+          }
+        } else {
+#pragma unroll
+          for (int q = 0; q < V; ++q) { const float t = comp(xv, q) - mean[q]; s0[q] += t; s1[q] += t * t; }
+        }
+      }
+    }
+    if (live) {
+#pragma unroll
+      for (int q = 0; q < V; ++q) {
+        red[(ty * 2 + 0) * W + tx * V + q] = s0[q];
+        red[(ty * 2 + 1) * W + tx * V + q] = s1[q];
+      }
+    }
+    __syncthreads();
+    if (ty == 0 && j < cv) {
+#pragma unroll
+      for (int q = 0; q < V; ++q) {
+        float a = 0.f, b = 0.f;
+        for (int r = 0; r < TY; ++r) { a += red[(r * 2 + 0) * W + tx * V + q]; b += red[(r * 2 + 1) * W + tx * V + q]; }
+        partial[((int64_t)vb * 2 + 0) * c + j * V + q] = a;
+        partial[((int64_t)vb * 2 + 1) * c + j * V + q] = b;
+      }
+    }
+    __syncthreads();
+  }
+}
+
+template <int V, typename ET>
+__device__ __forceinline__ void bn_bwd_apply_rows(const void *__restrict__ dy, const void *__restrict__ x,
+                                                  const void *__restrict__ y, const uint32_t *__restrict__ mask,
+                                                  const double *__restrict__ stat, const double *__restrict__ sums2,
+                                                  double count, const double *__restrict__ count_dev,
+                                                  const float *__restrict__ w, int64_t n, int c, int cv, int relu,
+                                                  void *__restrict__ dx, void *__restrict__ dres, int64_t lddy,
+                                                  float in_slope, unsigned vb, unsigned vgrid, unsigned tx, unsigned ty, unsigned TX,
+                                                  unsigned TY) {
+  using VT = typename NV<V>::T;
+  if (count_dev) count = *count_dev;
+  if (!(count > 0.0)) count = 1.0;
+  for (int j = tx; j < cv; j += TX) {
+    float mean[V], invstd[V], k1[V], k2[V], ws[V];
+#pragma unroll
+    for (int q = 0; q < V; ++q) {
+      const int ch = j * V + q;
+      mean[q] = (float)stat[ch]; invstd[q] = (float)stat[c + ch];
+      k1[q] = (float)(sums2[ch] / count);
+      k2[q] = (float)(sums2[c + ch] / count);
+      ws[q] = invstd[q] * (w ? w[ch] : 1.f);
+    }
+#pragma unroll 4
+    for (int64_t i = (int64_t)vb * TY + ty; i < n; i += (int64_t)vgrid * TY) {
+      const VT gv = ldv<V>(ET{}, dy, i * lddy + (int64_t)j * V);
+      const VT xv = ldv<V>(ET{}, x, i * c + (int64_t)j * V);
+      VT yv; unsigned bits = 0xFu;
+      if (relu) {
+        if (V == 4 && mask) bits = (mask[i * (c >> 5) + (j >> 3)] >> (4 * (j & 7))) & 0xFu;
+        else yv = ldv<V>(ET{}, y, i * c + (int64_t)j * V);
+      }
+      VT o, r;
+#pragma unroll
+      for (int q = 0; q < V; ++q) {
+        float g = comp(gv, q);
+        if (relu && ((V == 4 && mask) ? !((bits >> q) & 1u) : comp(yv, q) <= 0.f)) g = 0.f;
+        const float xh = (comp(xv, q) - mean[q]) * invstd[q];
+        float d = (g - k1[q] - xh * k2[q]) * ws[q];
+        if (in_slope != 1.f && !(comp(xv, q) > 0.f)) d *= in_slope;
+        setc(o, q, d);
+        setc(r, q, g);
+      }
+      stv(ET{}, dx, i * c + (int64_t)j * V, o);
+      if (dres) stv(ET{}, dres, i * c + (int64_t)j * V, r);
+    }
+  }
+}
+
+struct BnRide {
+  int pass;
+  int v, tx, ty;
+  const void *dy, *x, *y;
+  const uint32_t *mask;
+  const double *stat;
+  int64_t n, lddy;
+  int c, cv, relu;
+  float *partial;
+  const double *sums2;
+  double count;
+  const double *count_dev;
+  const float *w;
+  void *dx, *dres;
+};
+int wgrad_ride_try(hipStream_t st, const BnRide &r);
+
+}
diff --git a/openpcseg_amd/csrc/conv_wgrad.hip b/openpcseg_amd/csrc/conv_wgrad.hip
--- a/openpcseg_amd/csrc/conv_wgrad.hip
+++ b/openpcseg_amd/csrc/conv_wgrad.hip
@@ -1,4 +1,9 @@
 #include "conv_common.h"
+#include "bn_rows.h"
+
+#include <map>
+#include <mutex>
+#include <utility>
 
 using namespace pcs;
 
@@ -402,13 +407,13 @@
 }
 
 template <typename ET>
-__global__ void __launch_bounds__(256, 3) wgrad2_kernel(Wgrad2Args w) {
+__device__ __forceinline__ void wgrad2_tile(const Wgrad2Args &w, int pos, int by) {
   const int tid = threadIdx.x, lane = tid & 63, wid = tid >> 6;
   int beg, end, gsid;
-  find_split_wave(w.koff, w.K, w.pch, blockIdx.x, lane, &beg, &end, &gsid, w.interleave);
+  find_split_wave(w.koff, w.K, w.pch, pos, lane, &beg, &end, &gsid, w.interleave);
   const int nag = wg_ngroups(w.ca);
   const int nsb = (w.nbg + 1) >> 1;
-  const int sa = blockIdx.y / nsb, sb = blockIdx.y - sa * nsb;
+  const int sa = by / nsb, sb = by - sa * nsb;
   const int ag = 2 * sa + (wid >> 1), bg = 2 * sb + (wid & 1);
   if (beg >= end || ag >= nag || bg >= w.nbg) return;
   const int aw = wg_gwidth(w.ca), bw = wg_gwidth(w.cb);
@@ -420,6 +425,35 @@
   PCS_WG_CASE(32, 64) PCS_WG_CASE(32, 48) PCS_WG_CASE(32, 32) PCS_WG_CASE(32, 16)
   PCS_WG_CASE(16, 64) PCS_WG_CASE(16, 48) PCS_WG_CASE(16, 32) PCS_WG_CASE(16, 16)
 #undef PCS_WG_CASE
+}
+
+template <typename ET>
+__global__ void __launch_bounds__(256, 3) wgrad2_kernel(Wgrad2Args w) {
+  wgrad2_tile<ET>(w, (int)blockIdx.x, (int)blockIdx.y);
+}
+
+template <int V>
+__device__ __forceinline__ void bn_rider(const BnRide &r, unsigned rider, unsigned riders) {
+  const unsigned tid = threadIdx.x, tx = tid % (unsigned)r.tx, ty = tid / (unsigned)r.tx;
+  if (r.pass == 1) {
+    for (unsigned vb = rider; vb < (unsigned)kStatBlocks; vb += riders)
+      bn_partial_rows<true, V, Fp32, true>(r.x, r.dy, r.y, r.mask, r.stat, r.n, r.c, r.cv, r.relu, r.partial, r.lddy,
+                                           vb, (unsigned)kStatBlocks, (int)tx, (int)ty, r.tx, r.ty);
+  } else if (ty < (unsigned)r.ty) {
+    bn_bwd_apply_rows<V, Fp32>(r.dy, r.x, r.y, r.mask, r.stat, r.sums2, r.count, r.count_dev, r.w, r.n, r.c, r.cv, r.relu, r.dx,
+                               r.dres, r.lddy, 1.f, rider, riders, tx, ty, (unsigned)r.tx, (unsigned)r.ty);
+  }
+}
+
+template <typename ET>
+__global__ void __launch_bounds__(256, 3) wgrad2_ride_kernel(Wgrad2Args w, int s0, int riders, BnRide r) {
+  if ((int)blockIdx.x < riders) {
+    if (blockIdx.y != 0) return;
+    if (r.v == 4) bn_rider<4>(r, blockIdx.x, (unsigned)riders);
+    else bn_rider<1>(r, blockIdx.x, (unsigned)riders);
+    return;
+  }
+  wgrad2_tile<ET>(w, s0 + (int)blockIdx.x - riders, (int)blockIdx.y);
 }
 
 constexpr int W3_PB = 32;
@@ -718,6 +752,94 @@
   return PCS_EINVAL;
 }
 
+struct WgradRideEnv { int mode, riders; };
+const WgradRideEnv &wgrad_ride_env() {
+  auto num = [](const char *v, int dflt) { return v ? atoi(v) : dflt; };
+  static const WgradRideEnv env = {num(getenv("PCS_WGRAD_RIDE"), 1), num(getenv("PCS_WGRAD_RIDERS"), 0)};
+  return env;
+}
+int g_wgrad_ride = -1, g_wgrad_riders = 0;
+int wgrad_ride_mode() { return g_wgrad_ride >= 0 ? g_wgrad_ride : wgrad_ride_env().mode; }
+
+constexpr double kRideWgradFlops = 100e12;
+constexpr double kRideBnBytes = 5.3e12;
+constexpr int kRideRiders = 256;
+bool wgrad_ride_route(double pairs, int ca, int cb, double pass_bytes) {
+  const int mode = wgrad_ride_mode();
+  if (mode == 0) return false;
+  if (mode == 2) return true;
+  return 2.0 * pairs * ca * cb / kRideWgradFlops >= pass_bytes / kRideBnBytes;
+}
+
+struct WgradPending {
+  Wgrad2Args w;
+  int K, pch, nx, nsy;
+  int64_t cc, pairs;
+  float *gW;
+  const float *ws;
+  int next;
+};
+std::mutex g_pending_mu;
+std::map<std::pair<int, hipStream_t>, WgradPending> g_pending;
+std::pair<int, hipStream_t> pending_key(hipStream_t st) {
+  int dev = 0;
+  (void)hipGetDevice(&dev);
+  return {dev, st};
+}
+
+int wgrad_launch_range(const WgradPending &pd, int s0, int s1, const BnRide *r, int riders, hipStream_t st) {
+  if (!r) riders = 0;
+  if (s1 - s0 + riders <= 0) return PCS_OK;
+  if (!r && s0 == 0 && s1 == pd.nx) {
+    hipLaunchKernelGGL(wgrad2_kernel<Fp32>, dim3((unsigned)pd.nx, (unsigned)pd.nsy), dim3(256), 0, st, pd.w);
+    return check_launch("pcs_conv_wgrad_f32");
+  }
+  BnRide none = {};
+  const size_t lds = r && r->pass == 1 ? (size_t)r->ty * 2 * r->tx * r->v * sizeof(float) : 0;
+  hipLaunchKernelGGL(wgrad2_ride_kernel<Fp32>, dim3((unsigned)(riders + s1 - s0), (unsigned)pd.nsy), dim3(256), lds, st, pd.w, s0, riders,
+                     r ? *r : none);
+  return check_launch("pcs_conv_wgrad_f32(ride)");
+}
+
+int wgrad_launch_reduce4(const WgradPending &pd, hipStream_t st) {
+  hipLaunchKernelGGL(wgrad_reduce4_kernel, dim3((unsigned)ceil_div(pd.cc, 64), pd.K), dim3(256), 0, st, pd.ws, pd.w.koff, pd.K, pd.pch,
+                     pd.cc, pd.gW);
+  return check_launch("pcs_conv_wgrad_f32(reduce)");
+}
+
+int wgrad_flush(hipStream_t st) {
+  std::lock_guard<std::mutex> lock(g_pending_mu);
+  auto it = g_pending.find(pending_key(st));
+  if (it == g_pending.end()) return PCS_OK;
+  const WgradPending pd = it->second;
+  g_pending.erase(it);
+  const int rc = wgrad_launch_range(pd, pd.next, pd.nx, nullptr, 0, st);
+  return rc ? rc : wgrad_launch_reduce4(pd, st);
+}
+
+}
+
+int pcs::wgrad_ride_try(hipStream_t st, const BnRide &r) {
+  std::lock_guard<std::mutex> lock(g_pending_mu);
+  auto it = g_pending.find(pending_key(st));
+  if (it == g_pending.end()) return 0;
+  WgradPending &pd = it->second;
+  const int rem = pd.nx - pd.next;
+  const int carry = r.pass == 1 && rem >= 2 ? std::min(std::max(rem * 4 / 11, 1), rem - 1) : rem;
+  const double rows = (double)r.n * r.c;
+  const double gate = !r.relu ? 0.0 : (r.mask ? rows / 8 : rows * 4);
+  const double bytes = (r.pass == 1 ? 2.0 : (r.dres ? 4.0 : 3.0)) * rows * 4 + gate;
+  if (!wgrad_ride_route((double)pd.pairs * carry / pd.nx, pd.w.ca, pd.w.cb, bytes)) return 0;
+  const int riders = g_wgrad_riders > 0 ? g_wgrad_riders : (wgrad_ride_env().riders > 0 ? wgrad_ride_env().riders : kRideRiders);
+  int rc = wgrad_launch_range(pd, pd.next, pd.next + carry, &r, riders, st);
+  if (rc) { g_pending.erase(it); return rc; }
+  pd.next += carry;
+  if (pd.next >= pd.nx) {
+    rc = wgrad_launch_reduce4(pd, st);
+    g_pending.erase(it);
+    if (rc) return rc;
+  }
+  return 1;
 }
 
 extern "C" size_t pcs_conv_wgrad_ws_bytes(const int32_t *koff_host, int32_t K, int32_t ca, int32_t cb) {
@@ -733,7 +855,7 @@
 
 static int conv_wgrad_any(const void *fa, int32_t ca, const void *fb, int32_t cb, const int32_t *pairs, int32_t a_col,
                           const int32_t *koff_dev, const int32_t *koff_host, int32_t K, float *gW, void *ws, size_t ws_bytes,
-                          int dtype, void *stream, bool force_split = false) {
+                          int dtype, void *stream, bool force_split = false, int32_t *defer = nullptr) {
   if (ca <= 0 || cb <= 0 || K <= 0 || !koff_dev || !koff_host || !gW || (a_col != 0 && a_col != 1) || dtype < 0 || dtype > 2) {
     set_error("pcs_conv_wgrad_f32: bad args");
     return PCS_EINVAL;
@@ -756,6 +878,14 @@
     case WgradFamily::wgrad2: {
       Wgrad2Args w = wgrad_args<Wgrad2Args>(fa, fb, pairs, koff_dev, ws, ca, cb, K, a_col, p.pch);
       w.nbg = wg_ngroups(cb); w.interleave = p.interleave;
+      if (defer && dtype == 0 && wgrad_ride_mode() != 0 && (((uintptr_t)ws | (uintptr_t)gW) & 15) == 0) {
+        WgradPending pd = {w, (int)K, p.pch, (int)p.grid.x, (int)p.grid.y, cc, (int64_t)koff_host[K] - koff_host[0], gW,
+                           reinterpret_cast<const float *>(ws), 0};
+        std::lock_guard<std::mutex> lock(g_pending_mu);
+        g_pending[pending_key(st)] = pd;
+        *defer = 1;
+        return PCS_OK;
+      }
       if (dtype == 0) hipLaunchKernelGGL(wgrad2_kernel<Fp32>, p.grid, dim3(256), 0, st, w);
       else if (dtype == 1) hipLaunchKernelGGL(wgrad2_kernel<Bf16>, p.grid, dim3(256), 0, st, w);
       else hipLaunchKernelGGL(wgrad2_kernel<Fp16>, p.grid, dim3(256), 0, st, w);
@@ -810,3 +940,23 @@
   if ((ca % 4) || (cb % 4) || (((uintptr_t)fa | (uintptr_t)fb) & 15)) { set_error("pcs_conv_wgrad_f32_bf16x3: needs 16-byte granular rows"); return PCS_EUNSUPPORTED; }
   return conv_wgrad_any(fa, ca, fb, cb, pairs, a_col, koff_dev, koff_host, K, gW, ws, ws_bytes, 0, stream, true);
 }
+
+extern "C" int pcs_conv_wgrad_f32_defer(const float *fa, int32_t ca, const float *fb, int32_t cb, const int32_t *pairs, int32_t a_col,
+                                        const int32_t *koff_dev, const int32_t *koff_host, int32_t K, float *gW, void *ws,
+                                        size_t ws_bytes, void *stream) {
+  int rc = wgrad_flush(as_stream(stream));
+  if (rc) return rc;
+  int32_t deferred = 0;
+  rc = conv_wgrad_any(fa, ca, fb, cb, pairs, a_col, koff_dev, koff_host, K, gW, ws, ws_bytes, 0, stream, false, &deferred);
+  return rc ? rc : deferred;
+}
+
+extern "C" int pcs_conv_wgrad_flush(void *stream) { return wgrad_flush(as_stream(stream)); }
+
+extern "C" int32_t pcs_conv_wgrad_pending(void *stream) {
+  std::lock_guard<std::mutex> lock(g_pending_mu);
+  auto it = g_pending.find(pending_key(as_stream(stream)));
+  return it == g_pending.end() ? 0 : it->second.nx - it->second.next;
+}
+
+extern "C" void pcs_debug_wgrad_ride(int32_t mode, int32_t riders) { g_wgrad_ride = mode; g_wgrad_riders = riders; }
diff --git a/openpcseg_amd/csrc/norm.hip b/openpcseg_amd/csrc/norm.hip
--- a/openpcseg_amd/csrc/norm.hip
+++ b/openpcseg_amd/csrc/norm.hip
@@ -1,29 +1,8 @@
-#include "row_storage.h"
+#include "bn_rows.h"
 
 using namespace pcs;
 
 namespace {
-
-template <int V> struct NV;
-template <> struct NV<4> { using T = float4; };
-template <> struct NV<1> { using T = float; };
-template <int V, typename ET> __device__ __forceinline__ typename NV<V>::T ldv(ET, const void *p, int64_t e) {
-  const Acc<V> a = widen(ET{}, *reinterpret_cast<const typename Raw<ET, V>::T *>(reinterpret_cast<const typename Elem<ET>::T *>(p) + e));
-  if constexpr (V == 4) return make_float4(a.f[0], a.f[1], a.f[2], a.f[3]);
-  else return a.f[0];
-}
-template <typename ET> __device__ __forceinline__ void stv(ET, void *p, int64_t e, const float4 &v) {
-  *reinterpret_cast<typename Raw<ET, 4>::T *>(reinterpret_cast<typename Elem<ET>::T *>(p) + e) = narrow(ET{}, Acc<4>{{v.x, v.y, v.z, v.w}});
-}
-template <typename ET> __device__ __forceinline__ void stv(ET, void *p, int64_t e, const float &v) {
-  reinterpret_cast<typename Elem<ET>::T *>(p)[e] = narrow(ET{}, Acc<1>{{v}});
-}
-
-__device__ __forceinline__ float comp(const float4 &v, int i) { return i == 0 ? v.x : (i == 1 ? v.y : (i == 2 ? v.z : v.w)); }
-__device__ __forceinline__ float comp(const float &v, int) { return v; }
-__device__ __forceinline__ void setc(float4 &v, int i, float s) { if (i == 0) v.x = s; else if (i == 1) v.y = s; else if (i == 2) v.z = s; else v.w = s; }
-__device__ __forceinline__ void setc(float &v, int, float s) { v = s; }
-
 
 template <bool BWD, int V, typename ET>
 __global__ void __launch_bounds__(256) bn_partial_kernel(const void *__restrict__ x, const void *__restrict__ dy,
@@ -280,7 +259,8 @@
 static bool al_v4(int dtype, const void *p) { return aligned(p, dtype == 0 ? 16 : 8); }
 
 static int bn_partial(bool bwd, int dtype, const void *x, const void *dy, const void *y, const uint32_t *mask, const double *stat,
-                      int64_t n, int c, int relu, float *partial, double *sums, hipStream_t st, int64_t lddy = 0) {
+                      int64_t n, int c, int relu, float *partial, double *sums, hipStream_t st, int64_t lddy = 0,
+                      bool may_ride = false) {
   if (lddy == 0) lddy = c;
   if (lddy < c) { set_error("pcs_bn: row stride of dy smaller than c"); return PCS_EINVAL; }
   const bool vec = (c & 3) == 0 && (lddy & 3) == 0 && al_v4(dtype, x) && al_v4(dtype, dy) && al_v4(dtype, y);
@@ -288,7 +268,17 @@
   const int V = vec ? 4 : 1, cv = c / V;
   const dim3 block = row_launch(n, cv, kRowsExact4).block;
   const size_t lds = (size_t)block.y * 2 * block.x * V * sizeof(float);
-  if (vec) {
+  int rode = 0;
+  if (may_ride && bwd && dtype == 0 && n > 0) {
+    BnRide r = {};
+    r.pass = 1; r.v = V; r.tx = (int)block.x; r.ty = (int)block.y;
+    r.dy = dy; r.x = x; r.y = y; r.mask = mask; r.stat = stat; r.n = n; r.lddy = lddy; r.c = c; r.cv = cv; r.relu = relu;
+    r.partial = partial;
+    rode = wgrad_ride_try(st, r);
+    if (rode < 0) return rode;
+  }
+  if (rode) {
+  } else if (vec) {
     if (bwd) PCS_DTYPE(dtype, hipLaunchKernelGGL((bn_partial_kernel<true, 4, ET>), dim3(kStatBlocks), block, lds, st, x, dy, y, mask, stat, n, c, cv, relu, partial, lddy));
     else PCS_DTYPE(dtype, hipLaunchKernelGGL((bn_partial_kernel<false, 4, ET>), dim3(kStatBlocks), block, lds, st, x, dy, y, mask, stat, n, c, cv, relu, partial, lddy));
   } else {
@@ -327,7 +317,7 @@
 static int bn_bwd_apply_any(int dtype, const void *dy, const void *x, const void *y, const uint32_t *mask,
                             const double *stat, const double *sums2, double count, const double *count_dev,
                             const float *w, int64_t n, int32_t c, int32_t relu, void *dx, void *dres, int64_t lddy,
-                            void *stream, float in_slope = 1.f) {
+                            void *stream, float in_slope = 1.f, bool may_ride = false) {
   if (n < 0 || c <= 0) { set_error("pcs_bn_bwd_apply: bad sizes"); return PCS_EINVAL; }
   if (n == 0) return PCS_OK;
   if (!count_dev && !(count > 0)) { set_error("pcs_bn_bwd_apply: count must be positive"); return PCS_EINVAL; }
@@ -337,6 +327,15 @@
   hipStream_t st = as_stream(stream);
   const bool vec = (c & 3) == 0 && (lddy & 3) == 0 && al_v4(dtype, dy) && al_v4(dtype, x) && al_v4(dtype, y) && al_v4(dtype, dx) && al_v4(dtype, dres);
   if (mask && (!vec || (c & 31))) { set_error("pcs_bn_bwd_apply: the ReLU bit mask needs c % 32 == 0 and aligned rows"); return PCS_EUNSUPPORTED; }
+  if (may_ride && dtype == 0) {
+    const RowLaunch g = vec ? geo<4>(n, c) : geo<1>(n, c);
+    BnRide r = {};
+    r.pass = 2; r.v = vec ? 4 : 1; r.tx = (int)g.block.x; r.ty = (int)g.block.y;
+    r.dy = dy; r.x = x; r.y = y; r.mask = mask; r.stat = stat; r.n = n; r.lddy = lddy; r.c = c; r.cv = g.cv; r.relu = relu;
+    r.sums2 = sums2; r.count = count; r.count_dev = count_dev; r.w = w; r.dx = dx; r.dres = dres;
+    const int rode = wgrad_ride_try(st, r);
+    if (rode) return rode < 0 ? rode : PCS_OK;
+  }
   if (vec) {
     const RowLaunch g = geo<4>(n, c);
     PCS_DTYPE(dtype, hipLaunchKernelGGL((bn_bwd_apply_kernel<4, ET>), g.grid, g.block, 0, st, dy, x, y, mask, stat, sums2, count, count_dev, w, n, c, g.cv, relu, dx, dres, lddy, in_slope));
@@ -402,7 +401,7 @@
                                     double *sums2, int64_t sums2_doubles, int64_t lddy, void *stream) {
   if (n < 0 || c <= 0 || (n > 0 && (!dy || !x || (relu && !y && !mask))) || !stat || !partial_ws || !sums2) { set_error("pcs_bn_bwd_stats: bad args"); return PCS_EINVAL; }
   if (sums2_doubles < 3 * (int64_t)c) { set_error("pcs_bn_bwd_stats: sums2 must hold 3c doubles (2c sums + the same 2c values as floats)"); return PCS_EWORKSPACE; }
-  return bn_partial(true, 0, x, dy, y, mask, stat, n, c, relu, partial_ws, sums2, as_stream(stream), lddy);
+  return bn_partial(true, 0, x, dy, y, mask, stat, n, c, relu, partial_ws, sums2, as_stream(stream), lddy, true);
 }
 extern "C" int pcs_bn_bwd_stats_h(const void *dy, const void *x, const void *y, const uint32_t *mask,
                                   const double *stat, int64_t n, int32_t c, int32_t relu, int32_t dtype, float *partial_ws,
@@ -416,7 +415,7 @@
                                     const double *stat, const double *sums2, double count, const double *count_dev,
                                     const float *w, int64_t n, int32_t c, int32_t relu, float *dx, float *dres,
                                     int64_t lddy, void *stream) {
-  return bn_bwd_apply_any(0, dy, x, y, mask, stat, sums2, count, count_dev, w, n, c, relu, dx, dres, lddy, stream);
+  return bn_bwd_apply_any(0, dy, x, y, mask, stat, sums2, count, count_dev, w, n, c, relu, dx, dres, lddy, stream, 1.f, true);
 }
 extern "C" int pcs_bn_bwd_apply_act(const void *dy, const void *x, const void *y, const uint32_t *mask,
                                     const double *stat, const double *sums2, double count, const double *count_dev,
diff --git a/openpcseg_amd/functional.py b/openpcseg_amd/functional.py
--- a/openpcseg_amd/functional.py
+++ b/openpcseg_amd/functional.py
@@ -201,6 +201,28 @@
 
 def get_conv_policy():
     return _CONV_POLICY["mode"]
+
+
+_WGRAD_RIDE_POLICY = {"mode": "off"}
+
+
+def set_wgrad_ride_policy(mode):
+    if mode not in ("auto", "off"):
+        raise ValueError("wgrad ride policy must be 'auto' or 'off'")
+    _WGRAD_RIDE_POLICY["mode"] = mode
+
+
+def get_wgrad_ride_policy():
+    return _WGRAD_RIDE_POLICY["mode"]
+
+
+def _wgrad_may_defer(be, x, dy, weight, hd, split=False):
+    return (_WGRAD_RIDE_POLICY["mode"] == "auto" and not split and hd is None and hasattr(be, "conv_wgrad_defer")
+            and x.is_cuda and x.dtype == torch.float32 and dy.dtype == torch.float32 and weight.dtype == torch.float32
+            and weight.grad is None and not getattr(weight, "_backward_hooks", None)
+            and not getattr(weight, "_post_accumulate_grad_hooks", None)
+            and not torch.is_grad_enabled()
+            and not (torch.distributed.is_available() and torch.distributed.is_initialized()))
 
 
 def _wgrad_split(cin, cout):
@@ -415,17 +437,22 @@
             grad_input = grad_skip
         if need_dw:
             a_col = 1 if transposed else 0
-            grad_weight = _weight_grad(be, x, grad_output.contiguous(), entry.fwd, a_col, x.dtype, split=_wgrad_split(cin, cout))
+            split = _wgrad_split(cin, cout)
+            grad_output = grad_output.contiguous()
+            grad_weight = _weight_grad(be, x, grad_output, entry.fwd, a_col, x.dtype, split=split,
+                                       defer=_wgrad_may_defer(be, x, grad_output, weight, hd, split))
             grad_weight = grad_weight.view_as(weight).to(weight.dtype)
         return grad_input, grad_weight, None, None, None, None, None
 
 
-def _weight_grad(be, fa, fb, kmap, a_col, hd, *, split=False, pad_a=False, pad_b=False):
+def _weight_grad(be, fa, fb, kmap, a_col, hd, *, split=False, pad_a=False, pad_b=False, defer=False):
     ca, cb = fa.shape[1], fb.shape[1]
     fa = torch.nn.functional.pad(fa, (0, (-ca) % 4)) if pad_a and ca % 4 else fa
     fb = torch.nn.functional.pad(fb, (0, (-cb) % 4)) if pad_b and cb % 4 else fb
     if hd in _HALF and hasattr(be, "conv_wgrad_h") and fa.shape[1] % 4 == 0 and fb.shape[1] % 4 == 0:
         gw = be.conv_wgrad_h(fa.to(hd), fb.to(hd), kmap, a_col)
+    elif defer:
+        gw = be.conv_wgrad_defer(fa, fb, kmap, a_col)
     else:
         gw = be.conv_wgrad(fa.float(), fb.float(), kmap, a_col, split=split)
     return gw if gw.shape[1:] == (ca, cb) else gw[:, :ca, :cb]
diff --git a/openpcseg_amd/native.py b/openpcseg_amd/native.py
--- a/openpcseg_amd/native.py
+++ b/openpcseg_amd/native.py
@@ -73,6 +73,10 @@
     "pcs_conv_wgrad_ws_bytes": (c_size_t, [_P, c_int32, c_int32, c_int32]),
     "pcs_conv_wgrad_f32": (c_int32, [_P, c_int32, _P, c_int32, _P, c_int32, _P, _P, c_int32, _P,
                                      _P, c_size_t, _P]),
+    "pcs_conv_wgrad_f32_defer": (c_int32, [_P, c_int32, _P, c_int32, _P, c_int32, _P, _P, c_int32, _P,
+                                           _P, c_size_t, _P]),
+    "pcs_conv_wgrad_flush": (c_int32, [_P]),
+    "pcs_conv_wgrad_pending": (c_int32, [_P]),
     "pcs_scatter_max_fwd_f32": (c_int32, [_P, _P, _P, c_int64, c_int32, _P, _P, _P]),
     "pcs_scatter_max_bwd_f32": (c_int32, [_P, _P, c_int64, c_int64, c_int32, _P, _P]),
     "pcs_map_count": (c_int32, [_P, c_int64, c_int32, c_int32, c_int32, _P, _P]),
@@ -149,6 +153,7 @@
     "pcs_lovasz_softmax_f32": (c_int32, [_P, _P, c_int64, c_int32, c_int32, c_int64, _P, _P, _P, c_int64, _P]),
     "pcs_debug_convh_ws": (None, [c_int32, c_int32, c_int32]),
     "pcs_debug_wgrad_interleave": (None, [c_int32]),
+    "pcs_debug_wgrad_ride": (None, [c_int32, c_int32]),
     "pcs_debug_conv_plan": (None, [c_int32] * 7 + [_P]),
     "pcs_debug_pointvoxel_h_inflight": (None, [c_int32]),
     "pcs_debug_cylscan_store": (None, [c_int32]),
@@ -349,12 +354,61 @@
         return KernelMap(pairs, koff, koff_host, self.nbsizes.flip(0), self.n_dst, self.n_src)
 
 
+def _graph_task_id():
+    return torch._C._current_graph_task_id()
+
+
+def _queue_engine_callback(fn):
+    torch.autograd.Variable._execution_engine.queue_callback(fn)
+
+
+class WgradSlot:
+
+    def __init__(self, lib, check=_check):
+        self.lib, self._check = lib, check
+        self.held = {}
+        self._cb_task = None
+
+    def sweep(self):
+        if not self.held:
+            return
+        task = _graph_task_id()
+        for key in [k for k, (t, _) in self.held.items() if t != task]:
+            self.flush(c_void_p(key))
+
+    def hold(self, stream, tensors):
+        task = _graph_task_id()
+        self.held[stream.value or 0] = (task, tensors)
+        if task >= 0 and self._cb_task != task:
+            self._cb_task = task
+            _queue_engine_callback(self._end_of_backward)
+
+    def settle(self, stream):
+        key = stream.value or 0
+        if key in self.held and self.lib.pcs_conv_wgrad_pending(stream) == 0:
+            del self.held[key]
+
+    def flush(self, stream=None):
+        for key in ([stream.value or 0] if stream is not None else list(self.held)):
+            if self.held.pop(key, None) is not None:
+                self._check(self.lib.pcs_conv_wgrad_flush(c_void_p(key)), "pcs_conv_wgrad_flush")
+
+    def pending(self):
+        self.sweep()
+        return len(self.held)
+
+    def _end_of_backward(self):
+        self._cb_task = None
+        self.flush()
+
+
 class HipBackend:
 
     name = "hip-gfx950"
 
     def __init__(self):
         self.lib = load_library()
+        self.wgrad_slot = WgradSlot(self.lib)
 
     def hash(self, coords):
         coords = _dev(coords, "coords", torch.int32)
@@ -878,13 +932,32 @@
         fn = self.lib.pcs_conv_wgrad_f32_bf16x3 if split else self.lib.pcs_conv_wgrad_f32
         return self._wgrad_launch(fn, _dev(fa, "input", torch.float32), _dev(fb, "grad_output", torch.float32), kmap, a_col)
 
-    def _wgrad_launch(self, fn, fa, fb, kmap, a_col, *tail):
+    def conv_wgrad_defer(self, fa, fb, kmap, a_col):
+        slot = self.wgrad_slot
+        slot.sweep()
+        slot.flush(_stream())
+        held = []
+        gw = self._wgrad_launch(self.lib.pcs_conv_wgrad_f32_defer, _dev(fa, "input", torch.float32),
+                                _dev(fb, "grad_output", torch.float32), kmap, a_col, held=held)
+        if held:
+            slot.hold(_stream(), tuple(held))
+        return gw
+
+    def wgrad_flush(self):
+        self.wgrad_slot.sweep()
+        self.wgrad_slot.flush(_stream())
+
+    def _wgrad_launch(self, fn, fa, fb, kmap, a_col, *tail, held=None):
         ca, cb = fa.shape[1], fb.shape[1]
         gw = torch.empty((kmap.K, ca, cb), dtype=torch.float32, device=fa.device)
         ws_bytes = self.lib.pcs_conv_wgrad_ws_bytes(kmap._koff_c, kmap.K, ca, cb)
         ws = torch.empty(max(ws_bytes, 4), dtype=torch.uint8, device=fa.device)
-        _check(fn(_ptr(fa), ca, _ptr(fb), cb, _ptr(kmap.pairs), a_col, _ptr(kmap.koff), kmap._koff_c, kmap.K, _ptr(gw),
-                  _ptr(ws), ws_bytes, *tail, _stream()), "pcs_conv_wgrad_h" if tail else "pcs_conv_wgrad_f32")
+        rc = fn(_ptr(fa), ca, _ptr(fb), cb, _ptr(kmap.pairs), a_col, _ptr(kmap.koff), kmap._koff_c, kmap.K, _ptr(gw),
+                _ptr(ws), ws_bytes, *tail, _stream())
+        if held is not None and rc == 1:
+            held.extend((fa, fb, kmap, gw.detach(), ws))
+            rc = 0
+        _check(rc, "pcs_conv_wgrad_h" if tail else "pcs_conv_wgrad_f32")
         return gw
 
     def _csr(self, index, m):
@@ -1076,8 +1149,11 @@
         sums2 = buf[:2 * c]
         sums2._pcs_f32 = buf[2 * c:].view(torch.float32)
         yp, mp = self._gate(gate, relu)
+        self.wgrad_slot.sweep()
         self._twin("pcs_bn_bwd_stats", self._CODE[x.dtype], [_ptr(dy), _ptr(x), yp, mp, _ptr(stat), n, c, int(relu)],
                    [_ptr(ws), _ptr(sums2), buf.numel(), lddy, _stream()])
+        if self.wgrad_slot.held:
+            self.wgrad_slot.settle(_stream())
         return sums2
 
     def bn_bwd_apply(self, dy, x, gate, stat, sums2, count, w, relu, want_res, count_dev=None, in_slope=None):
@@ -1092,9 +1168,12 @@
                                                  _ptr(w), n, c, int(relu), self._CODE[x.dtype], float(in_slope),
                                                  _ptr(dx), _ptr(dres), lddy, _stream()), "pcs_bn_bwd_apply_act")
             return dx, dres
+        self.wgrad_slot.sweep()
         self._twin("pcs_bn_bwd_apply", self._CODE[x.dtype],
                    [_ptr(dy), _ptr(x), yp, mp, _ptr(stat), _ptr(sums2), float(count), _ptr(count_dev), _ptr(w), n, c, int(relu)],
                    [_ptr(dx), _ptr(dres), lddy, _stream()])
+        if self.wgrad_slot.held:
+            self.wgrad_slot.settle(_stream())
         return dx, dres
 
     def _recon_rows(self, tensors):
```

Measured after the change: 106.0 frames/s (median of 3 runs). About the same (+0.0%).
